# otaviog/align3d

Hardware: AMD Instinct MI355X
Metric: ICP frame-pairs/sec (640x480, 3-lvl, 15 iters) (higher is better)
Workload: dtype f32; 1 GPU; ms3x15 x 64 pairs/GPU, distinct frames, 640x480, 3 lvl x 15 it, HBM-resident (configs[4] shard); pairs_per_gpu=64, global_pairs=64, levels=3, distinct_frames=True, ranks_in_collective=1, collective=none

## Files before the change

### align3d_amd/_abi.py

```python
import ctypes as C
import os
import threading

import numpy as np

A3D_OK = 0
A3D_INVALID_PARAMETER = 1
A3D_MISSING_FIELD = 2
A3D_SOLVE_FAILED = 3
A3D_HIP_ERROR = 4
A3D_NAN_IN_INPUT = 5
A3D_CAST_OVERFLOW = 6

STATUS_NAMES = {
    0: "A3D_OK",
    1: "A3D_INVALID_PARAMETER",
    2: "A3D_MISSING_FIELD",
    3: "A3D_SOLVE_FAILED",
    4: "A3D_HIP_ERROR",
    5: "A3D_NAN_IN_INPUT",
    6: "A3D_CAST_OVERFLOW",
}


class A3dError(Exception):

    def __init__(self, status, message=""):
        self.status = status
        super().__init__(f"{STATUS_NAMES.get(status, status)}: {message}")


class InvalidParameter(A3dError):
    def __init__(self, message):
        super().__init__(A3D_INVALID_PARAMETER, message)


class IcpParamsC(C.Structure):
    _fields_ = [
        ("max_iterations", C.c_uint64),
        ("weight", C.c_float),
        ("color_weight", C.c_float),
        ("max_point_to_plane_distance", C.c_float),
        ("max_distance", C.c_float),
        ("max_normal_angle", C.c_float),
        ("max_color_distance", C.c_float),
    ]


class PoseC(C.Structure):
    _fields_ = [("t", C.c_float * 3), ("q", C.c_float * 4)]


class RangeImageViewC(C.Structure):
    _fields_ = [
        ("points", C.c_void_p),
        ("mask", C.c_void_p),
        ("normals", C.c_void_p),
        ("intensities", C.c_void_p),
        ("intensity_map", C.c_void_p),
        ("fx", C.c_double),
        ("fy", C.c_double),
        ("cx", C.c_double),
        ("cy", C.c_double),
        ("width", C.c_uint64),
        ("height", C.c_uint64),
    ]


class PointCloudViewC(C.Structure):
    _fields_ = [("points", C.c_void_p), ("normals", C.c_void_p), ("len", C.c_uint64)]


class BuilderParamsC(C.Structure):
    _fields_ = [
        ("with_normals", C.c_uint32),
        ("with_intensity", C.c_uint32),
        ("use_bilateral", C.c_uint32),
        ("pad", C.c_uint32),
        ("sigma_space", C.c_double),
        ("sigma_color", C.c_double),
        ("pyramid_levels", C.c_uint64),
        ("blur_sigma", C.c_float),
        ("pad2", C.c_uint32),
    ]


class GnStateC(C.Structure):
    _fields_ = [
        ("hessian", C.c_float * 36),
        ("gradient", C.c_float * 6),
        ("squared_residual_sum", C.c_float),
        ("count", C.c_uint64),
    ]

    def as_dict(self):
        return {
            "H": np.array(self.hessian[:], dtype=np.float32).reshape(6, 6),
            "g": np.array(self.gradient[:], dtype=np.float32),
            "ssq": np.float32(self.squared_residual_sum),
            "count": int(self.count),
        }


def ptr(arr):
    if arr is None:
        return None
    assert arr.flags["C_CONTIGUOUS"], "arrays cross the ABI in standard layout"
    return arr.ctypes.data


_P = C.c_void_p
_PP = C.POINTER(C.c_void_p)
_ST = C.c_int
SIGNATURES = {
    "a3d_abi_version": (C.c_uint32, []),
    "a3d_last_error": (C.c_char_p, []),
    "a3d_status_string": (C.c_char_p, [C.c_int]),
    "a3d_device_count": (_ST, [C.POINTER(C.c_int32)]),
    "a3d_context_create": (_ST, [C.c_int32, _PP]),
    "a3d_context_create_with_priority": (_ST, [C.c_int32, C.c_int32, _PP]),
    "a3d_context_create_pair": (_ST, [C.c_int32, _PP, _PP]),
    "a3d_context_destroy": (_ST, [_P]),
    "a3d_context_synchronize": (_ST, [_P]),
    "a3d_context_stream": (_P, [_P]),
    "a3d_context_device": (C.c_int32, [_P]),
    "a3d_timer_start": (_ST, [_P]),
    "a3d_timer_stop": (_ST, [_P, C.POINTER(C.c_float)]),
    "a3d_malloc": (_ST, [_P, C.c_size_t, _PP]),
    "a3d_host_alloc": (_ST, [_P, C.c_size_t, _PP]),
    "a3d_host_free": (_ST, [_P, _P]),
    "a3d_free": (_ST, [_P, _P]),
    "a3d_memcpy_h2d": (_ST, [_P, _P, _P, C.c_size_t]),
    "a3d_memcpy_d2h": (_ST, [_P, _P, _P, C.c_size_t]),
    "a3d_memcpy_d2d": (_ST, [_P, _P, _P, C.c_size_t]),
    "a3d_icp_params_default": (None, [C.POINTER(IcpParamsC)]),
    "a3d_ms_icp_params_default": (None, [C.POINTER(IcpParamsC)]),
    "a3d_range_image_upload": (_ST, [_P, C.POINTER(RangeImageViewC), _PP]),
    "a3d_range_image_upload_pyramid": (_ST, [_P, C.POINTER(RangeImageViewC), C.c_uint64, _PP]),
    "a3d_range_image_free": (_ST, [_P]),
    "a3d_range_image_compute_normals": (_ST, [_P]),
    "a3d_range_image_download_normals": (_ST, [_P, _P]),
    "a3d_builder_params_default": (None, [C.POINTER(BuilderParamsC)]),
    "a3d_range_image_build_pyramid": (
        _ST,
        [_P, C.POINTER(BuilderParamsC), _P, _P, C.c_uint64, C.c_uint64, C.c_double, C.c_double, C.c_double,
         C.c_double, C.c_double, _PP],
    ),
    "a3d_range_image_build_pyramids": (
        _ST,
        [_P, C.POINTER(BuilderParamsC), C.c_uint64, _PP, _PP, C.c_uint64, C.c_uint64, C.c_double, C.c_double, C.c_double,
         C.c_double, C.c_double, _PP],
    ),
    "a3d_context_last_build_stats": (_ST, [_P, C.POINTER(C.c_uint64)]),
    "a3d_context_set_build_profiling": (_ST, [_P, C.c_int32]),
    "a3d_context_last_build_kernel_ms": (_ST, [_P, C.POINTER(C.c_float)]),
    "a3d_range_image_size": (_ST, [_P, C.POINTER(C.c_uint64), C.POINTER(C.c_uint64)]),
    "a3d_range_image_download": (_ST, [_P, _P, _P, _P, _P, _P, _P, C.POINTER(C.c_double)]),
    "a3d_compute_normals": (_ST, [_P, _P, _P, C.c_uint64, C.c_uint64, _P]),
    "a3d_range_image_compute_normals_batch": (_ST, [_PP, C.c_uint64]),
    "a3d_image_icp_align": (_ST, [_P, C.POINTER(IcpParamsC), _P, _P, C.POINTER(PoseC), C.POINTER(PoseC)]),
    "a3d_image_icp_accumulate": (
        _ST,
        [_P, C.POINTER(IcpParamsC), _P, _P, C.POINTER(PoseC), C.POINTER(GnStateC), C.POINTER(GnStateC)],
    ),
    "a3d_image_icp_align_trace": (
        _ST,
        [_P, C.POINTER(IcpParamsC), _P, _P, C.POINTER(PoseC), C.POINTER(PoseC), _P],
    ),
    "a3d_selftest_division": (_ST, [_P, _P, _P, C.c_uint64, C.POINTER(C.c_uint64)]),
    "a3d_selftest_transform": (_ST, [_P, _P, _P, _P, C.c_uint64, _P, _P, _P]),
    "a3d_multiscale_new": (_ST, [_P, C.POINTER(IcpParamsC), C.c_uint64, _PP, C.c_uint64, _PP]),
    "a3d_multiscale_align": (_ST, [_P, _PP, C.c_uint64, C.POINTER(PoseC)]),
    "a3d_multiscale_align_host": (_ST, [_P, C.POINTER(RangeImageViewC), C.c_uint64, C.POINTER(PoseC)]),
    "a3d_multiscale_free": (_ST, [_P]),
    "a3d_multiscale_batch_new": (
        _ST,
        [_P, C.POINTER(IcpParamsC), C.c_uint64, C.c_uint64, C.c_uint64, _PP, _PP, _PP],
    ),
    "a3d_multiscale_batch_align": (_ST, [_P, C.POINTER(PoseC), _P, C.POINTER(C.c_int32)]),
    "a3d_multiscale_batch_free": (_ST, [_P]),
    "a3d_multiscale_batch_rebind": (_ST, [_P, _P, _P]),
    "a3d_multiscale_batch_last_level_ms": (_ST, [_P, C.c_uint32, C.POINTER(C.c_float), C.POINTER(C.c_uint32)]),
    "a3d_multiscale_batch_results": (_ST, [_P, C.POINTER(PoseC), C.POINTER(C.c_int32)]),
    "a3d_multiscale_batch_last_timing": (_ST, [_P, C.POINTER(C.c_float), C.POINTER(C.c_uint64)]),
    "a3d_multiscale_batch_set_profiling": (_ST, [_P, C.c_int32]),
    "a3d_multiscale_batch_last_kernel_ms": (_ST, [_P, C.POINTER(C.c_float)]),
    "a3d_multiscale_batch_concurrency": (_ST, [_P, C.POINTER(C.c_uint32)]),
    "a3d_multiscale_batch_persistent_levels": (_ST, [_P, C.POINTER(C.c_uint32)]),
    "a3d_context_set_tiling": (_ST, [_P, C.c_uint32]),
    "a3d_context_create_on_pipe": (_ST, [C.c_int32, C.c_int32, C.c_int32, _PP]),
    "a3d_multi_shard_range": (_ST, [C.c_uint64, C.c_uint64, C.c_uint64, C.POINTER(C.c_uint64), C.POINTER(C.c_uint64)]),
    "a3d_multi_context_create": (_ST, [C.POINTER(C.c_int32), C.c_uint64, _PP]),
    "a3d_multi_context_destroy": (_ST, [_P]),
    "a3d_multi_context_size": (C.c_uint64, [_P]),
    "a3d_multi_context_device": (_P, [_P, C.c_uint64]),
    "a3d_multiscale_batch_new_multi": (
        _ST,
        [_P, C.POINTER(IcpParamsC), C.c_uint64, C.c_uint64, C.c_uint64, _PP, _PP, _PP],
    ),
    "a3d_multiscale_multi_batch_align": (_ST, [_P, C.POINTER(PoseC), _P, C.POINTER(C.c_int32), _PP]),
    "a3d_multiscale_multi_batch_free": (_ST, [_P]),
    "a3d_kdtree_stats": (_ST, [_P, C.POINTER(C.c_uint64)]),
    "a3d_kdtree_download": (_ST, [_P, _P, _P, C.POINTER(C.c_uint64)]),
    "a3d_kdtree_new": (_ST, [_P, _P, C.c_uint64, _PP]),
    "a3d_kdtree_new_device": (_ST, [_P, _P, C.c_uint64, _PP]),
    "a3d_kdtree_build_path": (_ST, [_P, C.POINTER(C.c_int32)]),
    "a3d_kdtree_build_ms": (_ST, [_P, C.POINTER(C.c_float)]),
    "a3d_kdtree_nearest": (_ST, [_P, _P, C.c_uint64, _P, _P]),
    "a3d_kdtree_nearest_device": (_ST, [_P, _P, C.c_uint64, _P, _P]),
    "a3d_kdtree_free": (_ST, [_P]),
    "a3d_pcl_icp_new": (_ST, [_P, C.POINTER(IcpParamsC), C.POINTER(PointCloudViewC), _PP]),
    "a3d_pcl_icp_align": (_ST, [_P, C.POINTER(PointCloudViewC), C.POINTER(PoseC)]),
    "a3d_pcl_icp_new_device": (_ST, [_P, C.POINTER(IcpParamsC), C.POINTER(PointCloudViewC), _PP]),
    "a3d_pcl_icp_align_device": (_ST, [_P, C.POINTER(PointCloudViewC), C.POINTER(PoseC)]),
    "a3d_pcl_icp_accumulate": (_ST, [_P, C.POINTER(PointCloudViewC), C.POINTER(PoseC), C.POINTER(GnStateC)]),
    "a3d_pcl_icp_last_device_ms": (_ST, [_P, C.POINTER(C.c_float)]),
    "a3d_pcl_icp_free": (_ST, [_P]),
    "a3d_bilateral_default_sigmas": (None, [C.POINTER(C.c_double), C.POINTER(C.c_double)]),
    "a3d_bilateral_filter_u16": (
        _ST,
        [_P, _P, C.c_uint64, C.c_uint64, C.c_double, C.c_double, _P, C.POINTER(C.c_uint64)],
    ),
    "a3d_bilateral_filter_u16_device": (_ST, [_P, _P, C.c_uint64, C.c_uint64, C.c_uint64, C.c_double, C.c_double, _P]),
}

DIAG_SIGNATURES = {
    "a3d_image_icp_accumulate_exact": (
        _ST,
        [_P, C.POINTER(IcpParamsC), _P, _P, C.POINTER(PoseC), C.POINTER(GnStateC), C.POINTER(GnStateC)],
    ),
    "a3d_image_icp_accumulate_weighted": (
        _ST,
        [_P, C.POINTER(IcpParamsC), _P, _P, C.POINTER(PoseC), C.POINTER(GnStateC)],
    ),
}

_CSRC = os.path.join(os.path.dirname(os.path.abspath(__file__)), "csrc")
LIB_PATH = os.environ.get("A3D_LIBRARY") or os.path.join(_CSRC, "libalign3d_hip.so")
DIAG_LIB_PATH = os.path.join(_CSRC, "libalign3d_hip_diag.so")
_libs = {}


def load_library(path=None):
    path = os.path.abspath(path or LIB_PATH)
    if path in _libs:
        return _libs[path]
    if not os.path.exists(path):
        raise RuntimeError(
            f"{path} not found: build the HIP extension first "
            "(python -c 'import __graft_entry__ as g; g.build()' or make -C align3d_amd/csrc all)"
        )
    lib = C.CDLL(path)
    for name, (restype, argtypes) in SIGNATURES.items():
        fn = getattr(lib, name)
        fn.restype = restype
        fn.argtypes = argtypes
        if restype is _ST:
            _note_failures(lib, fn)
    for name, (restype, argtypes) in DIAG_SIGNATURES.items():
        fn = getattr(lib, name, None)
        if fn is not None:
            fn.restype = restype
            fn.argtypes = argtypes
            if restype is _ST:
                _note_failures(lib, fn)
    if lib.a3d_abi_version() != 1:
        raise RuntimeError("libalign3d_hip.so ABI version mismatch")
    _libs[path] = lib
    return lib


_failed = threading.local()


def _note_failures(lib, fn):
    def errcheck(result, func, args):
        if result != A3D_OK:
            _failed.lib = lib
        return result
    fn.errcheck = errcheck


def check(status, what="", lib=None):
    if status != A3D_OK:
        lib = lib or getattr(_failed, "lib", None) or load_library()
        msg = lib.a3d_last_error().decode("utf-8", "replace")
        raise A3dError(status, f"{what}: {msg}" if what else msg)
```

### align3d_amd/csrc/common.hpp

```cpp
#pragma once
#include <hip/hip_runtime.h>

#include <atomic>
#include <memory>
#include <cstdarg>
#include <cstdio>
#include <cstring>
#include <mutex>
#include <string>
#include <utility>
#include <vector>

#include "../../include/align3d_hip.h"
#include "devmath.hpp"

struct a3d_context;

#ifdef A3D_DIAGNOSTICS
#define A3D_DIAG_ENV(name) getenv(name)
#else
#define A3D_DIAG_ENV(name) ((const char*)nullptr)
#endif

namespace a3d {

void set_error(const char* fmt, ...);

#define A3D_HIP_TRY(expr)                                                                 \
  do {                                                                                    \
    hipError_t _e = (expr);                                                               \
    if (_e != hipSuccess) {                                                               \
      a3d::set_error("%s failed: %s (%s:%d)", #expr, hipGetErrorString(_e), __FILE__, __LINE__); \
      return A3D_HIP_ERROR;                                                               \
    }                                                                                     \
  } while (0)

#define A3D_TRY(expr)                  \
  do {                                 \
    a3d_status _s = (expr);            \
    if (_s != A3D_OK) return _s;       \
  } while (0)

#define A3D_REQUIRE(cond, status, msg) \
  do {                                 \
    if (!(cond)) {                     \
      a3d::set_error("%s", msg);       \
      return status;                   \
    }                                  \
  } while (0)

inline Pose pose_from_c(const a3d_pose* p) {
  return Pose{{p->t[0], p->t[1], p->t[2]}, {p->q[0], p->q[1], p->q[2], p->q[3]}};
}
inline void pose_to_c(const Pose& p, a3d_pose* o) {
  o->t[0] = p.t.x, o->t[1] = p.t.y, o->t[2] = p.t.z;
  o->q[0] = p.q.i, o->q[1] = p.q.j, o->q[2] = p.q.k, o->q[3] = p.q.w;
}

float acos_gate_threshold(float thr, bool strict);

}

namespace a3d {
a3d_status bilateral_filter_device(a3d_context* ctx, const uint16_t* d_img, uint16_t* d_out, uint32_t w, uint32_t h,
                                   double sigma_space, double sigma_color, uint64_t out_grid_dims[3]);
a3d_status upload_pyramid(a3d_context* ctx, const a3d_range_image_view* views, uint64_t n_levels,
                          a3d_device_image** out_images, hipEvent_t* level_events);
a3d_status compute_normals_device(a3d_context* ctx, const float* d_points, const uint8_t* d_mask, float* d_normals,
                                  uint32_t w, uint32_t h);
}

namespace a3d {
struct UseFence;
}
struct a3d_context {
  int device = 0;
  hipStream_t stream = nullptr;
  hipEvent_t ev_start = nullptr, ev_stop = nullptr;
  hipEvent_t kd_ev[2] = {nullptr, nullptr};
  int num_cus = 0;
  void* scratch[3] = {nullptr, nullptr, nullptr};
  size_t scratch_size[3] = {0, 0, 0};
  struct SpareBlock {
    void* p;
    size_t bytes;
  };
  std::vector<SpareBlock> spare_blocks;
  std::atomic<bool> kd_wide_place{true};
  std::atomic<int> kd_quiet_builds{0};
  std::mutex pool_mutex;
  std::vector<std::pair<void*, size_t>> arena_pool;
  std::vector<void*> single_arenas;
  std::vector<void*> arena_slabs;
  std::vector<size_t> slab_sizes;
  size_t slab_bytes_total = 0;
  void* icp_engine = nullptr;
  void (*icp_engine_free)(void*) = nullptr;
  uint32_t* pinned_words = nullptr;
  static constexpr size_t PINNED_WORDS = 16384;
  static constexpr size_t PINNED_EXTRA = 16;
  hipStream_t copy_stream = nullptr;
  std::vector<hipEvent_t> copy_events;
  unsigned long long grid_capacity = 0;
  struct GridLayoutKey {
    const void* region = nullptr;
    unsigned long long capacity = 0;
    uint32_t cell_bytes = 0, flags_stride = 0, frames = 0, columns = 0;
  } grid_clean;
  uint32_t grid_layout_frames = 0;
  std::vector<std::pair<size_t, uint32_t>> arena_requests;
  struct CachedTable {
    uint32_t key[4];
    void* d;
  };
  std::vector<CachedTable> tables;
  int stream_priority = 0;
  std::mutex stream_mutex;
  std::vector<hipStream_t> side_streams;
  uint64_t build_stats[4] = {0, 0, 0, 0};
  bool build_profiling = false;
  std::vector<hipEvent_t> build_events;
  float last_build_kernel_ms = 0.f;
  uint32_t tiles_per_pair = 0;
  int live_arenas = 0;
  bool zombie = false;
};

namespace a3d {
a3d_status ctx_side_stream(a3d_context* ctx, uint32_t index, hipStream_t* out);
a3d_status ctx_scratch(a3d_context* ctx, int which, size_t bytes, void** out);
a3d_status ctx_block_alloc(a3d_context* ctx, size_t bytes, void** out, size_t* out_bytes);
void ctx_block_release(a3d_context* ctx, void* p, size_t bytes);

struct DeviceArena {
  void* base = nullptr;
  size_t bytes = 0;
  bool slab_slice = false;
  std::atomic<int> refs{0};
  std::mutex fence_mutex;
  std::vector<std::shared_ptr<struct UseFence>> fences;
  std::shared_ptr<struct UseFence> self_fence;
};

struct UseFence {
  std::mutex m;
  hipEvent_t ev = nullptr;
  bool recorded = false;
  hipStream_t deferred = nullptr;
  int deferred_device = -1;
  void record_locked(hipStream_t s) {
    if (!ev && hipEventCreateWithFlags(&ev, hipEventDisableTiming) != hipSuccess) {
      ev = nullptr;
      return;
    }
    recorded = hipEventRecord(ev, s) == hipSuccess;
  }
  void record(hipStream_t s) {
    std::lock_guard<std::mutex> lock(m);
    record_locked(s);
  }
  void record_later(hipStream_t s, int device) {
    std::lock_guard<std::mutex> lock(m);
    deferred = s, deferred_device = device;
  }
  void settle_locked() {
    if (deferred && !recorded) {
      int current = -1;
      const bool switched = deferred_device >= 0 && hipGetDevice(&current) == hipSuccess && current != deferred_device &&
                            hipSetDevice(deferred_device) == hipSuccess;
      record_locked(deferred);
      if (!recorded) (void)hipStreamSynchronize(deferred);
      if (switched) (void)hipSetDevice(current);
    }
    deferred = nullptr;
  }
  void wait() {
    std::lock_guard<std::mutex> lock(m);
    settle_locked();
    if (ev && recorded) hipEventSynchronize(ev);
  }
  bool wait_on(hipStream_t s) {
    std::lock_guard<std::mutex> lock(m);
    if (deferred == s && !recorded) return true;
    settle_locked();
    return !(ev && recorded) || hipStreamWaitEvent(s, ev, 0) == hipSuccess;
  }
  void retire() {
    std::lock_guard<std::mutex> lock(m);
    if (ev) hipEventDestroy(ev);
    ev = nullptr, recorded = false;
  }
  ~UseFence() {
    if (ev) hipEventDestroy(ev);
  }
};
#ifdef __HIPCC__
__device__ __forceinline__ uint32_t xcd_contiguous_index(uint32_t b, uint32_t n) {
  const uint32_t g = b & 7u, k = b >> 3, q = n >> 3, r = n & 7u;
  return (g < r ? g * (q + 1u) : r * (q + 1u) + (g - r) * q) + k;
}
#endif

a3d_status ctx_cached_table(a3d_context* ctx, const uint32_t key[4], const void* host, size_t bytes, void** out);

a3d_status ctx_arena_acquire(a3d_context* ctx, size_t bytes, DeviceArena* out);
void ctx_arena_release(a3d_context* ctx, DeviceArena* arena);
void ctx_destroy_now(a3d_context* ctx);
}

struct a3d_device_image;
namespace a3d {
void attach_fence(const a3d_device_image* im, const std::shared_ptr<UseFence>& fence);
}

struct a3d_device_image {
  a3d_context* ctx = nullptr;
  uint32_t width = 0, height = 0;
  double fx64 = 0, fy64 = 0, cx64 = 0, cy64 = 0;
  float fx = 0, fy = 0, cx = 0, cy = 0;
  float* points = nullptr;
  uint8_t* mask = nullptr;
  float* normals = nullptr;
  uint8_t* intensities = nullptr;
  float* imap = nullptr;
  uint8_t* colors = nullptr;
  bool has_normals = false, has_intensities = false, has_imap = false;
  a3d::DeviceArena* arena = nullptr;
  bool built = false;
  bool mask_is_z = false;
  bool own_normals = false;
};
```

### align3d_amd/csrc/devmath.hpp

```cpp
#pragma once
#include <hip/hip_runtime.h>
#include <math.h>
#include <stdint.h>

#define A3D_HD __host__ __device__ __forceinline__

namespace a3d {

struct V3 {
  float x, y, z;
};
A3D_HD V3 operator+(V3 a, V3 b) { return {a.x + b.x, a.y + b.y, a.z + b.z}; }
A3D_HD V3 operator-(V3 a, V3 b) { return {a.x - b.x, a.y - b.y, a.z - b.z}; }
A3D_HD V3 operator*(V3 a, float s) { return {a.x * s, a.y * s, a.z * s}; }
A3D_HD V3 operator/(V3 a, float s) { return {a.x / s, a.y / s, a.z / s}; }
A3D_HD float dot(V3 a, V3 b) { return (a.x * b.x + a.y * b.y) + a.z * b.z; }
A3D_HD float norm_squared(V3 a) { return dot(a, a); }
A3D_HD V3 cross(V3 a, V3 b) {
  return {a.y * b.z - a.z * b.y, a.z * b.x - a.x * b.z, a.x * b.y - a.y * b.x};
}

struct Quat {
  float i, j, k, w;
};
struct Pose {
  V3 t;
  Quat q;
};
A3D_HD Pose pose_eye() { return {{0.f, 0.f, 0.f}, {0.f, 0.f, 0.f, 1.f}}; }

A3D_HD V3 rotate(const Quat& q, V3 v) {
  V3 qv{q.i, q.j, q.k};
  V3 t = cross(qv, v) * 2.0f;
  V3 c = cross(qv, t);
  return (t * q.w + c) + v;
}
A3D_HD V3 transform_vector(const Pose& p, V3 v) { return rotate(p.q, v) + p.t; }
A3D_HD V3 transform_normal(const Pose& p, V3 v) { return rotate(p.q, v); }

A3D_HD Quat qmul(const Quat& a, const Quat& b) {
  Quat r;
  r.w = a.w * b.w - a.i * b.i - a.j * b.j - a.k * b.k;
  r.i = a.w * b.i + a.i * b.w + a.j * b.k - a.k * b.j;
  r.j = a.w * b.j - a.i * b.k + a.j * b.w + a.k * b.i;
  r.k = a.w * b.k + a.i * b.j - a.j * b.i + a.k * b.w;
  return r;
}
A3D_HD Pose compose(const Pose& a, const Pose& b) {
  Pose r;
  r.t = a.t + rotate(a.q, b.t);
  r.q = qmul(a.q, b.q);
  return r;
}

A3D_HD Quat qnormalize(Quat q) {
  float a = q.i * q.i, b = q.j * q.j, c = q.k * q.k, d = q.w * q.w;
  a += c;
  b += d;
  float n = sqrtf(a + b);
  return {q.i / n, q.j / n, q.k / n, q.w / n};
}

A3D_HD float sin_f32(float x) { return sinf(x); }
A3D_HD float cos_f32(float x) { return cosf(x); }

struct Se3Trig {
  float theta, sin_half, cos_half, sin_theta, cos_theta;
};
A3D_HD float se3_theta(const float u[6]) { return sqrtf(norm_squared(V3{u[3], u[4], u[5]})); }

A3D_HD Pose exp_se3_trig(const float u[6], const Se3Trig& tg) {
  const float EPS = 1e-8f;
  V3 omega{u[3], u[4], u[5]};
  float theta_sq0 = norm_squared(omega);
  float theta, imag, real;
  if (theta_sq0 < EPS * EPS) {
    float po4 = theta_sq0 * theta_sq0;
    theta = 0.0f;
    imag = 0.5f - (1.0f / 48.0f) * theta_sq0 + (1.0f / 3840.0f) * po4;
    real = 1.0f - (1.0f / 8.0f) * theta_sq0 + (1.0f / 384.0f) * po4;
  } else {
    theta = tg.theta;
    imag = tg.sin_half / theta;
    real = tg.cos_half;
  }
  Quat q = qnormalize(Quat{imag * omega.x, imag * omega.y, imag * omega.z, real});
  float theta_sq = theta * theta;
  float W[3][3] = {{0.f, -omega.z, omega.y}, {omega.z, 0.f, -omega.x}, {-omega.y, omega.x, 0.f}};
  float V[3][3];
  if (theta_sq < EPS) {
    for (int r = 0; r < 3; ++r)
      for (int c = 0; c < 3; ++c) V[r][c] = (r == c ? 1.0f : 0.0f) + W[r][c] * 0.5f;
  } else {
    float W2[3][3];
    for (int c = 0; c < 3; ++c)
      for (int r = 0; r < 3; ++r) {
        float acc = W[r][0] * W[0][c];
        acc = W[r][1] * W[1][c] + acc;
        acc = W[r][2] * W[2][c] + acc;
        W2[r][c] = acc;
      }
    float a = (1.0f - tg.cos_theta) / theta_sq;
    float b = (theta - tg.sin_theta) / (theta_sq * theta);
    for (int r = 0; r < 3; ++r)
      for (int c = 0; c < 3; ++c) V[r][c] = ((r == c ? 1.0f : 0.0f) + W[r][c] * a) + W2[r][c] * b;
  }
  Pose p;
  float rho[3] = {u[0], u[1], u[2]}, t[3];
  for (int r = 0; r < 3; ++r) {
    float acc = V[r][0] * rho[0];
    acc = V[r][1] * rho[1] + acc;
    acc = V[r][2] * rho[2] + acc;
    t[r] = acc;
  }
  p.t = {t[0], t[1], t[2]};
  p.q = q;
  return p;
}

A3D_HD Pose exp_se3(const float u[6]) {
  Se3Trig tg;
  tg.theta = se3_theta(u);
  const float half = 0.5f * tg.theta;
  tg.sin_half = sin_f32(half), tg.cos_half = cos_f32(half);
  tg.sin_theta = sin_f32(tg.theta), tg.cos_theta = cos_f32(tg.theta);
  return exp_se3_trig(u, tg);
}

A3D_HD void pose_to_matrix(const Pose& p, float m[16]) {
  const float i = p.q.i, j = p.q.j, k = p.q.k, w = p.q.w;
  float ww = w * w, ii = i * i, jj = j * j, kk = k * k;
  float ij = i * j * 2.0f, wk = w * k * 2.0f, wj = w * j * 2.0f, ik = i * k * 2.0f;
  float jk = j * k * 2.0f, wi = w * i * 2.0f;
  m[0] = ww + ii - jj - kk, m[1] = ij - wk, m[2] = wj + ik, m[3] = p.t.x;
  m[4] = wk + ij, m[5] = ww - ii + jj - kk, m[6] = jk - wi, m[7] = p.t.y;
  m[8] = ik - wj, m[9] = wi + jk, m[10] = ww - ii - jj + kk, m[11] = p.t.z;
  m[12] = 0.f, m[13] = 0.f, m[14] = 0.f, m[15] = 1.f;
}

A3D_HD bool gn_solve6(const float H[36], const float g[6], float out[6]) {
  double L[6][6], b[6];
  for (int r = 0; r < 6; ++r) {
    for (int c = 0; c < 6; ++c) L[r][c] = (double)H[r * 6 + c];
    b[r] = (double)g[r];
  }
  for (int j = 0; j < 6; ++j) {
    for (int k = 0; k < j; ++k) {
      double factor = -L[j][k];
      for (int r = j; r < 6; ++r) L[r][j] = factor * L[r][k] + L[r][j];
    }
    double diag = L[j][j];
    if (diag == 0.0) return false;
    if (!(diag >= 0.0)) return false;
    double denom = sqrt(diag);
    L[j][j] = denom;
    for (int r = j + 1; r < 6; ++r) L[r][j] /= denom;
  }
  for (int i = 0; i < 6; ++i) {
    double coeff = b[i] / L[i][i];
    b[i] = coeff;
    for (int r = i + 1; r < 6; ++r) b[r] = -coeff * L[r][i] + b[r];
  }
  for (int i = 5; i >= 0; --i) {
    double d = 0.0;
    for (int r = i + 1; r < 6; ++r) d += L[r][i] * b[r];
    b[i] = (b[i] - d) / L[i][i];
  }
  for (int i = 0; i < 6; ++i) out[i] = (float)b[i];
  return true;
}

A3D_HD constexpr int tri6(int r, int c) { return r * 6 - (r * (r - 1)) / 2 + (c - r); }

#if defined(__HIPCC__)
struct DivBy {
  float negz, y;
};
__device__ __forceinline__ DivBy div_prepare(float z) {
  const float r = __builtin_amdgcn_rcpf(z);
  const float e = __builtin_fmaf(-z, r, 1.0f);
  return {-z, __builtin_fmaf(e, r, r)};
}
__device__ __forceinline__ float div_by(float a, const DivBy d) {
  const float q = a * d.y;
  const float r1 = __builtin_fmaf(d.negz, q, a);
  const float q1 = __builtin_fmaf(r1, d.y, q);
  const float r2 = __builtin_fmaf(d.negz, q1, a);
  return __builtin_fmaf(r2, d.y, q1);
}
__device__ __forceinline__ bool div_den_ok(float z) { return (fabsf(z) > 1e-9f) & (fabsf(z) < 1e9f); }
__device__ __forceinline__ bool div_num_ok(float a) { return (a == 0.0f) | ((fabsf(a) > 1e-20f) & (fabsf(a) < 1e9f)); }


__device__ __forceinline__ V3 normal_from_neighbours_dev(V3 center, V3 left, V3 right, V3 top, V3 bottom) {
  const float ld = norm_squared(left - center), rd = norm_squared(right - center);
  V3 left_to_right;
  if ((ld < 4.0f * rd) & (4.0f * ld > rd))
    left_to_right = right - left;
  else if (ld < rd)
    left_to_right = center - left;
  else
    left_to_right = right - center;
  const float bd = norm_squared(bottom - center), td = norm_squared(top - center);
  V3 bottom_to_top;
  if ((bd < 4.0f * td) & (4.0f * bd > td))
    bottom_to_top = top - bottom;
  else if (bd < td)
    bottom_to_top = center - bottom;
  else
    bottom_to_top = top - center;
  const V3 n = cross(left_to_right, bottom_to_top);
  const float mag = sqrtf(norm_squared(n));
  V3 out{0.f, 0.f, 0.f};
  const bool keep = mag > 1e-6f;
  const bool fast = div_den_ok(mag) & div_num_ok(n.x) & div_num_ok(n.y) & div_num_ok(n.z);
  if (__builtin_expect(__builtin_amdgcn_ballot_w64(keep & !fast) != 0ull, 0)) {
    if (keep) out = n / mag;
  } else if (keep) {
    const DivBy d = div_prepare(mag);
    out = V3{n.x == 0.0f ? n.x : div_by(n.x, d), n.y == 0.0f ? n.y : div_by(n.y, d), n.z == 0.0f ? n.z : div_by(n.z, d)};
  }
  return out;
}

#endif

A3D_HD V3 normal_from_neighbours(V3 center, V3 left, V3 right, V3 top, V3 bottom) {
  const float thr_sq = 2.0f * 2.0f;
  float ld = norm_squared(left - center), rd = norm_squared(right - center);
  float lr_ratio = ld / rd;
  V3 left_to_right;
  if (lr_ratio < thr_sq && lr_ratio > 1.0f / thr_sq)
    left_to_right = right - left;
  else if (ld < rd)
    left_to_right = center - left;
  else
    left_to_right = right - center;
  float bd = norm_squared(bottom - center), td = norm_squared(top - center);
  float bt_ratio = bd / td;
  V3 bottom_to_top;
  if (bt_ratio < thr_sq && bt_ratio > 1.0f / thr_sq)
    bottom_to_top = top - bottom;
  else if (bd < td)
    bottom_to_top = center - bottom;
  else
    bottom_to_top = top - center;
  V3 n = cross(left_to_right, bottom_to_top);
  float mag = sqrtf(norm_squared(n));
  V3 out{0.f, 0.f, 0.f};
  if (mag > 1e-6f) out = n / mag;
  return out;
}

}
```

### align3d_amd/csrc/frame.hip

```cpp
#include <cmath>
#include <cstdlib>
#include <memory>

#include "bilateral.hpp"

using namespace a3d;

namespace {

#ifndef A3D_MAX_BATCH
#define A3D_MAX_BATCH 48
#endif
#ifndef A3D_GRID_BUDGET_GB
#define A3D_GRID_BUDGET_GB 4
#endif
constexpr uint32_t MAX_BATCH = A3D_MAX_BATCH;
struct FrameBases {
  char* arena[MAX_BATCH];
};

typedef float f32x3 __attribute__((ext_vector_type(3)));
typedef f32x3 __attribute__((aligned(4))) f32x3_u;
__device__ __forceinline__ void st_v3(float* base, size_t idx, V3 v) { *(f32x3_u*)(base + 3 * idx) = f32x3{v.x, v.y, v.z}; }
__device__ __forceinline__ void st_v3u(void* base, uint32_t idx, V3 v) {
  *(f32x3_u __attribute__((address_space(1)))*)((a3d_gptr)base + idx * 12u) = f32x3{v.x, v.y, v.z};
}
__device__ __forceinline__ void st_u8u(void* base, uint32_t idx, uint8_t v) {
  *(uint8_t __attribute__((address_space(1)))*)((a3d_gptr)base + idx) = v;
}
__device__ __forceinline__ void st_v3u_stream(void* base, uint32_t idx, V3 v) {
#ifdef A3D_BUILDER_NO_NT
  st_v3u(base, idx, v);
#else
  __builtin_nontemporal_store(f32x3{v.x, v.y, v.z}, (f32x3_u __attribute__((address_space(1)))*)((a3d_gptr)base + idx * 12u));
#endif
}
__device__ __forceinline__ void st_u8u_stream(void* base, uint32_t idx, uint8_t v) {
#ifdef A3D_BUILDER_NO_NT
  st_u8u(base, idx, v);
#else
  __builtin_nontemporal_store(v, (uint8_t __attribute__((address_space(1)))*)((a3d_gptr)base + idx));
#endif
}
__device__ __forceinline__ V3 ld_v3g(const float* base, size_t idx) {
  const f32x3 v = *(const f32x3_u*)(base + 3 * idx);
  return V3{v.x, v.y, v.z};
}

struct LevelLayout {
  uint32_t w, h;
  size_t points, mask, normals, colors, intensities, imap;
};
constexpr uint32_t MAX_LEVELS = 16;
struct PyramidLayout {
  LevelLayout lv[MAX_LEVELS];
};

__device__ __forceinline__ V3 pick_nearest_to_mean(const V3 (&cand)[4], const bool (&ok)[4], int* n_valid) {
  int n = 0;
#pragma unroll
  for (int q = 0; q < 4; ++q) n += ok[q] ? 1 : 0;
  *n_valid = n;
  V3 nearest{0.f, 0.f, 0.f};
  if (n > 0) {
    V3 sum{0.f, 0.f, 0.f};
#pragma unroll
    for (int q = 0; q < 4; ++q)
      if (ok[q]) sum = sum + cand[q];
    V3 mean = sum * (n == 1 ? 1.0f : (n == 2 ? 0.5f : 0.25f));
    if (__builtin_amdgcn_ballot_w64(n == 3) != 0ull)
      if (n == 3) mean = sum / 3.0f;
    float min_dist = 3.402823466e+38f;
#pragma unroll
    for (int q = 0; q < 4; ++q) {
      const float d = norm_squared(cand[q] - mean);
      if (ok[q] && d < min_dist) {
        min_dist = d;
        nearest = cand[q];
      }
    }
  }
  return nearest;
}

#ifdef A3D_DIAGNOSTICS
constexpr int ST_W = 32, ST_H = 16, OWN_W = ST_W - 2, OWN_H = ST_H - 2;

constexpr int L0_PPT = 2, L0_THREADS = ST_W * ST_H / L0_PPT;
#ifndef A3D_L0_PROBE
#define A3D_L0_PROBE 0
#endif
template <bool FILTER>
__global__ void __launch_bounds__(L0_THREADS)
    level0_kernel(const uint16_t* __restrict__ depth, uint32_t w, uint32_t h, double inv_ss, double inv_sc,
                  const double* __restrict__ grids, unsigned long long capacity, uint32_t* __restrict__ scal, float fx,
                  float fy, float cx, float cy, float scale, FrameBases bases, size_t off_points, size_t off_mask,
                  size_t off_normals, bool with_normals, LevelLayout L1, bool emit_l1) {
  __shared__ float sp[3][ST_H][ST_W + 1];
  __shared__ float sn[3][OWN_H][OWN_W + 1];
  __shared__ uint8_t sm[ST_H][ST_W];
  const uint32_t f = blockIdx.z;
  const int lx = threadIdx.x % ST_W, ly0 = threadIdx.x / ST_W;
  const int col = (int)blockIdx.x * OWN_W + lx - 1;
  int ly[L0_PPT], row[L0_PPT];
  bool in[L0_PPT];
  uint32_t d[L0_PPT];
  float px[L0_PPT], py[L0_PPT], pz[L0_PPT];
#pragma unroll
  for (int k = 0; k < L0_PPT; ++k) {
    ly[k] = ly0 + k * (ST_H / L0_PPT);
    row[k] = (int)blockIdx.y * OWN_H + ly[k] - 1;
    in[k] = col >= 0 && col < (int)w && row[k] >= 0 && row[k] < (int)h;
    d[k] = in[k] ? *(const uint16_t __attribute__((address_space(1)))*)((a3d_gptr_c)(depth + (size_t)f * w * h) +
                                                                        (__umul24((uint32_t)row[k], w) + (uint32_t)col) * 2u)
                 : 0u;
    px[k] = py[k] = pz[k] = 0.f;
  }
  const DivBy dfx = div_prepare(fx), dfy = div_prepare(fy);
  const bool focal_ok = div_den_ok(fx) & div_den_ok(fy);
#pragma unroll
  for (int k = 0; k < L0_PPT; ++k) {
    if (in[k]) {
      if (FILTER) {
        uint32_t* sc = scal + f * SC_STRIDE;
        GridDims g;
        uint32_t cmin;
        if (dyn_dims(sc, &g, &cmin)) {
          uint16_t v;
          if (!slice_pixel<true>(d[k], (uint32_t)row[k], (uint32_t)col, inv_ss, inv_sc, cmin, g, grids + f * capacity, &v))
            atomicOr(&sc[SC_OVERFLOW], 1u);
          d[k] = v;
        }
      }
      if (d[k] > 0) {
        pz[k] = (float)d[k] * scale;
        const float ax = ((float)col - cx) * pz[k], ay = ((float)row[k] - cy) * pz[k];
        const bool fast = focal_ok & div_num_ok(ax) & div_num_ok(ay);
        if (__builtin_expect(__builtin_amdgcn_ballot_w64(!fast) != 0ull, 0)) {
          px[k] = ax / fx, py[k] = ay / fy;
        } else {
          px[k] = ax == 0.0f ? ax : div_by(ax, dfx), py[k] = ay == 0.0f ? ay : div_by(ay, dfy);
        }
      }
    }
    sp[0][ly[k]][lx] = px[k], sp[1][ly[k]][lx] = py[k], sp[2][ly[k]][lx] = pz[k];
    sm[ly[k]][lx] = d[k] > 0 ? 1 : 0;
  }
  __syncthreads();
  char* base = bases.arena[f];
  auto at = [&](int y, int x) { return V3{sp[0][y][x], sp[1][y][x], sp[2][y][x]}; };
  bool owned[L0_PPT];
  V3 nrm[L0_PPT];
#pragma unroll
  for (int k = 0; k < L0_PPT; ++k) {
    owned[k] = in[k] && lx != 0 && lx != ST_W - 1 && ly[k] != 0 && ly[k] != ST_H - 1;
    nrm[k] = V3{0.f, 0.f, 0.f};
    if (owned[k] && with_normals && A3D_L0_PROBE != 2 && A3D_L0_PROBE != 4) {
      nrm[k] = normal_from_neighbours_dev(V3{px[k], py[k], pz[k]}, at(ly[k], lx - 1), at(ly[k], lx + 1), at(ly[k] - 1, lx),
                                      at(ly[k] + 1, lx));
      if (emit_l1) sn[0][ly[k] - 1][lx - 1] = nrm[k].x, sn[1][ly[k] - 1][lx - 1] = nrm[k].y, sn[2][ly[k] - 1][lx - 1] = nrm[k].z;
    }
  }
  if (emit_l1) __syncthreads();
#pragma unroll
  for (int k = 0; k < L0_PPT; ++k)
    if (owned[k] && ((A3D_L0_PROBE != 1 && A3D_L0_PROBE != 4) || px[k] == 12345.678f)) {
      const uint32_t idx = __umul24((uint32_t)row[k], w) + (uint32_t)col;
      st_v3u_stream(base + off_points, idx, V3{px[k], py[k], pz[k]});
      st_u8u_stream(base + off_mask, idx, d[k] > 0 ? 1 : 0);
      if (with_normals) st_v3u_stream(base + off_normals, idx, nrm[k]);
    }
  if (!emit_l1 || A3D_L0_PROBE == 3 || A3D_L0_PROBE == 4) return;
  constexpr int L1W = OWN_W / 2, L1N = (OWN_W / 2) * (OWN_H / 2);
  const int t = (int)threadIdx.x;
  const bool normals_task = t >= L1N;
  const int task = normals_task ? t - L1N : t;
  if (task >= L1N || (normals_task && !with_normals)) return;
  const int oy = 2 * (task / L1W), ox = 2 * (task % L1W);
  const uint32_t r0 = blockIdx.y * OWN_H + (uint32_t)oy, c0 = blockIdx.x * OWN_W + (uint32_t)ox;
  if (r0 >= h || c0 >= w) return;
  V3 cand[4];
  bool ok[4];
#pragma unroll
  for (int a = 0; a < 2; ++a)
#pragma unroll
    for (int b = 0; b < 2; ++b) {
      const int q = a * 2 + b;
      cand[q] = normals_task ? V3{sn[0][oy + a][ox + b], sn[1][oy + a][ox + b], sn[2][oy + a][ox + b]}
                             : at(oy + 1 + a, ox + 1 + b);
      ok[q] = sm[oy + 1 + a][ox + 1 + b] == 1;
    }
  int n_valid;
  const V3 pk = pick_nearest_to_mean(cand, ok, &n_valid);
  const uint32_t i1 = __umul24(r0 >> 1, L1.w) + (c0 >> 1);
  st_v3u(base + (normals_task ? L1.normals : L1.points), i1, pk);
  if (!normals_task) st_u8u(base + L1.mask, i1, n_valid > 0 ? 1 : 0);
}
#endif

constexpr int QS = 32, QT = QS / 2;

__device__ __forceinline__ V3 backproject_px(uint32_t d, int row, int col, float fx, float fy, float cx, float cy, float scale,
                                             const DivBy dfx, const DivBy dfy, bool focal_ok) {
  V3 p{0.f, 0.f, 0.f};
  if (d > 0) {
    p.z = (float)d * scale;
    const float ax = ((float)col - cx) * p.z, ay = ((float)row - cy) * p.z;
    const bool fast = focal_ok & div_num_ok(ax) & div_num_ok(ay);
    if (__builtin_expect(__builtin_amdgcn_ballot_w64(!fast) != 0ull, 0)) {
      p.x = ax / fx, p.y = ay / fy;
    } else {
      p.x = ax == 0.0f ? ax : div_by(ax, dfx), p.y = ay == 0.0f ? ay : div_by(ay, dfy);
    }
  }
  return p;
}

template <bool FILTER>
__global__ void __launch_bounds__(256)
    level0_quad_kernel(const uint16_t* __restrict__ depth, uint32_t w, uint32_t h, double inv_ss, double inv_sc,
                       const double* __restrict__ grids, unsigned long long capacity, uint32_t* __restrict__ scal, float fx,
                       float fy, float cx, float cy, float scale, FrameBases bases, size_t off_points, size_t off_mask,
                       size_t off_normals, bool with_normals, LevelLayout L1, bool emit_l1, LevelLayout L2, bool emit_l2,
                       bool l2_is_last, Unsplat unsplat, uint32_t patches_x, uint32_t patches_y) {
  __shared__ float sp[3][QS + 2][QS + 3];
  __shared__ float s1[2][3][QT][QT + 1];
  __shared__ uint8_t s1m[QT][QT];
  __shared__ __attribute__((aligned(4))) uint8_t sm[QS][QS];
#ifndef A3D_LQ_XCD
#define A3D_LQ_XCD 0
#endif
  uint32_t f = blockIdx.z, bx = blockIdx.x, by = blockIdx.y;
  if (patches_x) {
    const uint32_t v = A3D_LQ_XCD ? xcd_contiguous_index(blockIdx.x, gridDim.x) : blockIdx.x;
    const uint32_t per_frame = patches_x * patches_y;
    f = v / per_frame;
    const uint32_t in_frame = v - f * per_frame;
    by = in_frame / patches_x, bx = in_frame - by * patches_x;
  }
  const int t = (int)threadIdx.x, tx = t & (QT - 1), ty = t >> 4;
  const int r0 = (int)by * QS, c0 = (int)bx * QS;
  const uint16_t __attribute__((address_space(1)))* dimg =
      (const uint16_t __attribute__((address_space(1)))*)(depth + (size_t)f * w * h);
  auto load_depth = [&](int row, int col) -> uint32_t {
    const uint32_t r = (uint32_t)min(max(row, 0), (int)h - 1), c = (uint32_t)min(max(col, 0), (int)w - 1);
    return *(const uint16_t __attribute__((address_space(1)))*)((a3d_gptr_c)dimg + (__umul24(r, w) + c) * 2u);
  };
  int row[2], col[2];
  bool rin[2], cin[2];
#pragma unroll
  for (int a = 0; a < 2; ++a) {
    row[a] = r0 + 2 * ty + a, col[a] = c0 + 2 * tx + a;
    rin[a] = row[a] < (int)h, cin[a] = col[a] < (int)w;
  }
  const bool halo_thread = t < 4 * QS;
  const int side = t >> 5, hi = t & (QS - 1);
  const int hy = side == 0 ? 0 : (side == 1 ? QS + 1 : hi + 1), hx = side == 2 ? 0 : (side == 3 ? QS + 1 : hi + 1);
  const int hrow = r0 + hy - 1, hcol = c0 + hx - 1;
  const bool hin = halo_thread && hrow >= 0 && hrow < (int)h && hcol >= 0 && hcol < (int)w;
  uint32_t d[2][2], dh = 0;
#pragma unroll
  for (int a = 0; a < 2; ++a)
#pragma unroll
    for (int b = 0; b < 2; ++b) d[a][b] = load_depth(row[a], col[b]);
  if (halo_thread) dh = load_depth(hrow, hcol);
#pragma unroll
  for (int a = 0; a < 2; ++a)
#pragma unroll
    for (int b = 0; b < 2; ++b) d[a][b] = (rin[a] && cin[b]) ? d[a][b] : 0u;
  dh = hin ? dh : 0u;
  const DivBy dfx = div_prepare(fx), dfy = div_prepare(fy);
  const bool focal_ok = div_den_ok(fx) & div_den_ok(fy);
  GridDims g{0, 0, 0};
  bool grid_ok = false;
  if (FILTER) {
    uint32_t* sc = scal + f * SC_STRIDE;
    uint32_t cmin;
    grid_ok = dyn_dims(sc, &g, &cmin);
    if (grid_ok) {
      const double* grid = grids + f * capacity;
      SliceAxis ry[2], cxs[2];
#pragma unroll
      for (int a = 0; a < 2; ++a) {
        ry[a] = slice_axis_spatial((uint32_t)min(row[a], (int)h - 1), inv_ss, g.gh);
        cxs[a] = slice_axis_spatial((uint32_t)min(col[a], (int)w - 1), inv_ss, g.gw);
      }
      SliceAxis hry{}, hcx{};
      if (halo_thread) {
        hry = slice_axis_spatial((uint32_t)min(max(hrow, 0), (int)h - 1), inv_ss, g.gh);
        hcx = slice_axis_spatial((uint32_t)min(max(hcol, 0), (int)w - 1), inv_ss, g.gw);
      }
      auto colour_axis = [&](uint32_t dv) { return slice_axis((double)(dv - cmin) * inv_sc + 2.0, g.gd); };
      SliceAxis cz[2][2], czh{};
#pragma unroll
      for (int a = 0; a < 2; ++a)
#pragma unroll
        for (int b = 0; b < 2; ++b) cz[a][b] = colour_axis(d[a][b]);
      if (halo_thread) czh = colour_axis(dh);
      auto gather = [&](const SliceAxis& ry_, const SliceAxis& cx_, const SliceAxis& cz_, SliceTaps* tp) {
        tp->za = cz_.frac;
        const uint32_t g0 = __umul24(ry_.lo, g.gw), g1 = __umul24(ry_.hi, g.gw);
        const uint32_t b00 = __umul24(g0 + cx_.lo, g.gd), b01 = __umul24(g0 + cx_.hi, g.gd), b10 = __umul24(g1 + cx_.lo, g.gd),
                       b11 = __umul24(g1 + cx_.hi, g.gd);
        tp->v[0] = cell_value32(grid, b00, cz_.lo), tp->v[1] = cell_value32(grid, b01, cz_.lo);
        tp->v[2] = cell_value32(grid, b10, cz_.lo), tp->v[3] = cell_value32(grid, b11, cz_.lo);
        tp->v[4] = cell_value32(grid, b00, cz_.hi), tp->v[5] = cell_value32(grid, b01, cz_.hi);
        tp->v[6] = cell_value32(grid, b10, cz_.hi), tp->v[7] = cell_value32(grid, b11, cz_.hi);
      };
      bool overflow = false;
      auto finish = [&](const SliceTaps& tp, double ya, double xa, bool in) -> uint32_t {
        uint16_t v;
        const bool fits = slice_combine(tp, ya, xa, &v);
        overflow |= in && !fits;
        return in ? (uint32_t)v : 0u;
      };
      {
        SliceTaps taps[2], htaps;
        gather(ry[0], cxs[0], cz[0][0], &taps[0]);
        gather(ry[0], cxs[1], cz[0][1], &taps[1]);
        if (halo_thread) gather(hry, hcx, czh, &htaps);
        d[0][0] = finish(taps[0], ry[0].frac, cxs[0].frac, rin[0] && cin[0]);
        d[0][1] = finish(taps[1], ry[0].frac, cxs[1].frac, rin[0] && cin[1]);
        __builtin_amdgcn_sched_barrier(0);
        gather(ry[1], cxs[0], cz[1][0], &taps[0]);
        gather(ry[1], cxs[1], cz[1][1], &taps[1]);
        if (halo_thread) dh = finish(htaps, hry.frac, hcx.frac, hin);
        d[1][0] = finish(taps[0], ry[1].frac, cxs[0].frac, rin[1] && cin[0]);
        d[1][1] = finish(taps[1], ry[1].frac, cxs[1].frac, rin[1] && cin[1]);
      }
      if (overflow) atomicOr(&sc[SC_OVERFLOW], 1u);
    }
  }
  V3 P[2][2];
#pragma unroll
  for (int a = 0; a < 2; ++a)
#pragma unroll
    for (int b = 0; b < 2; ++b) {
      P[a][b] = backproject_px(d[a][b], row[a], col[b], fx, fy, cx, cy, scale, dfx, dfy, focal_ok);
      const int y = 2 * ty + a + 1, x = 2 * tx + b + 1;
      sp[0][y][x] = P[a][b].x, sp[1][y][x] = P[a][b].y, sp[2][y][x] = P[a][b].z;
      sm[y - 1][x - 1] = d[a][b] > 0 ? 1 : 0;
    }
  if (halo_thread) {
    const V3 ph = backproject_px(dh, hrow, hcol, fx, fy, cx, cy, scale, dfx, dfy, focal_ok);
    sp[0][hy][hx] = ph.x, sp[1][hy][hx] = ph.y, sp[2][hy][hx] = ph.z;
  }
  __syncthreads();
#ifdef A3D_DIAGNOSTICS
  if (FILTER && grid_ok && unsplat.packed)
    unsplat_columns(unsplat, f, g, inv_ss, r0, min(r0 + QS, (int)h), c0, min(c0 + QS, (int)w), by * patches_x + bx,
                    patches_x * patches_y);
#endif
  char* base = bases.arena[f];
  auto at = [&](int y, int x) { return V3{sp[0][y][x], sp[1][y][x], sp[2][y][x]}; };
  V3 N[2][2];
#pragma unroll
  for (int a = 0; a < 2; ++a)
#pragma unroll
    for (int b = 0; b < 2; ++b) {
      N[a][b] = V3{0.f, 0.f, 0.f};
      if (with_normals && rin[a] && cin[b]) {
        const int y = 2 * ty + a + 1, x = 2 * tx + b + 1;
        const V3 left = b ? P[a][0] : at(y, x - 1), right = b ? at(y, x + 1) : P[a][1];
        const V3 top = a ? P[0][b] : at(y - 1, x), bottom = a ? at(y + 1, x) : P[1][b];
        N[a][b] = normal_from_neighbours_dev(P[a][b], left, right, top, bottom);
      }
    }
#ifndef A3D_LQ_PROBE
#define A3D_LQ_PROBE 0
#endif
  const int sx = t & (QS - 1), sy0 = t >> 5;
  const bool scol_in = c0 + sx < (int)w;
  auto store_rows = [&](size_t off, bool with_mask) {
#pragma unroll
    for (int k = 0; k < 4; ++k) {
      const int y = sy0 + 8 * k;
      if (scol_in && r0 + y < (int)h && (A3D_LQ_PROBE != 1 || sp[0][y + 1][sx + 1] == 12345.678f)) {
        const uint32_t idx = __umul24((uint32_t)(r0 + y), w) + (uint32_t)(c0 + sx);
        st_v3u_stream(base + off, idx, at(y + 1, sx + 1));
        if (with_mask) st_u8u_stream(base + off_mask, idx, sm[y][sx]);
      }
    }
  };
  const bool mask_words = (w & 3u) == 0;
  if (mask_words) {
    const int my = t >> 3, mx = 4 * (t & 7);
    if (r0 + my < (int)h && c0 + mx < (int)w && A3D_LQ_PROBE != 1)
      __builtin_nontemporal_store(*(const uint32_t*)&sm[my][mx],
                                  (uint32_t __attribute__((address_space(1)))*)((a3d_gptr)(base + off_mask) +
                                                                               (__umul24((uint32_t)(r0 + my), w) + (uint32_t)(c0 + mx))));
  }
  store_rows(off_points, !mask_words);
  if (with_normals) {
    __syncthreads();
#pragma unroll
    for (int a = 0; a < 2; ++a)
#pragma unroll
      for (int b = 0; b < 2; ++b) {
        const int y = 2 * ty + a + 1, x = 2 * tx + b + 1;
        sp[0][y][x] = N[a][b].x, sp[1][y][x] = N[a][b].y, sp[2][y][x] = N[a][b].z;
      }
    __syncthreads();
    store_rows(off_normals, false);
  }
  if (!emit_l1 || A3D_LQ_PROBE == 3) return;
  const bool quad_in = rin[0] && cin[0];
  V3 cand[4];
  bool ok[4];
#pragma unroll
  for (int q = 0; q < 4; ++q) cand[q] = P[q >> 1][q & 1], ok[q] = d[q >> 1][q & 1] > 0;
  int n_valid = 0;
  const V3 pk_p = pick_nearest_to_mean(cand, ok, &n_valid);
  V3 pk_n{0.f, 0.f, 0.f};
  if (with_normals) {
#pragma unroll
    for (int q = 0; q < 4; ++q) cand[q] = N[q >> 1][q & 1];
    int unused;
    pk_n = pick_nearest_to_mean(cand, ok, &unused);
  }
  if (quad_in) {
    const uint32_t i1 = __umul24((uint32_t)row[0] >> 1, L1.w) + ((uint32_t)col[0] >> 1);
    if (emit_l2) {
      st_v3u_stream(base + L1.points, i1, pk_p);
      st_u8u_stream(base + L1.mask, i1, n_valid > 0 ? 1 : 0);
      if (with_normals) st_v3u_stream(base + L1.normals, i1, pk_n);
    } else {
      st_v3u(base + L1.points, i1, pk_p);
      st_u8u(base + L1.mask, i1, n_valid > 0 ? 1 : 0);
      if (with_normals) st_v3u(base + L1.normals, i1, pk_n);
    }
  }
  if (!emit_l2) return;
  s1[0][0][ty][tx] = pk_p.x, s1[0][1][ty][tx] = pk_p.y, s1[0][2][ty][tx] = pk_p.z;
  s1[1][0][ty][tx] = pk_n.x, s1[1][1][ty][tx] = pk_n.y, s1[1][2][ty][tx] = pk_n.z;
  s1m[ty][tx] = (quad_in && n_valid > 0) ? 1 : 0;
  __syncthreads();
  const int which = t >> 6;
  if (which > 1 || (which == 1 && !with_normals)) return;
  const int ly = (t >> 3) & 7, lx = t & 7;
  const uint32_t r2 = ((uint32_t)r0 >> 2) + (uint32_t)ly, c2 = ((uint32_t)c0 >> 2) + (uint32_t)lx;
  if (r2 >= L2.h || c2 >= L2.w) return;
#pragma unroll
  for (int q = 0; q < 4; ++q) {
    const int y = 2 * ly + (q >> 1), x = 2 * lx + (q & 1);
    cand[q] = V3{s1[which][0][y][x], s1[which][1][y][x], s1[which][2][y][x]};
    ok[q] = s1m[y][x] == 1;
  }
  const V3 pk2 = pick_nearest_to_mean(cand, ok, &n_valid);
  const uint32_t i2 = __umul24(r2, L2.w) + c2;
  char* dst = base + (which ? L2.normals : L2.points);
  if (l2_is_last) {
    st_v3u_stream(dst, i2, pk2);
    if (!which) st_u8u_stream(base + L2.mask, i2, n_valid > 0 ? 1 : 0);
  } else {
    st_v3u(dst, i2, pk2);
    if (!which) st_u8u(base + L2.mask, i2, n_valid > 0 ? 1 : 0);
  }
}

__global__ void __launch_bounds__(256) scatter_colors_kernel(const uint4* __restrict__ staged, size_t bytes_per_frame,
                                                             size_t off_colors, FrameBases bases) {
  const size_t i = (size_t)blockIdx.x * 256 + threadIdx.x, n16 = bytes_per_frame / 16;
  const uint8_t* src = (const uint8_t*)staged + (size_t)blockIdx.z * bytes_per_frame;
  uint8_t* dst = (uint8_t*)(bases.arena[blockIdx.z] + off_colors);
  if (i < n16) ((uint4*)dst)[i] = ((const uint4*)src)[i];
  if (i == 0)
    for (size_t k = n16 * 16; k < bytes_per_frame; ++k) dst[k] = src[k];
}

__device__ __forceinline__ uint8_t luma_u8(const uint8_t* __restrict__ rgb, uint32_t i) {
  const float l = (float)rgb[3 * i] * 0.3f + (float)rgb[3 * i + 1] * 0.59f + (float)rgb[3 * i + 2] * 0.11f;
  return l >= 255.0f ? 255 : (l <= 0.0f ? 0 : (uint8_t)l);
}

__device__ __forceinline__ uint8_t luma_of(uint32_t r, uint32_t g, uint32_t b) {
  const float l = (float)r * 0.3f + (float)g * 0.59f + (float)b * 0.11f;
  return l >= 255.0f ? 255 : (l <= 0.0f ? 0 : (uint8_t)l);
}
__device__ __forceinline__ float imap_border_cell(const uint8_t* __restrict__ rgb, uint32_t w, uint32_t h, uint32_t r, uint32_t c) {
  if (r >= h && c + 1 < w) return (float)luma_u8(rgb, (h - 1) * w + c) / 255.0f;
  if (c >= w && r + 1 < h) return (float)luma_u8(rgb, r * w + (w - 1)) / 255.0f;
  if ((r == h && c == w) || (r == h + 1 && c == w + 1)) return (float)luma_u8(rgb, (h - 1) * w + (w - 1)) / 255.0f;
  return 0.0f;
}
template <bool QUADS>
__global__ void __launch_bounds__(256) luma_imap_kernel(PyramidLayout layout, FrameBases bases) {
  const LevelLayout L = layout.lv[blockIdx.y];
  const uint32_t i = blockIdx.x * blockDim.x + threadIdx.x;
  const uint32_t w = L.w, h = L.h, mw = w + 2, mh = h + 2;
  char* base = bases.arena[blockIdx.z];
  const uint8_t* __restrict__ rgb = (const uint8_t*)(base + L.colors);
  float* __restrict__ imap = (float*)(base + L.imap);
  if (QUADS) {
    const uint32_t qpr = w / 4, n_quads = h * qpr, n_border = 2 * mw + 2 * h;
    if (i < n_quads) {
      const uint32_t r = i / qpr, c = 4 * (i % qpr), px = r * w + c;
      const uint32_t* src = (const uint32_t*)(rgb + (size_t)px * 3);
      const uint32_t a = src[0], b = src[1], d = src[2];
      const uint8_t l0 = luma_of(a & 255u, (a >> 8) & 255u, (a >> 16) & 255u);
      const uint8_t l1 = luma_of(a >> 24, b & 255u, (b >> 8) & 255u);
      const uint8_t l2 = luma_of((b >> 16) & 255u, b >> 24, d & 255u);
      const uint8_t l3 = luma_of((d >> 8) & 255u, (d >> 16) & 255u, d >> 24);
      const uint32_t packed4 = (uint32_t)l0 | ((uint32_t)l1 << 8) | ((uint32_t)l2 << 16) | ((uint32_t)l3 << 24);
      float* o = imap + (size_t)r * mw + c;
#ifdef A3D_BUILDER_NO_NT
      *(uint32_t*)((uint8_t*)(base + L.intensities) + px) = packed4;
      o[0] = (float)l0 / 255.0f, o[1] = (float)l1 / 255.0f, o[2] = (float)l2 / 255.0f, o[3] = (float)l3 / 255.0f;
#else
      __builtin_nontemporal_store(packed4, (uint32_t*)((uint8_t*)(base + L.intensities) + px));
      __builtin_nontemporal_store((float)l0 / 255.0f, o), __builtin_nontemporal_store((float)l1 / 255.0f, o + 1);
      __builtin_nontemporal_store((float)l2 / 255.0f, o + 2), __builtin_nontemporal_store((float)l3 / 255.0f, o + 3);
#endif
    } else if (i < n_quads + n_border) {
      const uint32_t j = i - n_quads;
      uint32_t r, c;
      if (j < 2 * mw) r = h + j / mw, c = j % mw;
      else r = (j - 2 * mw) / 2, c = w + ((j - 2 * mw) & 1u);
      imap[(size_t)r * mw + c] = imap_border_cell(rgb, w, h, r, c);
    }
    return;
  }
  if (i >= mw * mh) return;
  const uint32_t r = i / mw, c = i % mw;
  float v;
  if (r < h && c < w) {
    const uint8_t l = luma_u8(rgb, r * w + c);
    ((uint8_t*)(base + L.intensities))[r * w + c] = l;
    v = (float)l / 255.0f;
  } else {
    v = imap_border_cell(rgb, w, h, r, c);
  }
  imap[i] = v;
}

__global__ void __launch_bounds__(256) resize_pick_kernel(LevelLayout S, LevelLayout D, FrameBases bases) {
  const uint32_t sw = S.w, sh = S.h, dw = D.w, dh = D.h;
  const uint32_t i = blockIdx.x * blockDim.x + threadIdx.x;
  if (i >= dw * dh) return;
  char* base = bases.arena[blockIdx.z];
  const bool normals = blockIdx.y == 1;
  const float* __restrict__ src = (const float*)(base + (normals ? S.normals : S.points));
  float* __restrict__ dst = (float*)(base + (normals ? D.normals : D.points));
  const uint8_t* __restrict__ src_mask = (const uint8_t*)(base + S.mask);
  const uint32_t dv = i / dw, du = i % dw;
  const float hr = (float)sh / (float)dh, wr = (float)sw / (float)dw;
  const uint32_t sv = (uint32_t)((float)dv * hr), su = (uint32_t)((float)du * wr);
  V3 cand[4];
  bool ok[4];
#pragma unroll
  for (uint32_t a = 0; a < 2; ++a)
#pragma unroll
    for (uint32_t b = 0; b < 2; ++b) {
      const uint32_t r = sv + a, c = su + b, q = a * 2 + b;
      const bool in = r < sh && c < sw;
      const uint32_t k = in ? r * sw + c : 0u;
      ok[q] = in && src_mask[k] == 1;
      cand[q] = ld_v3g(src, k);
    }
  int n;
  const V3 nearest = pick_nearest_to_mean(cand, ok, &n);
  st_v3u_stream(dst, i, nearest);
  if (!normals) st_u8u_stream(base + D.mask, i, n > 0 ? 1 : 0);
}

constexpr int MAX_TAPS = 14;
struct TapRow {
  int32_t left, count;
  float w[MAX_TAPS];
};
__host__ __device__ __forceinline__ void tap_range(uint32_t o, float support, uint32_t size, int32_t* left, int32_t* count) {
  const float in = (float)o + 0.5f;
  int32_t l = (int32_t)floorf(in - support);
  l = l < 0 ? 0 : (l > (int32_t)size - 1 ? (int32_t)size - 1 : l);
  int32_t r = (int32_t)ceilf(in + support);
  r = r < l + 1 ? l + 1 : (r > (int32_t)size ? (int32_t)size : r);
  *left = l, *count = r - l < MAX_TAPS ? r - l : MAX_TAPS;
}

constexpr uint32_t BLUR_TILE = 64, BLUR_ROWS = 4;
constexpr uint32_t BLUR_SPAN = 3 * (2 * BLUR_TILE + MAX_TAPS + 2);
constexpr uint32_t RAW_ROWS = 2 * (BLUR_ROWS - 1) + MAX_TAPS;
constexpr uint32_t RAW_PITCH = ((BLUR_SPAN + 3 + 3) / 4) * 4;
__global__ void __launch_bounds__(256)
    blur_halve_kernel(size_t off_src, uint32_t w, uint32_t dw, uint32_t dh, const TapRow* __restrict__ taps_v,
                      const TapRow* __restrict__ taps_h, size_t off_dst, FrameBases bases) {
  __shared__ uint32_t s_raw[RAW_ROWS * RAW_PITCH / 4];
  __shared__ float s_v[BLUR_ROWS * BLUR_SPAN];
  __shared__ uint32_t s_shift[RAW_ROWS];
  const uint8_t* __restrict__ rgb = (const uint8_t*)(bases.arena[blockIdx.z] + off_src);
  uint8_t* __restrict__ out = (uint8_t*)(bases.arena[blockIdx.z] + off_dst);
  const uint32_t dy0 = blockIdx.y * BLUR_ROWS, rows = min(BLUR_ROWS, dh - dy0);
  const uint32_t dx0 = blockIdx.x * BLUR_TILE, dx1 = min(dx0 + BLUR_TILE, dw) - 1;
  const int32_t vtop = taps_v[dy0].left, vbot = taps_v[dy0 + rows - 1].left + taps_v[dy0 + rows - 1].count;
  const int32_t cmin = taps_h[dx0].left, cmax = taps_h[dx1].left + taps_h[dx1].count;
  const uint32_t span = (uint32_t)(cmax - cmin) * 3u, nraw = (uint32_t)(vbot - vtop);
  const uint32_t words = (span + 3 + 3) / 4;
  for (uint32_t e = threadIdx.x; e < nraw * words; e += 256) {
    const uint32_t j = e / words, k = e % words;
    const size_t first = ((size_t)(vtop + (int32_t)j) * w + (size_t)cmin) * 3;
    s_raw[j * (RAW_PITCH / 4) + k] = *(const uint32_t*)(rgb + (first & ~(size_t)3) + 4 * (size_t)k);
  }
  if (threadIdx.x < nraw)
    s_shift[threadIdx.x] = (uint32_t)((((size_t)(vtop + (int32_t)threadIdx.x) * w + (size_t)cmin) * 3) & 3);
  __syncthreads();
  const uint8_t* raw = (const uint8_t*)s_raw;
  for (uint32_t r = 0; r < rows; ++r) {
    const TapRow* tv = taps_v + dy0 + r;
    const int32_t j0 = tv->left - vtop, vcount = tv->count;
    for (uint32_t x = threadIdx.x; x < span; x += 256) {
      float acc = 0.0f;
#pragma unroll
      for (int k = 0; k < MAX_TAPS; ++k)
        if (k < vcount) {
          const uint32_t j = (uint32_t)(j0 + k);
          acc += (float)raw[j * RAW_PITCH + s_shift[j] + x] * tv->w[k];
        }
      s_v[r * BLUR_SPAN + x] = acc;
    }
  }
  __syncthreads();
  const uint32_t o = threadIdx.x, dx = dx0 + o / 3, ch = o % 3;
  if (o >= BLUR_TILE * 3 || dx >= dw) return;
  const TapRow th = taps_h[dx];
  const uint32_t h0 = (uint32_t)(th.left - cmin) * 3u + ch;
  for (uint32_t r = 0; r < rows; ++r) {
    float acc = 0.0f;
#pragma unroll
    for (int k = 0; k < MAX_TAPS; ++k)
      if (k < th.count) acc += s_v[r * BLUR_SPAN + h0 + 3u * (uint32_t)k] * th.w[k];
    acc = fminf(fmaxf(acc, 0.0f), 255.0f);
    *(uint8_t __attribute__((address_space(1)))*)((a3d_gptr)out + (((dy0 + r) * dw + dx) * 3u + ch)) = (uint8_t)roundf(acc);
  }
}

__global__ void __launch_bounds__(256)
    blur_halve_words_kernel(size_t off_src, uint32_t w, uint32_t h, uint32_t dw, uint32_t dh, float support,
                            const TapRow* __restrict__ taps_v, const TapRow* __restrict__ taps_h, size_t off_dst,
                            FrameBases bases) {
  constexpr uint32_t PITCH_W = RAW_PITCH / 4;
  __shared__ uint32_t s_raw[RAW_ROWS * PITCH_W];
  __shared__ __attribute__((aligned(16))) float s_v[BLUR_ROWS * PITCH_W * 4];
  __shared__ uint32_t s_tv[BLUR_ROWS][16];
  static_assert(sizeof(TapRow) == 64, "a tap row is sixteen words");
  const uint8_t* __restrict__ rgb = (const uint8_t*)(bases.arena[blockIdx.z] + off_src);
  uint8_t* __restrict__ out = (uint8_t*)(bases.arena[blockIdx.z] + off_dst);
  const uint32_t dy0 = blockIdx.y * BLUR_ROWS, rows = min(BLUR_ROWS, dh - dy0);
  const uint32_t dx0 = blockIdx.x * BLUR_TILE, dx1 = min(dx0 + BLUR_TILE, dw) - 1;
  int32_t vtop, vbot, cmin, cmax, cnt;
  tap_range(2 * dy0, support, h, &vtop, &cnt);
  tap_range(2 * (dy0 + rows - 1), support, h, &vbot, &cnt), vbot += cnt;
  tap_range(2 * dx0, support, w, &cmin, &cnt);
  tap_range(2 * dx1, support, w, &cmax, &cnt), cmax += cnt;
  const uint32_t span = (uint32_t)(cmax - cmin) * 3u, nraw = (uint32_t)(vbot - vtop);
  const uint32_t sh = ((uint32_t)cmin * 3u) & 3u;
  const uint32_t words = (span + sh + 3) / 4;
  const uint32_t o = threadIdx.x, dx = dx0 + o / 3, ch = o % 3;
  const bool owns_output = o < BLUR_TILE * 3 && dx < dw;
  uint4 th4[4] = {};
  if (owns_output) {
    const uint4* src = (const uint4*)(taps_h + dx);
#pragma unroll
    for (int i = 0; i < 4; ++i) th4[i] = src[i];
  }
  const bool stages_taps = threadIdx.x < rows * 16u;
  const uint32_t tv_word = stages_taps ? ((const uint32_t*)(taps_v + dy0))[threadIdx.x] : 0u;
  {
    const uint32_t k = threadIdx.x & 127u, jj = threadIdx.x >> 7;
    const uint32_t row_bytes = w * 3u;
    const uint32_t first = (((uint32_t)vtop * w + (uint32_t)cmin) * 3u & ~3u) + 4u * k;
    uint32_t got[RAW_ROWS / 2];
#pragma unroll
    for (uint32_t i = 0; i < RAW_ROWS / 2; ++i) {
      const uint32_t j = jj + 2 * i;
      got[i] = (k < words && j < nraw) ? *(const uint32_t __attribute__((address_space(1)))*)((a3d_gptr_c)rgb + (first + j * row_bytes)) : 0u;
    }
#pragma unroll
    for (uint32_t i = 0; i < RAW_ROWS / 2; ++i) {
      const uint32_t j = jj + 2 * i;
      if (k < words && j < nraw) s_raw[j * PITCH_W + k] = got[i];
    }
  }
  if (stages_taps) s_tv[threadIdx.x >> 4][threadIdx.x & 15u] = tv_word;
  __syncthreads();
  for (uint32_t e = threadIdx.x; e < rows * 128u; e += 256) {
    const uint32_t r = e >> 7, q = e & 127u;
    if (q >= words) continue;
    const int32_t j0 = (int32_t)s_tv[r][0] - vtop, vcount = __builtin_amdgcn_readfirstlane((int32_t)s_tv[r][1]);
    float a0 = 0.0f, a1 = 0.0f, a2 = 0.0f, a3 = 0.0f;
    auto tap = [&](int k) {
      const uint32_t word = s_raw[(uint32_t)(j0 + k) * PITCH_W + q];
      const float wk = __uint_as_float(s_tv[r][2 + k]);
      a0 += (float)(word & 255u) * wk, a1 += (float)((word >> 8) & 255u) * wk;
      a2 += (float)((word >> 16) & 255u) * wk, a3 += (float)(word >> 24) * wk;
    };
    constexpr int SHORT_TAPS = 6;
    if (vcount <= SHORT_TAPS) {
#pragma unroll
      for (int k = 0; k < SHORT_TAPS; ++k)
        if (k < vcount) tap(k);
    } else {
#pragma unroll
      for (int k = 0; k < MAX_TAPS; ++k)
        if (k < vcount) tap(k);
    }
    *(float4*)(s_v + (r * PITCH_W + q) * 4) = make_float4(a0, a1, a2, a3);
  }
  __syncthreads();
  if (!owns_output) return;
  const uint32_t tw[16] = {th4[0].x, th4[0].y, th4[0].z, th4[0].w, th4[1].x, th4[1].y, th4[1].z, th4[1].w,
                           th4[2].x, th4[2].y, th4[2].z, th4[2].w, th4[3].x, th4[3].y, th4[3].z, th4[3].w};
  const int32_t hcount = (int32_t)tw[1];
  const uint32_t h0 = (uint32_t)((int32_t)tw[0] - cmin) * 3u + ch + sh;
  const bool short_taps = __builtin_amdgcn_ballot_w64(hcount > 6) == 0ull;
  for (uint32_t r = 0; r < rows; ++r) {
    float acc = 0.0f;
    if (short_taps) {
#pragma unroll
      for (int k = 0; k < 6; ++k)
        if (k < hcount) acc += s_v[r * PITCH_W * 4 + h0 + 3u * (uint32_t)k] * __uint_as_float(tw[2 + k]);
    } else {
#pragma unroll
      for (int k = 0; k < MAX_TAPS; ++k)
        if (k < hcount) acc += s_v[r * PITCH_W * 4 + h0 + 3u * (uint32_t)k] * __uint_as_float(tw[2 + k]);
    }
    acc = fminf(fmaxf(acc, 0.0f), 255.0f);
    *(uint8_t __attribute__((address_space(1)))*)((a3d_gptr)out + (((dy0 + r) * dw + dx) * 3u + ch)) = (uint8_t)roundf(acc);
  }
}

std::vector<TapRow> make_taps(uint32_t size, float sigma, uint32_t stride, uint32_t count) {
  const float support = 2.0f * sigma;
  std::vector<TapRow> rows(count);
  for (uint32_t k = 0; k < count; ++k) {
    const uint32_t o = k * stride;
    const float in = (float)o + 0.5f;
    const float c = in - 0.5f;
    TapRow r{};
    tap_range(o, support, size, &r.left, &r.count);
    const int64_t left = r.left;
    float sum = 0.0f, wv[MAX_TAPS];
    for (int i = 0; i < r.count; ++i) {
      const float x = (float)(left + i) - c;
      wv[i] = 1.0f / (std::sqrt(2.0f * 3.14159265358979323846f) * sigma) * std::exp(-(x * x) / (2.0f * sigma * sigma));
      sum += wv[i];
    }
    for (int i = 0; i < r.count; ++i) r.w[i] = wv[i] / sum;
    rows[k] = r;
  }
  return rows;
}

inline size_t padded(size_t bytes) { return ((std::max<size_t>(1, bytes) + 255) / 256) * 256; }

struct ArenaPlan {
  PyramidLayout layout{};
  size_t bytes = 0;
};
ArenaPlan plan_arena(uint32_t w, uint32_t h, const a3d_builder_params* prm) {
  ArenaPlan p;
  auto take = [&](size_t bytes) {
    const size_t at = p.bytes;
    p.bytes += padded(bytes);
    return at;
  };
  for (uint64_t l = 0; l < prm->pyramid_levels; ++l) {
    LevelLayout& L = p.layout.lv[l];
    L.w = w >> l, L.h = h >> l;
    const size_t n = (size_t)L.w * L.h;
    L.colors = take(n * 3);
    L.points = take(n * 12);
    L.mask = take(n);
    L.normals = prm->with_normals ? take(n * 12) : 0;
    L.intensities = prm->with_intensity ? take(n) : 0;
    L.imap = prm->with_intensity ? take((size_t)(L.w + 2) * (L.h + 2) * 4) : 0;
  }
  return p;
}

a3d_status taps_for(a3d_context* ctx, uint32_t size, uint32_t count, float sigma, TapRow** out) {
  uint32_t key[4] = {0x54415053u , size, count, 0};
  memcpy(&key[3], &sigma, 4);
  for (const auto& t : ctx->tables)
    if (!memcmp(t.key, key, sizeof(key))) {
      *out = (TapRow*)t.d;
      return A3D_OK;
    }
  const std::vector<TapRow> rows = make_taps(size, sigma, 2, count);
  return ctx_cached_table(ctx, key, rows.data(), rows.size() * sizeof(TapRow), (void**)out);
}

a3d_status enqueue_chunk(a3d_context* ctx, const a3d_builder_params* prm, uint32_t F, const uint16_t* d_depth, uint32_t w,
                         uint32_t h, float fx, float fy, float cx, float cy, float depth_scale, const ArenaPlan& plan,
                         const FrameBases& bases, uint32_t* result, bool depth_part, bool color_part) {
  hipStream_t s = ctx->stream;
  hipStream_t color_stream = s;
  const PyramidLayout& P = plan.layout;
  const LevelLayout& L0 = P.lv[0];
  const bool fuse_allowed = !(A3D_DIAG_ENV("A3D_BUILDER_FUSE_L1") && atoi(A3D_DIAG_ENV("A3D_BUILDER_FUSE_L1")) == 0);
  const bool fuse2_allowed = !(A3D_DIAG_ENV("A3D_BUILDER_FUSE_L2") && atoi(A3D_DIAG_ENV("A3D_BUILDER_FUSE_L2")) == 0);
  const bool fuse_l1 = fuse_allowed && prm->pyramid_levels >= 2 && w % 2 == 0 && h % 2 == 0;
  bool fuse_l2 = fuse_l1 && fuse2_allowed && prm->pyramid_levels >= 3 && w % 4 == 0 && h % 4 == 0;
  bool quad = true;
#ifdef A3D_DIAGNOSTICS
  const bool patch_kernel = A3D_DIAG_ENV("A3D_BUILDER_L0") && !strcmp(A3D_DIAG_ENV("A3D_BUILDER_L0"), "patch");
  quad = !patch_kernel;
  if (!quad) fuse_l2 = false;
#endif
  const LevelLayout& L2 = P.lv[prm->pyramid_levels >= 3 ? 2 : 0];
  const bool l2_is_last = prm->pyramid_levels == 3;
  const dim3 gridq((w + QS - 1) / QS, (h + QS - 1) / QS, F);
  if (!depth_part) {
  } else if (prm->use_bilateral) {
    GridBatch gb;
    const bool defer = quad && A3D_DIAG_ENV("A3D_BUILDER_UNSPLAT") && !strcmp(A3D_DIAG_ENV("A3D_BUILDER_UNSPLAT"), "fused");
    A3D_TRY(bilateral_grids_enqueue(ctx, d_depth, F, w, h, prm->sigma_space, prm->sigma_color, ctx->grid_capacity, &gb, defer));
    if (quad) {
      hipLaunchKernelGGL(level0_quad_kernel<true>, dim3(gridq.x * gridq.y * gridq.z), dim3(256), 0, s, d_depth, w, h, 1.0 / prm->sigma_space,
                         1.0 / prm->sigma_color, (const double*)gb.blurred, gb.capacity, gb.scal, fx, fy, cx, cy, depth_scale,
                         bases, L0.points, L0.mask, L0.normals, prm->with_normals != 0, P.lv[1], fuse_l1, L2, fuse_l2, l2_is_last,
                         gb.unsplat, gridq.x, gridq.y);
      if (defer) {
        A3D_HIP_TRY(hipGetLastError());
        ctx->grid_clean = gb.clean;
      }
    }
#ifdef A3D_DIAGNOSTICS
    else
      hipLaunchKernelGGL(level0_kernel<true>, dim3((w + OWN_W - 1) / OWN_W, (h + OWN_H - 1) / OWN_H, F), dim3(L0_THREADS), 0, s,
                         d_depth, w, h, 1.0 / prm->sigma_space, 1.0 / prm->sigma_color, (const double*)gb.blurred, gb.capacity,
                         gb.scal, fx, fy, cx, cy, depth_scale, bases, L0.points, L0.mask, L0.normals, prm->with_normals != 0,
                         P.lv[1], fuse_l1);
#endif
    A3D_HIP_TRY(hipMemcpyAsync(result, gb.scal, (size_t)F * SC_STRIDE * sizeof(uint32_t), hipMemcpyDeviceToHost, s));
  } else {
    if (quad)
      hipLaunchKernelGGL(level0_quad_kernel<false>, dim3(gridq.x * gridq.y * gridq.z), dim3(256), 0, s, d_depth, w, h, 0.0, 0.0,
                         (const double*)nullptr, 0ull, (uint32_t*)nullptr, fx, fy, cx, cy, depth_scale, bases, L0.points, L0.mask,
                         L0.normals, prm->with_normals != 0, P.lv[1], fuse_l1, L2, fuse_l2, l2_is_last, Unsplat{}, gridq.x, gridq.y);
#ifdef A3D_DIAGNOSTICS
    else
      hipLaunchKernelGGL(level0_kernel<false>, dim3((w + OWN_W - 1) / OWN_W, (h + OWN_H - 1) / OWN_H, F), dim3(L0_THREADS), 0, s,
                         d_depth, w, h, 0.0, 0.0, (const double*)nullptr, 0ull, (uint32_t*)nullptr, fx, fy, cx, cy, depth_scale,
                         bases, L0.points, L0.mask, L0.normals, prm->with_normals != 0, P.lv[1], fuse_l1);
#endif
  }
  float sigma = prm->blur_sigma;
  if (sigma <= 0.0f) sigma = 1.0f;
  for (uint64_t l = 1; l < prm->pyramid_levels; ++l) {
    const LevelLayout &S = P.lv[l - 1], &D = P.lv[l];
    if (depth_part && !(l == 1 && fuse_l1) && !(l == 2 && fuse_l2))
      hipLaunchKernelGGL(resize_pick_kernel, dim3((D.w * D.h + 255) / 256, prm->with_normals ? 2 : 1, F), dim3(256), 0, s, S,
                         D, bases);
    if (!color_part) continue;
    TapRow *d_tv = nullptr, *d_th = nullptr;
    A3D_TRY(taps_for(ctx, S.h, D.h, sigma, &d_tv));
    A3D_TRY(taps_for(ctx, S.w, D.w, sigma, &d_th));
    static const bool blur_words = !(A3D_DIAG_ENV("A3D_BUILDER_BLUR") && !strcmp(A3D_DIAG_ENV("A3D_BUILDER_BLUR"), "bytes"));
    const dim3 blur_grid((D.w + BLUR_TILE - 1) / BLUR_TILE, (D.h + BLUR_ROWS - 1) / BLUR_ROWS, F);
    if (blur_words && (S.w * 3) % 4 == 0 && (RAW_PITCH / 4) <= 128)
      hipLaunchKernelGGL(blur_halve_words_kernel, blur_grid, dim3(256), 0, color_stream, S.colors, S.w, S.h, D.w, D.h, 2.0f * sigma, d_tv,
                         d_th, D.colors, bases);
    else
      hipLaunchKernelGGL(blur_halve_kernel, blur_grid, dim3(256), 0, color_stream, S.colors, S.w, D.w, D.h, d_tv, d_th, D.colors, bases);
  }
  if (prm->with_intensity && color_part) {
    bool quads = true;
    for (uint64_t l = 0; l < prm->pyramid_levels; ++l) quads = quads && P.lv[l].w % 4 == 0;
    if (quads)
      hipLaunchKernelGGL(luma_imap_kernel<true>, dim3((h * (w / 4) + 2 * (w + 2) + 2 * h + 255) / 256, (uint32_t)prm->pyramid_levels, F),
                         dim3(256), 0, color_stream, P, bases);
    else
      hipLaunchKernelGGL(luma_imap_kernel<false>, dim3(((w + 2) * (h + 2) + 255) / 256, (uint32_t)prm->pyramid_levels, F),
                         dim3(256), 0, color_stream, P, bases);
  }
  A3D_HIP_TRY(hipGetLastError());
  return A3D_OK;
}

struct Chunk {
  uint32_t F = 0;
  FrameBases bases{};
  uint16_t* d_depth = nullptr;
  uint8_t* d_colors = nullptr;
  bool colors_staged = false;
  std::vector<a3d_device_image*> images;
  uint32_t* result = nullptr;
};

a3d_status chunk_prepare(a3d_context* ctx, const a3d_builder_params* prm, const ArenaPlan& plan, Chunk& c,
                         const uint16_t* const* depth, const uint8_t* const* rgb, uint32_t w, uint32_t h, double fx,
                         double fy, double cx, double cy, hipEvent_t uploaded, bool mask_is_z) {
  const size_t n = (size_t)w * h;
  const uint64_t L = prm->pyramid_levels;
  for (uint32_t f = 0; f < c.F; ++f) {
    DeviceArena* arena = new DeviceArena();
    if (ctx_arena_acquire(ctx, plan.bytes, arena) != A3D_OK) {
      delete arena;
      set_error("a3d_range_image_build_pyramids: hipMalloc(%zu) failed", plan.bytes);
      return A3D_HIP_ERROR;
    }
    c.bases.arena[f] = (char*)arena->base;
    for (uint64_t l = 0; l < L; ++l) {
      const LevelLayout& Y = plan.layout.lv[l];
      a3d_device_image* im = new a3d_device_image();
      im->ctx = ctx, im->arena = arena, im->built = true;
      im->mask_is_z = mask_is_z;
      ++arena->refs;
      im->width = Y.w, im->height = Y.h;
      const double k = std::ldexp(1.0, -(int)l);
      im->fx64 = fx * k, im->fy64 = fy * k, im->cx64 = cx * k, im->cy64 = cy * k;
      im->fx = (float)im->fx64, im->fy = (float)im->fy64, im->cx = (float)im->cx64, im->cy = (float)im->cy64;
      char* b = (char*)arena->base;
      im->colors = (uint8_t*)(b + Y.colors), im->points = (float*)(b + Y.points), im->mask = (uint8_t*)(b + Y.mask);
      if (prm->with_normals) im->normals = (float*)(b + Y.normals), im->has_normals = true;
      if (prm->with_intensity) {
        im->intensities = (uint8_t*)(b + Y.intensities), im->imap = (float*)(b + Y.imap);
        im->has_intensities = im->has_imap = true;
      }
      c.images.push_back(im);
    }
  }
  auto page_locked = [](const void* p) {
    hipPointerAttribute_t a;
    if (hipPointerGetAttributes(&a, p) != hipSuccess) {
      (void)hipGetLastError();
      return false;
    }
    return a.type == hipMemoryTypeHost;
  };
  bool depth_contig = page_locked(depth[0]), rgb_contig = (n * 3) % 16 == 0 && page_locked(rgb[0]);
  for (uint32_t f = 1; f < c.F; ++f) {
    depth_contig &= depth[f] == depth[f - 1] + n;
    rgb_contig &= rgb[f] == rgb[f - 1] + n * 3;
  }
  hipError_t e = hipSuccess;
  if (depth_contig) {
    e = hipMemcpyAsync(c.d_depth, depth[0], (size_t)c.F * n * 2, hipMemcpyHostToDevice, ctx->copy_stream);
  } else {
    for (uint32_t f = 0; f < c.F && e == hipSuccess; ++f)
      e = hipMemcpyAsync(c.d_depth + (size_t)f * n, depth[f], n * 2, hipMemcpyHostToDevice, ctx->copy_stream);
  }
  c.colors_staged = rgb_contig && c.F > 1;
  if (e == hipSuccess && c.colors_staged) {
    e = hipMemcpyAsync(c.d_colors, rgb[0], (size_t)c.F * n * 3, hipMemcpyHostToDevice, ctx->copy_stream);
  } else {
    for (uint32_t f = 0; f < c.F && e == hipSuccess; ++f)
      e = hipMemcpyAsync(c.bases.arena[f] + plan.layout.lv[0].colors, rgb[f], n * 3, hipMemcpyHostToDevice, ctx->copy_stream);
  }
  if (e != hipSuccess) {
    set_error("a3d_range_image_build_pyramids: upload failed: %s", hipGetErrorString(e));
    return A3D_HIP_ERROR;
  }
  A3D_HIP_TRY(hipEventRecord(uploaded, ctx->copy_stream));
  return A3D_OK;
}

a3d_status build_frames(a3d_context* ctx, const a3d_builder_params* prm, uint64_t n_frames, uint64_t chunk_frames,
                        const uint16_t* const* depth, const uint8_t* const* rgb, uint32_t w, uint32_t h, double fx,
                        double fy, double cx, double cy, double depth_scale, a3d_device_image** out_levels) {
  hipStream_t s = ctx->stream;
  const size_t n = (size_t)w * h;
  const ArenaPlan plan = plan_arena(w, h, prm);
  const size_t n_chunks = (size_t)((n_frames + chunk_frames - 1) / chunk_frames);
  std::vector<Chunk> chunks(n_chunks);
  auto fail = [&](a3d_status st) {
    hipStreamSynchronize(ctx->copy_stream);
    hipStreamSynchronize(s);
    for (Chunk& c : chunks)
      for (a3d_device_image* im : c.images) a3d_range_image_free(im);
    return st;
  };
  void* staging = nullptr;
  const size_t depth_bytes = padded((size_t)n_frames * n * 2);
  if (ctx_scratch(ctx, 0, depth_bytes + (size_t)n_frames * n * 3 + 256, &staging) != A3D_OK) return A3D_HIP_ERROR;
  while (ctx->copy_events.size() < n_chunks) {
    hipEvent_t e;
    A3D_HIP_TRY(hipEventCreateWithFlags(&e, hipEventDisableTiming));
    ctx->copy_events.push_back(e);
  }
  if (prm->use_bilateral && ctx->grid_capacity == 0)
    ctx->grid_capacity = bilateral_grid_cells(w, h, prm->sigma_space, prm->sigma_color, 4096);
  for (size_t k = 0; k < n_chunks; ++k) {
    Chunk& c = chunks[k];
    const uint64_t f0 = k * chunk_frames;
    c.F = (uint32_t)std::min<uint64_t>(chunk_frames, n_frames - f0);
    c.d_depth = (uint16_t*)staging + f0 * n;
    c.d_colors = (uint8_t*)staging + depth_bytes + f0 * n * 3;
    c.result = ctx->pinned_words + k * (MAX_BATCH * SC_STRIDE);
    const float fscale = (float)depth_scale;
    const bool mask_is_z = fscale >= 1.1754944e-38f && std::isfinite(fscale);
    const a3d_status st = chunk_prepare(ctx, prm, plan, c, depth + f0, rgb + f0, w, h, fx, fy, cx, cy, ctx->copy_events[k],
                                        mask_is_z);
    if (st != A3D_OK) return fail(st);
  }
  std::vector<size_t> todo(n_chunks);
  for (size_t k = 0; k < n_chunks; ++k) todo[k] = k;
  size_t n_profiled = 0;
  for (int attempt = 0; attempt < 3 && !todo.empty(); ++attempt) {
    for (size_t k : todo) {
      Chunk& c = chunks[k];
      if (attempt == 0 && hipStreamWaitEvent(s, ctx->copy_events[k], 0) != hipSuccess) return fail(A3D_HIP_ERROR);
      if (ctx->build_profiling) {
        while (ctx->build_events.size() < 2 * (n_profiled + 1)) {
          hipEvent_t e;
          if (hipEventCreate(&e) != hipSuccess) return fail(A3D_HIP_ERROR);
          ctx->build_events.push_back(e);
        }
        (void)hipEventRecord(ctx->build_events[2 * n_profiled], s);
      }
      if (attempt == 0 && c.colors_staged)
        hipLaunchKernelGGL(scatter_colors_kernel, dim3((uint32_t)((n * 3 / 16 + 255) / 256), 1, c.F), dim3(256), 0, s,
                           (const uint4*)c.d_colors, n * 3, plan.layout.lv[0].colors, c.bases);
      const a3d_status st = enqueue_chunk(ctx, prm, c.F, c.d_depth, w, h, (float)fx, (float)fy, (float)cx, (float)cy,
                                          (float)depth_scale, plan, c.bases, c.result, true, attempt == 0);
      if (st != A3D_OK) return fail(st);
      if (ctx->build_profiling) (void)hipEventRecord(ctx->build_events[2 * n_profiled++ + 1], s);
    }
    if (hipStreamSynchronize(s) != hipSuccess) {
      set_error("a3d_range_image_build_pyramids: %s", hipGetErrorString(hipGetLastError()));
      return fail(A3D_HIP_ERROR);
    }
    if (!prm->use_bilateral) {
      todo.clear();
      break;
    }
    unsigned long long need = 0;
    bool overflow = false;
    std::vector<size_t> again;
    for (size_t k : todo) {
      bool redo = false;
      for (uint32_t f = 0; f < chunks[k].F; ++f) {
        const uint32_t* r = chunks[k].result + f * SC_STRIDE;
        if (r[SC_TOO_BIG]) need = std::max<unsigned long long>(need, (unsigned long long)r[SC_GH] * r[SC_GW] * r[SC_GD]), redo = true;
        overflow |= r[SC_OVERFLOW] != 0 && !r[SC_TOO_BIG];
      }
      if (redo) again.push_back(k);
    }
    if (overflow) {
      set_error("bilateral slice produced a value outside u16 (the reference panics in num::cast().unwrap())");
      return fail(A3D_CAST_OVERFLOW);
    }
    if (need >= (1ull << 29)) {
      set_error("a3d_range_image_build_pyramids: a frame's bilateral grid would have %llu cells (the device builder handles "
                "grids below 2^29 cells: raise sigma_color or sigma_space)", need);
      return fail(A3D_INVALID_PARAMETER);
    }
    if (need) ctx->grid_capacity = need + need / 4;
    todo.swap(again);
  }
  if (!todo.empty()) {
    set_error("a3d_range_image_build_pyramids: the bilateral grid kept outgrowing its scratch region");
    return fail(A3D_HIP_ERROR);
  }
  for (size_t k = 0; k < n_profiled; ++k) {
    float ms = 0.f;
    if (hipEventElapsedTime(&ms, ctx->build_events[2 * k], ctx->build_events[2 * k + 1]) == hipSuccess) ctx->last_build_kernel_ms += ms;
  }
  size_t o = 0;
  for (Chunk& c : chunks) {
    for (a3d_device_image* im : c.images) out_levels[o++] = im;
    ctx->build_stats[0] += c.F;
    if (prm->use_bilateral)
      for (uint32_t f = 0; f < c.F; ++f) {
        const uint32_t* r = c.result + f * SC_STRIDE;
        ctx->build_stats[1] += (uint64_t)r[SC_GH] * r[SC_GW] * r[SC_GD];
        ctx->build_stats[2] += r[SC_NLIST], ctx->build_stats[3] += r[SC_NZERO];
      }
  }
  return A3D_OK;
}

}

extern "C" {

void a3d_builder_params_default(a3d_builder_params* out) {
  out->with_normals = 1;
  out->with_intensity = 1;
  out->use_bilateral = 0;
  a3d_bilateral_default_sigmas(&out->sigma_space, &out->sigma_color);
  out->pyramid_levels = 3;
  out->blur_sigma = 1.0f;
}

a3d_status a3d_range_image_build_pyramids(a3d_context* ctx, const a3d_builder_params* prm, uint64_t n_frames,
                                          const uint16_t* const* depth_frames, const uint8_t* const* rgb_frames,
                                          uint64_t width, uint64_t height, double fx, double fy, double cx, double cy,
                                          double depth_scale, a3d_device_image** out_levels) {
  A3D_REQUIRE(ctx && prm && depth_frames && rgb_frames && out_levels, A3D_INVALID_PARAMETER, "null argument");
  A3D_REQUIRE(n_frames >= 1 && n_frames <= (1u << 20), A3D_INVALID_PARAMETER, "bad frame count");
  for (uint64_t f = 0; f < n_frames; ++f)
    A3D_REQUIRE(depth_frames[f] && rgb_frames[f], A3D_INVALID_PARAMETER, "null frame pointer");
  A3D_REQUIRE(width > 0 && height > 0 && width * height < (1ull << 28), A3D_INVALID_PARAMETER, "bad image size");
  A3D_REQUIRE(width < (1ull << 23) && height < (1ull << 23), A3D_INVALID_PARAMETER, "image side too long");
  A3D_REQUIRE(prm->pyramid_levels >= 1 && prm->pyramid_levels <= MAX_LEVELS, A3D_INVALID_PARAMETER, "bad pyramid_levels");
  A3D_REQUIRE((width >> (prm->pyramid_levels - 1)) >= 2 && (height >> (prm->pyramid_levels - 1)) >= 2,
              A3D_INVALID_PARAMETER, "image too small for this many pyramid levels");
  A3D_REQUIRE(!prm->use_bilateral || (prm->sigma_space > 0.0 && prm->sigma_color > 0.0 && std::isfinite(prm->sigma_space) &&
                                      std::isfinite(prm->sigma_color)),
              A3D_INVALID_PARAMETER, "bilateral sigmas must be positive and finite");
  A3D_REQUIRE(std::isfinite(prm->blur_sigma), A3D_INVALID_PARAMETER, "blur_sigma must be finite");
  A3D_REQUIRE(prm->pyramid_levels == 1 || prm->blur_sigma <= 3.0f, A3D_INVALID_PARAMETER,
              "blur_sigma above 3 is not supported by the device builder");
  A3D_REQUIRE(!prm->use_bilateral || width * height < (1ull << 24), A3D_INVALID_PARAMETER,
              "the device frame builder's bilateral filter handles images below 2^24 pixels");
  A3D_HIP_TRY(hipSetDevice(ctx->device));
  const uint64_t L = prm->pyramid_levels;
  uint64_t chunk = MAX_BATCH;
  if (prm->use_bilateral) {
    const unsigned long long cap = ctx->grid_capacity ? ctx->grid_capacity
                                                      : bilateral_grid_cells((uint32_t)width, (uint32_t)height, prm->sigma_space,
                                                                             prm->sigma_color, 4096);
    chunk = std::max<uint64_t>(1, std::min<uint64_t>(MAX_BATCH, ((unsigned long long)A3D_GRID_BUDGET_GB << 30) / (cap * 24 + 1)));
  }
  for (uint64_t& v : ctx->build_stats) v = 0;
  ctx->last_build_kernel_ms = 0.f;
  const uint64_t pass = chunk * (a3d_context::PINNED_WORDS / (MAX_BATCH * SC_STRIDE));
  for (uint64_t f0 = 0; f0 < n_frames; f0 += pass) {
    const uint64_t F = std::min<uint64_t>(pass, n_frames - f0);
    const uint64_t pieces = (F + chunk - 1) / chunk, balanced = (F + pieces - 1) / pieces;
    const a3d_status st = build_frames(ctx, prm, F, balanced, depth_frames + f0, rgb_frames + f0, (uint32_t)width, (uint32_t)height,
                                       fx, fy, cx, cy, depth_scale, out_levels + f0 * L);
    if (st != A3D_OK) {
      for (uint64_t k = 0; k < f0 * L; ++k) a3d_range_image_free(out_levels[k]);
      return st;
    }
  }
  return A3D_OK;
}

a3d_status a3d_range_image_build_pyramid(a3d_context* ctx, const a3d_builder_params* prm, const uint16_t* depth,
                                         const uint8_t* rgb, uint64_t width, uint64_t height, double fx, double fy,
                                         double cx, double cy, double depth_scale, a3d_device_image** out_levels) {
  return a3d_range_image_build_pyramids(ctx, prm, 1, &depth, &rgb, width, height, fx, fy, cx, cy, depth_scale, out_levels);
}

a3d_status a3d_context_last_build_stats(a3d_context* ctx, uint64_t out_stats[4]) {
  A3D_REQUIRE(ctx && out_stats, A3D_INVALID_PARAMETER, "null argument");
  for (int k = 0; k < 4; ++k) out_stats[k] = ctx->build_stats[k];
  return A3D_OK;
}

a3d_status a3d_context_set_build_profiling(a3d_context* ctx, int32_t on) {
  A3D_REQUIRE(ctx, A3D_INVALID_PARAMETER, "ctx is null");
  ctx->build_profiling = on != 0;
  return A3D_OK;
}
a3d_status a3d_context_last_build_kernel_ms(a3d_context* ctx, float* out_ms) {
  A3D_REQUIRE(ctx && out_ms, A3D_INVALID_PARAMETER, "null argument");
  *out_ms = ctx->last_build_kernel_ms;
  return A3D_OK;
}

a3d_status a3d_range_image_size(const a3d_device_image* im, uint64_t* out_width, uint64_t* out_height) {
  A3D_REQUIRE(im && out_width && out_height, A3D_INVALID_PARAMETER, "null argument");
  *out_width = im->width, *out_height = im->height;
  return A3D_OK;
}

a3d_status a3d_range_image_download(a3d_device_image* im, float* points, uint8_t* mask, float* normals,
                                    uint8_t* intensities, float* intensity_map, uint8_t* colors, double out_intrinsics[4]) {
  A3D_REQUIRE(im, A3D_INVALID_PARAMETER, "image is null");
  hipStream_t s = im->ctx->stream;
  const size_t n = (size_t)im->width * im->height;
  auto get = [&](void* dst, const void* src, size_t bytes, const char* what) -> a3d_status {
    if (!dst) return A3D_OK;
    A3D_REQUIRE(src, A3D_MISSING_FIELD, what);
    A3D_HIP_TRY(hipMemcpyAsync(dst, src, bytes, hipMemcpyDeviceToHost, s));
    return A3D_OK;
  };
  A3D_TRY(get(points, im->points, n * 12, "image has no points"));
  A3D_TRY(get(mask, im->mask, n, "image has no mask"));
  A3D_TRY(get(normals, im->has_normals ? im->normals : nullptr, n * 12, "image has no normals"));
  A3D_TRY(get(intensities, im->has_intensities ? im->intensities : nullptr, n, "image has no intensities"));
  A3D_TRY(get(intensity_map, im->has_imap ? im->imap : nullptr, (size_t)(im->width + 2) * (im->height + 2) * 4,
              "image has no intensity map"));
  A3D_TRY(get(colors, im->colors, n * 3, "image has no colors"));
  if (out_intrinsics) out_intrinsics[0] = im->fx64, out_intrinsics[1] = im->fy64, out_intrinsics[2] = im->cx64, out_intrinsics[3] = im->cy64;
  A3D_HIP_TRY(hipStreamSynchronize(s));
  return A3D_OK;
}

}
```

### align3d_amd/csrc/image_icp.hip

```cpp
#include <cstdlib>
#include <memory>

#include "icp_engine.hpp"

using namespace a3d;

namespace {

struct LevelDesc {
  const float* src_points;
  const uint8_t* src_mask;
  const uint8_t* src_intensities;
  const float* tgt_points;
  const float* tgt_normals;
  const uint8_t* tgt_mask;
  const float* imap;
  uint32_t src_n;
  uint32_t tw, th;
  float fx, fy, cx, cy;
  uint32_t flags;
  uint32_t ppt;
  uint32_t pad;
};
static_assert(sizeof(LevelDesc) == 96, "LevelDesc layout");

struct Gates {
  float max_distance_sqr;
  float max_color_distance_sqr;
  float dot_reject_max;
};

__device__ __forceinline__ uint32_t f32_as_usize(float x) {
  uint32_t r;
  asm("v_cvt_u32_f32_e32 %0, %1" : "=v"(r) : "v"(x));
  return r;
}
__device__ __forceinline__ int32_t f32_as_i32(float x) {
  int32_t r;
  asm("v_cvt_i32_f32_e32 %0, %1" : "=v"(r) : "v"(x));
  return r;
}

typedef const char __attribute__((address_space(1)))* gptr_c;
template <typename T>
__device__ __forceinline__ T ld(const void* base, uint32_t byte_off) {
  return *(const T __attribute__((address_space(1)))*)((gptr_c)base + byte_off);
}
typedef float f32x3 __attribute__((ext_vector_type(3)));
typedef f32x3 __attribute__((aligned(4))) f32x3_u;
typedef float f32x2 __attribute__((ext_vector_type(2)));
typedef f32x2 __attribute__((aligned(4))) f32x2_u;
__device__ __forceinline__ V3 ld_v3(const float* base, uint32_t idx) {
  uint32_t off;
  asm("v_lshl_add_u32 %0, %1, 1, %1" : "=v"(off) : "v"(idx));
  const f32x3 v = ld<f32x3_u>(base, off << 2);
  return {v.x, v.y, v.z};
}


__device__ __forceinline__ uint32_t texel_offset(uint32_t row, uint32_t width, uint32_t col) {
  return (__umul24(row, width) + col) * 4u;
}

__device__ __forceinline__ float bilerp(float v00, float v10, float v01, float v11, float uf, float vf) {
  float u0 = v00 * (1.0f - uf) + v10 * uf;
  float u1 = v01 * (1.0f - uf) + v11 * uf;
  return u0 * (1.0f - vf) + u1 * vf;
}
__device__ __forceinline__ float bilinear_at(const float* imap, uint32_t mw, float u, float v) {
  const uint32_t ui = f32_as_usize(u), vi = f32_as_usize(v);
  const uint32_t o = texel_offset(vi, mw, ui);
  const f32x2 a = ld<f32x2_u>(imap, o), b = ld<f32x2_u>(imap, o + mw * 4u);
  return bilerp(a.x, a.y, b.x, b.y, u - (float)ui, v - (float)vi);
}

struct SrcPx {
  V3 sp;
  uint8_t intensity;
  bool live;
};
template <bool ZMASK = false>
__device__ __forceinline__ SrcPx stage_a(const LevelDesc& d, uint32_t i, bool in_range) {
  const uint32_t ii = in_range ? i : 0u;
  SrcPx s;
  s.sp = ld_v3(d.src_points, ii);
  s.intensity = ld<uint8_t>(d.src_intensities, ii);
  if (ZMASK) {
    s.live = in_range & (s.sp.z != 0.0f);
    return s;
  }
  const uint8_t mask = ld<uint8_t>(d.src_mask, ii);
  s.live = in_range & (mask != 0);
  return s;
}

struct ProjPx {
  V3 p;
  float u, v;
  V3 tp, tn;
  uint8_t tmask;
  bool live;
};
template <bool ZMASK = false>
__device__ __forceinline__ ProjPx stage_b(const LevelDesc& d, const Pose& T, const SrcPx& s, float twf, float thf) {
  ProjPx o;
  o.p = transform_vector(T, s.sp);
  const float z = o.p.z, au = o.p.x * d.fx, av = o.p.y * d.fy;
  const DivBy dz = div_prepare(z);
  float qu = div_by(au, dz), qv = div_by(av, dz);
  if (__builtin_expect(__builtin_amdgcn_ballot_w64(!(div_den_ok(z) & div_num_ok(au) & div_num_ok(av))) != 0ull, 0))
    qu = au / z, qv = av / z;
  o.u = qu + d.cx;
  o.v = qv + d.cy;
  const float ur = o.u + 0.5f, vr = o.v + 0.5f;
  o.live = s.live & !((ur <= -1.0f) | (ur >= twf) | (vr <= -1.0f) | (vr >= thf));
  const uint32_t col = (uint32_t)f32_as_i32(ur), row = (uint32_t)f32_as_i32(vr);
  const uint32_t tidx = o.live ? __umul24(row, d.tw) + col : 0u;
  o.tp = ld_v3(d.tgt_points, tidx);
  o.tn = ld_v3(d.tgt_normals, tidx);
  o.tmask = ZMASK ? (uint8_t)0 : ld<uint8_t>(d.tgt_mask, tidx);
  return o;
}

struct MapPx {
  float t00, t10, t01, t11;
  uint32_t ui, vi;
};
template <bool ZMASK = false>
__device__ __forceinline__ MapPx stage_c(const LevelDesc& d, const Gates& gt, ProjPx& px, uint32_t mw) {
  const V3 diff = px.tp - px.p;
  const float pn = dot(px.p, px.tn);
  px.live = px.live & (ZMASK ? px.tp.z != 0.0f : px.tmask == 1)
            & !(norm_squared(diff) > gt.max_distance_sqr)
            & !((pn >= -1.0f) & (pn <= gt.dot_reject_max));
  MapPx m;
  m.ui = f32_as_usize(px.u), m.vi = f32_as_usize(px.v);
  const uint32_t o = px.live ? texel_offset(m.vi, mw, m.ui) : 0u;
  const f32x2 a = ld<f32x2_u>(d.imap, o), b = ld<f32x2_u>(d.imap, o + mw * 4u);
  m.t00 = a.x, m.t10 = a.y, m.t01 = b.x, m.t11 = b.y;
  return m;
}

struct Terms {
  float Jg[6], rg;
  float Jc[6], rc;
  bool color;
};
template <bool EXACT = false>
__device__ __forceinline__ Terms stage_d(const LevelDesc& d, const Gates& gt, const ProjPx& px, const MapPx& m,
                                         uint8_t intensity, uint32_t mw) {
  auto fms = [](float a, float b, float c, float e) { return __builtin_fmaf(a, b, -(c * e)); };
  Terms t;
  const V3 P = px.p, n = px.tn;
  {
    const V3 df = px.tp - P;
    t.Jg[0] = n.x, t.Jg[1] = n.y, t.Jg[2] = n.z;
    if (EXACT) {
      t.rg = dot(df, n);
      const V3 tw = cross(P, n);
      t.Jg[3] = tw.x, t.Jg[4] = tw.y, t.Jg[5] = tw.z;
    } else {
      t.rg = __builtin_fmaf(df.z, n.z, __builtin_fmaf(df.y, n.y, df.x * n.x));
      t.Jg[3] = fms(P.y, n.z, P.z, n.y), t.Jg[4] = fms(P.z, n.x, P.x, n.z), t.Jg[5] = fms(P.x, n.y, P.y, n.x);
    }
  }
  const float uf = px.u - (float)m.ui, vf = px.v - (float)m.vi;
  const float value = bilerp(m.t00, m.t10, m.t01, m.t11, uf, vf);
  const float Hh = 0.005f, H_INV = 1.0f / 0.005f;
  const float u2 = px.u + Hh, v2 = px.v + Hh;
  float uh = bilerp(m.t00, m.t10, m.t01, m.t11, u2 - (float)m.ui, vf);
  float vh = bilerp(m.t00, m.t10, m.t01, m.t11, uf, v2 - (float)m.vi);
  const bool u_leaves = f32_as_usize(u2) != m.ui, v_leaves = f32_as_usize(v2) != m.vi;
  if (__builtin_expect(__builtin_amdgcn_ballot_w64(u_leaves | v_leaves) != 0ull, 0)) {
    if (u_leaves) uh = bilinear_at(d.imap, mw, u2, px.v);
    if (v_leaves) vh = bilinear_at(d.imap, mw, px.u, v2);
  }
  const float du = (uh - value) * H_INV;
  const float dv = (vh - value) * H_INV;
  const float sc = (float)intensity * 0.003921569f;
  const float z = P.z;
  t.rc = sc - value;
  t.color = t.rc * t.rc <= gt.max_color_distance_sqr;
  if (EXACT) {
    const float zz = z * z;
    const float dfx = d.fx / z, dcx = -P.x * d.fx / zz, dfy = d.fy / z, dcy = -P.y * d.fy / zz;
    const V3 gr{du * dfx, dv * dfy, du * dcx + dv * dcy};
    const V3 tw = cross(P, gr);
    t.Jc[0] = gr.x, t.Jc[1] = gr.y, t.Jc[2] = gr.z, t.Jc[3] = tw.x, t.Jc[4] = tw.y, t.Jc[5] = tw.z;
    return t;
  }
  const float r0 = __builtin_amdgcn_rcpf(z);
  const float rz = __builtin_fmaf(__builtin_fmaf(-z, r0, 1.0f), r0, r0), rzz = rz * rz;
  const float dfx = d.fx * rz, dfy = d.fy * rz, dcx = (-P.x * d.fx) * rzz, dcy = (-P.y * d.fy) * rzz;
  const V3 gr{du * dfx, dv * dfy, __builtin_fmaf(du, dcx, dv * dcy)};
  t.Jc[0] = gr.x, t.Jc[1] = gr.y, t.Jc[2] = gr.z;
  t.Jc[3] = fms(P.y, gr.z, P.z, gr.y), t.Jc[4] = fms(P.z, gr.x, P.x, gr.z), t.Jc[5] = fms(P.x, gr.y, P.y, gr.x);
  return t;
}

#ifdef A3D_DIAGNOSTICS
template <int G, bool MERGED>
__global__ void __launch_bounds__(256, MERGED ? 5 : 1)
    image_icp_kernel(const LevelDesc* __restrict__ descs, JobState* __restrict__ states, Gates gt,
                     float* __restrict__ partials, unsigned* __restrict__ counters, SolveArgs solve, int PPT) {
  const int pair = blockIdx.y;
  const uint32_t tile = blockIdx.x;
  constexpr int NACC = MERGED ? GN_MERGED : GN_PARTIAL;
  float acc[NACC];
#pragma unroll
  for (int k = 0; k < NACC; ++k) acc[k] = 0.0f;
  const float wg = solve.weight, wc = solve.color_weight;
  auto accumulate = [&](const Terms& t) {
    if (MERGED) {
      float Jg[6], Jc[6];
#pragma unroll
      for (int k = 0; k < 6; ++k) Jg[k] = wg * t.Jg[k], Jc[k] = t.color ? wc * t.Jc[k] : 0.0f;
      gn_step_merged(acc, t.rg, Jg, t.color ? t.rc : 0.0f, Jc, t.color ? 1.0f : 0.0f);
    } else {
      gn_step(acc, t.rg, t.Jg);
      if (t.color) gn_step(acc + (MERGED ? 0 : GN_ACC), t.rc, t.Jc);
    }
  };
  JobState* st = &states[pair];
#ifdef A3D_TAIL_STAMPS
  if (threadIdx.x == 0 && pair == 0 && blockIdx.x == 0) g_tail_stamps[8] = __builtin_amdgcn_s_memrealtime();
#endif
  if (st->status == A3D_OK) {
    const LevelDesc d = descs[pair];
    const Pose T = st->pose;
    const uint32_t mw = d.tw + 2;
    const float twf = (float)d.tw, thf = (float)d.th;
    const uint32_t base = tile * (256u * (uint32_t)PPT) + threadIdx.x;
    auto src_at = [&](int k0, int g) {
      const uint32_t i = base + (uint32_t)(k0 + g) * 256u;
      return stage_a(d, i, (k0 < PPT) && (i < d.src_n));
    };
    if (G == 1) {
      SrcPx sa, sb;
      ProjPx pa, pb;
      uint8_t ia, ib;
      {
        const SrcPx s0 = src_at(0, 0);
        sa = src_at(1, 0);
        pa = stage_b(d, T, s0, twf, thf);
        ia = s0.intensity;
      }
      auto step = [&](ProjPx& cur, uint8_t cur_i, ProjPx& nxt, uint8_t& nxt_i, const SrcPx& s_next, SrcPx& s_new, int k0) {
        s_new = src_at(k0 + 2, 0);
        const MapPx mp = stage_c(d, gt, cur, mw);
        nxt = stage_b(d, T, s_next, twf, thf);
        nxt_i = s_next.intensity;
        if (cur.live) accumulate(stage_d(d, gt, cur, mp, cur_i, mw));
      };
#pragma unroll 1
      for (int k0 = 0; k0 < PPT; k0 += 2) {
        step(pa, ia, pb, ib, sa, sb, k0);
        step(pb, ib, pa, ia, sb, sa, k0 + 1);
      }
    } else {
    SrcPx s1[G];
    ProjPx cur[G];
    uint8_t cur_int[G];
#pragma unroll
    for (int g = 0; g < G; ++g) {
      const SrcPx s0 = src_at(0, g);
      s1[g] = src_at(G, g);
      cur[g] = stage_b(d, T, s0, twf, thf);
      cur_int[g] = s0.intensity;
    }
#pragma unroll 1
    for (int k0 = 0; k0 < PPT; k0 += G) {
      SrcPx s2[G];
      MapPx mp[G];
      ProjPx nxt[G];
      uint8_t nxt_int[G];
#pragma unroll
      for (int g = 0; g < G; ++g) s2[g] = src_at(k0 + 2 * G, g);
#pragma unroll
      for (int g = 0; g < G; ++g) mp[g] = stage_c(d, gt, cur[g], mw);
#pragma unroll
      for (int g = 0; g < G; ++g) {
        nxt[g] = stage_b(d, T, s1[g], twf, thf);
        nxt_int[g] = s1[g].intensity;
      }
#pragma unroll
      for (int g = 0; g < G; ++g) {
        if (cur[g].live) accumulate(stage_d(d, gt, cur[g], mp[g], cur_int[g], mw));
      }
#pragma unroll
      for (int g = 0; g < G; ++g) cur[g] = nxt[g], cur_int[g] = nxt_int[g], s1[g] = s2[g];
    }
    }
  }
#ifdef A3D_TAIL_STAMPS
  if (threadIdx.x == 0 && pair == 0 && blockIdx.x == 0) g_tail_stamps[9] = __builtin_amdgcn_s_memrealtime();
#endif
  SolveArgs sa = solve;
  if (st->status != A3D_OK) sa.mode = SOLVE_NONE;
  block_finish<NACC>(acc, partials + (size_t)pair * gridDim.x * GN_PARTIAL, tile, gridDim.x,
                     counters + pair, st, sa, pair);
}

__global__ void __launch_bounds__(256)
    image_icp_exact_kernel(const LevelDesc* __restrict__ descs, const JobState* __restrict__ states, Gates gt,
                           float* __restrict__ partials, int PPT) {
  float acc[GN_PARTIAL];
#pragma unroll
  for (int k = 0; k < GN_PARTIAL; ++k) acc[k] = 0.0f;
  const LevelDesc d = descs[0];
  const Pose T = states[0].pose;
  const uint32_t mw = d.tw + 2;
  const float twf = (float)d.tw, thf = (float)d.th;
  auto step_exact = [](float* a, float r, const float J[6]) {
    int t = 0;
    for (int i = 0; i < 6; ++i)
      for (int j = i; j < 6; ++j) {
        const float m = J[i] * J[j];
        a[t] = a[t] + m;
        ++t;
      }
    for (int i = 0; i < 6; ++i) {
      const float m = J[i] * r;
      a[21 + i] = a[21 + i] + m;
    }
    const float rr = r * r;
    a[27] = a[27] + rr;
    a[28] += 1.0f;
  };
  for (int k0 = 0; k0 < PPT; ++k0) {
    const uint32_t i = blockIdx.x * (256u * (uint32_t)PPT) + threadIdx.x + (uint32_t)k0 * 256u;
    const SrcPx s0 = stage_a(d, i, i < d.src_n);
    ProjPx px = stage_b(d, T, s0, twf, thf);
    const MapPx mp = stage_c(d, gt, px, mw);
    if (px.live) {
      const Terms t = stage_d<true>(d, gt, px, mp, s0.intensity, mw);
      step_exact(acc, t.rg, t.Jg);
      if (t.color) step_exact(acc + GN_ACC, t.rc, t.Jc);
    }
  }
  block_reduce_store<GN_PARTIAL, false>(acc, partials + (size_t)blockIdx.x * GN_PARTIAL);
}

#endif

template <bool ZMASK>
__device__ __forceinline__ SrcPx pixel_source_at(const LevelDesc& d, uint32_t base, int ppt, int k0) {
  const uint32_t i = base + (uint32_t)k0 * 256u;
  return stage_a<ZMASK>(d, i, (k0 < ppt) && (i < d.src_n));
}
template <bool ZMASK>
__device__ __forceinline__ void pixel_pass(const LevelDesc& d, const Gates& gt, const Pose& T, uint32_t base, int ppt,
                                           const SrcPx& s0, SrcPx sa, float (&acc)[GN_PARTIAL]) {
  const uint32_t mw = d.tw + 2;
  const float twf = (float)d.tw, thf = (float)d.th;
  SrcPx sb;
  ProjPx pa = stage_b<ZMASK>(d, T, s0, twf, thf), pb;
  uint8_t ia = s0.intensity, ib;
  auto step = [&](ProjPx& cur, uint8_t cur_i, ProjPx& nxt, uint8_t& nxt_i, const SrcPx& s_next, SrcPx& s_new, int k0) {
    s_new = pixel_source_at<ZMASK>(d, base, ppt, k0 + 2);
    const MapPx mp = stage_c<ZMASK>(d, gt, cur, mw);
    nxt = stage_b<ZMASK>(d, T, s_next, twf, thf);
    nxt_i = s_next.intensity;
    if (cur.live) {
      const Terms t = stage_d(d, gt, cur, mp, cur_i, mw);
      gn_step(acc, t.rg, t.Jg);
      if (t.color) gn_step(acc + GN_ACC, t.rc, t.Jc);
    }
  };
#pragma unroll 1
  for (int k0 = 0; k0 < ppt; k0 += 2) {
    step(pa, ia, pb, ib, sa, sb, k0);
    step(pb, ib, pa, ia, sb, sa, k0 + 1);
  }
}

template <bool ZMASK>
__global__ void __launch_bounds__(256, 1)
    image_icp_head_kernel(const LevelDesc* __restrict__ descs, const JobState* __restrict__ states_in,
                          JobState* __restrict__ states_out, Gates gt, const float* __restrict__ partials_in,
                          float* __restrict__ partials_out, uint32_t job_stride, HeadArgs head) {
  __shared__ uint32_t s_state[JOB_WORDS];
  const int pair = blockIdx.y;
  const uint32_t tile = blockIdx.x;
  float acc[GN_PARTIAL];
#pragma unroll
  for (int k = 0; k < GN_PARTIAL; ++k) acc[k] = 0.0f;
#if defined(A3D_DIAGNOSTICS) && defined(A3D_TAIL_STAMPS)
  const bool stamping = threadIdx.x == 0 && pair == 0 && tile + 1 == gridDim.x;
  unsigned long long* stamp = g_tail_stamps + 16 + 8 * ((states_out > states_in) ? 1 : 0);
#define A3D_HEAD_STAMP(k) do { if (stamping) stamp[k] = __builtin_amdgcn_s_memrealtime(); } while (0)
#else
#define A3D_HEAD_STAMP(k) do { } while (0)
#endif
  A3D_HEAD_STAMP(0);
  const LevelDesc d = descs[pair];
  const int ppt = (int)d.ppt;
  const uint32_t base = tile * (256u * (uint32_t)ppt) + threadIdx.x;
  const SrcPx s0 = pixel_source_at<ZMASK>(d, base, ppt, 0), s1 = pixel_source_at<ZMASK>(d, base, ppt, 1);
  A3D_HEAD_STAMP(1);
  head_advance(states_in + pair, tile == 0 ? states_out + pair : nullptr, partials_in + (size_t)pair * job_stride, head,
               pair, s_state, tile == 0);
  A3D_HEAD_STAMP(2);
  if ((int)s_state[15] == A3D_OK) {
    auto uni = [&](int k) { return __uint_as_float(__builtin_amdgcn_readfirstlane(s_state[k])); };
    const Pose T{{uni(0), uni(1), uni(2)}, {uni(3), uni(4), uni(5), uni(6)}};
    pixel_pass<ZMASK>(d, gt, T, base, ppt, s0, s1, acc);
  }
  A3D_HEAD_STAMP(3);
  block_reduce_store<GN_PARTIAL, false>(acc, partials_out + (size_t)pair * job_stride + (size_t)tile * GN_PARTIAL);
  A3D_HEAD_STAMP(4);
#undef A3D_HEAD_STAMP
}

#ifdef A3D_DIAGNOSTICS
struct PersistLevel {
  uint32_t desc_base;
  uint32_t iterations;
  uint32_t tiles;
  float weight, color_weight;
  Gates gates;
};
constexpr int PERSIST_MAX_LEVELS = 16;
constexpr uint32_t PAIR_CTRL_WORDS = 64;
constexpr uint32_t ROSTER_CLOSED = 0x80000000u;
constexpr unsigned long long ROSTER_WAIT_TICKS = 2000ull, PERSIST_SPIN_BOUND_TICKS = 200'000'000ull;
struct PersistPlan {
  uint32_t n_levels;
  uint32_t seq0;
  uint32_t counter_base;
  uint32_t finish;
  uint32_t parity;
  int trace_index0;
  int trace_stride;
  HeadArgs prev;
  PersistLevel lv[PERSIST_MAX_LEVELS];
};
struct PersistOut {
  Pose* poses;
  int32_t* status;
  float* matrices;
  unsigned long long* stamps;
};

template <bool ZMASK>
__global__ void __launch_bounds__(256, 4)
    image_icp_persistent_kernel(const LevelDesc* __restrict__ descs, uint32_t n_pairs_total, JobState* __restrict__ states,
                                float* __restrict__ partials, uint32_t partials_half, uint32_t job_stride,
                                unsigned* __restrict__ ctrl, PersistPlan plan, PersistOut out) {
  __shared__ uint32_t s_state[JOB_WORDS];
  __shared__ uint32_t s_rank, s_members;
  __shared__ int s_go;
  const int pair = blockIdx.y;
  unsigned* const counter = ctrl + (size_t)pair * PAIR_CTRL_WORDS;
  unsigned* const roster = counter + 1 + plan.parity;
  unsigned* const members = counter + 3 + plan.parity;
  float* const job_partials = partials + (size_t)pair * job_stride;
  if (threadIdx.x == 0) {
    const uint32_t old = __hip_atomic_fetch_add(roster, 1u, __ATOMIC_RELAXED, __HIP_MEMORY_SCOPE_AGENT);
    uint32_t rank = old & 0xffffu, R = 0;
    if (old & ROSTER_CLOSED) {
      rank = 0xffffffffu;
    } else {
      unsigned long long t0 = 0;
      for (uint32_t spin = 0;; ++spin) {
        R = __hip_atomic_load(members, __ATOMIC_RELAXED, __HIP_MEMORY_SCOPE_AGENT);
        if (R) break;
        uint32_t cur = __hip_atomic_load(roster, __ATOMIC_RELAXED, __HIP_MEMORY_SCOPE_AGENT);
        bool close = !(cur & ROSTER_CLOSED) && (cur & 0xffffu) >= gridDim.x;
        if (!close && !(cur & ROSTER_CLOSED) && (spin & 15u) == 15u) {
          const unsigned long long now = __builtin_amdgcn_s_memrealtime();
          if (!t0) t0 = now;
          close = now - t0 > ROSTER_WAIT_TICKS;
        }
        if (close && __hip_atomic_compare_exchange_strong(roster, &cur, cur | ROSTER_CLOSED, __ATOMIC_RELAXED,
                                                          __ATOMIC_RELAXED, __HIP_MEMORY_SCOPE_AGENT)) {
          R = cur & 0xffffu;
          __hip_atomic_store(members, R, __ATOMIC_RELAXED, __HIP_MEMORY_SCOPE_AGENT);
          break;
        }
        __builtin_amdgcn_s_sleep(1);
      }
    }
    s_rank = rank, s_members = R;
  }
  if (threadIdx.x < JOB_WORDS) s_state[threadIdx.x] = ((const uint32_t*)(states + (size_t)(plan.seq0 & 1u) * n_pairs_total + pair))[threadIdx.x];
  __syncthreads();
  const uint32_t rank = s_rank, R = s_members;
  if (rank == 0xffffffffu) return;
  HeadArgs prev = plan.prev;
  uint32_t seq = plan.seq0;
  uint32_t expected = plan.counter_base;
  int trace_index = plan.trace_index0;
  bool alive = true;
  auto head = [&](bool write_trace) {
    if (prev.mode != SOLVE_NONE) {
      if (threadIdx.x == 0) {
        int go = 1;
        unsigned long long t0 = 0;
        for (uint32_t spin = 0; (int)(__hip_atomic_load(counter, __ATOMIC_RELAXED, __HIP_MEMORY_SCOPE_AGENT) - expected) < 0; ++spin) {
          __builtin_amdgcn_s_sleep(1);
          if ((spin & 255u) == 255u) {
            const unsigned long long now = __builtin_amdgcn_s_memrealtime();
            if (!t0) t0 = now;
            if (now - t0 > PERSIST_SPIN_BOUND_TICKS) {
              go = 0;
              break;
            }
          }
        }
        s_go = go;
      }
      __syncthreads();
      if (!s_go) {
        alive = false;
        return;
      }
    }
    const uint32_t state_bits = threadIdx.x < JOB_WORDS ? s_state[threadIdx.x] : 0u;
    head_sum_and_advance<true>(state_bits, job_partials + (size_t)((seq + 1u) & 1u) * partials_half, prev, pair, s_state,
                               write_trace);
  };
#pragma unroll 1
  for (uint32_t l = 0; l < plan.n_levels && alive; ++l) {
    const PersistLevel lv = plan.lv[l];
    const LevelDesc d = descs[lv.desc_base + pair];
    const int ppt = (int)d.ppt;
    const uint32_t own_tiles = (d.src_n + 256u * d.ppt - 1u) / (256u * d.ppt);
    const uint32_t mine = rank < lv.tiles ? (lv.tiles - rank + R - 1u) / R : 0u;
    if (out.stamps && rank == 0 && threadIdx.x == 0) out.stamps[((size_t)pair * plan.n_levels + l) * 2] = __builtin_amdgcn_s_memrealtime();
#pragma unroll 1
    for (uint32_t it = 0; it < lv.iterations; ++it) {
      const uint32_t base0 = rank * (256u * (uint32_t)ppt) + threadIdx.x;
      SrcPx s0{}, s1{};
      if (mine) s0 = pixel_source_at<ZMASK>(d, base0, ppt, 0), s1 = pixel_source_at<ZMASK>(d, base0, ppt, 1);
      head(rank == 0);
      if (!alive) break;
      const bool ok = (int)s_state[15] == A3D_OK;
      auto uni = [&](int k) { return __uint_as_float(__builtin_amdgcn_readfirstlane(s_state[k])); };
      const Pose T{{uni(0), uni(1), uni(2)}, {uni(3), uni(4), uni(5), uni(6)}};
#pragma unroll 1
      for (uint32_t tile = rank; tile < lv.tiles; tile += R) {
        float acc[GN_PARTIAL];
#pragma unroll
        for (int k = 0; k < GN_PARTIAL; ++k) acc[k] = 0.0f;
        if (ok && tile < own_tiles) {
          const uint32_t base = tile * (256u * (uint32_t)ppt) + threadIdx.x;
          if (tile != rank) s0 = pixel_source_at<ZMASK>(d, base, ppt, 0), s1 = pixel_source_at<ZMASK>(d, base, ppt, 1);
          pixel_pass<ZMASK>(d, lv.gates, T, base, ppt, s0, s1, acc);
        }
        block_reduce_store<GN_PARTIAL, true>(acc, job_partials + (size_t)(seq & 1u) * partials_half + (size_t)tile * GN_PARTIAL);
        __syncthreads();
      }
      if (mine) {
        asm volatile("s_waitcnt vmcnt(0)" ::: "memory");
        __syncthreads();
        if (threadIdx.x == 0) __hip_atomic_fetch_add(counter, mine, __ATOMIC_RELAXED, __HIP_MEMORY_SCOPE_AGENT);
      }
      expected += lv.tiles;
      prev.weight = lv.weight, prev.color_weight = lv.color_weight, prev.mode = SOLVE_IMAGE_ICP;
      prev.tiles = lv.tiles;
      prev.first_in_level = it == 0, prev.last_in_level = it + 1 == lv.iterations;
      prev.trace_index = trace_index++;
      ++seq;
    }
    if (out.stamps && rank == 0 && threadIdx.x == 0) out.stamps[((size_t)pair * plan.n_levels + l) * 2 + 1] = __builtin_amdgcn_s_memrealtime();
  }
  if (alive && plan.finish) head(rank == 0);
  if (rank != 0) return;
  if (threadIdx.x == 0) {
    __hip_atomic_store(counter + 1 + (plan.parity ^ 1u), 0u, __ATOMIC_RELAXED, __HIP_MEMORY_SCOPE_AGENT);
    __hip_atomic_store(counter + 3 + (plan.parity ^ 1u), 0u, __ATOMIC_RELAXED, __HIP_MEMORY_SCOPE_AGENT);
  }
  if (!alive) {
    if (threadIdx.x == 0) {
      states[(size_t)(seq & 1u) * n_pairs_total + pair].status = A3D_HIP_ERROR;
      if (out.status) out.status[pair] = A3D_HIP_ERROR;
    }
    return;
  }
  if (threadIdx.x < JOB_WORDS) ((uint32_t*)(states + (size_t)(seq & 1u) * n_pairs_total + pair))[threadIdx.x] = s_state[threadIdx.x];
  if (plan.finish && threadIdx.x == 0) {
    const float* f = (const float*)s_state;
    const Pose p{{f[0], f[1], f[2]}, {f[3], f[4], f[5], f[6]}};
    if (out.poses) out.poses[pair] = p;
    if (out.status) out.status[pair] = (int32_t)s_state[15];
    if (out.matrices) {
      float m[16];
      pose_to_matrix(p, m);
      for (int k = 0; k < 16; ++k) out.matrices[(size_t)pair * 16 + k] = m[k];
    }
  }
}

#endif

#ifdef A3D_DIAGNOSTICS
struct LevelPlan {
  uint32_t iterations;
  uint32_t epoch_base;
  int trace_base;
};

template <int G>
__global__ void __launch_bounds__(256, 3)
    image_icp_level_kernel(const LevelDesc* __restrict__ descs, JobState* __restrict__ states, Gates gt,
                           float* __restrict__ partials, unsigned* __restrict__ counters,
                           unsigned* __restrict__ epochs, SolveArgs solve, LevelPlan plan, int PPT) {
  __shared__ float s_pose[8];
  __shared__ int s_go;
  const int pair = blockIdx.y;
  JobState* st = &states[pair];
  const LevelDesc d = descs[pair];
  const uint32_t mw = d.tw + 2;
  const float twf = (float)d.tw, thf = (float)d.th;
  const uint32_t base = blockIdx.x * (256u * (uint32_t)PPT) + threadIdx.x;
  float* job_partials = partials + (size_t)pair * gridDim.x * GN_PARTIAL;
#pragma unroll 1
  for (uint32_t it = 0; it < plan.iterations; ++it) {
    if (threadIdx.x == 0) {
      const unsigned want = plan.epoch_base + it;
      int go = load_status(st) == A3D_OK;
      unsigned spins = 0;
      while (go && __hip_atomic_load(&epochs[pair], __ATOMIC_RELAXED, __HIP_MEMORY_SCOPE_AGENT) != want) {
        __builtin_amdgcn_s_sleep(4);
        ++spins;
        if ((spins & 63u) == 0 && load_status(st) != A3D_OK) go = 0;
        if (spins > (1u << 22)) {
          store_status(st, A3D_HIP_ERROR);
          go = 0;
        }
      }
      if (go && load_status(st) != A3D_OK) go = 0;
      const Pose T0 = load_pose(&st->pose);
      s_pose[0] = T0.t.x, s_pose[1] = T0.t.y, s_pose[2] = T0.t.z;
      s_pose[3] = T0.q.i, s_pose[4] = T0.q.j, s_pose[5] = T0.q.k, s_pose[6] = T0.q.w;
      s_go = go;
    }
    __syncthreads();
    if (!s_go) return;
    auto uni = [](float v) { return __uint_as_float(__builtin_amdgcn_readfirstlane(__float_as_uint(v))); };
    const Pose T{{uni(s_pose[0]), uni(s_pose[1]), uni(s_pose[2])},
                 {uni(s_pose[3]), uni(s_pose[4]), uni(s_pose[5]), uni(s_pose[6])}};
    float acc[GN_PARTIAL];
#pragma unroll
    for (int k = 0; k < GN_PARTIAL; ++k) acc[k] = 0.0f;
    {
      auto src_at = [&](int k0, int g) {
        const uint32_t i = base + (uint32_t)(k0 + g) * 256u;
        return stage_a(d, i, (k0 < PPT) && (i < d.src_n));
      };
      SrcPx s1[G];
      ProjPx cur[G];
      uint8_t cur_int[G];
#pragma unroll
      for (int g = 0; g < G; ++g) {
        const SrcPx s0 = src_at(0, g);
        s1[g] = src_at(G, g);
        cur[g] = stage_b(d, T, s0, twf, thf);
        cur_int[g] = s0.intensity;
      }
#pragma unroll 1
      for (int k0 = 0; k0 < PPT; k0 += G) {
        SrcPx s2[G];
        MapPx mp[G];
        ProjPx nxt[G];
        uint8_t nxt_int[G];
#pragma unroll
        for (int g = 0; g < G; ++g) s2[g] = src_at(k0 + 2 * G, g);
#pragma unroll
        for (int g = 0; g < G; ++g) mp[g] = stage_c(d, gt, cur[g], mw);
#pragma unroll
        for (int g = 0; g < G; ++g) {
          nxt[g] = stage_b(d, T, s1[g], twf, thf);
          nxt_int[g] = s1[g].intensity;
        }
#pragma unroll
        for (int g = 0; g < G; ++g) {
          if (cur[g].live) {
            const Terms t = stage_d(d, gt, cur[g], mp[g], cur_int[g], mw);
            gn_step(acc, t.rg, t.Jg);
            if (t.color) gn_step(acc + GN_ACC, t.rc, t.Jc);
          }
        }
#pragma unroll
        for (int g = 0; g < G; ++g) cur[g] = nxt[g], cur_int[g] = nxt_int[g], s1[g] = s2[g];
      }
    }
    __syncthreads();
    SolveArgs sa = solve;
    sa.first_in_level = it == 0;
    sa.last_in_level = it + 1 == plan.iterations;
    sa.trace_index = plan.trace_base + (int)it;
    float* out = job_partials + (size_t)blockIdx.x * GN_PARTIAL;
    block_reduce_store<GN_PARTIAL, true>(acc, out);
    const bool was_last = block_publish_and_finish(job_partials, gridDim.x, counters + pair, st, sa, pair);
    if (was_last && threadIdx.x == 0) {
      asm volatile("s_waitcnt vmcnt(0)" ::: "memory");
      __hip_atomic_store(&epochs[pair], plan.epoch_base + it + 1, __ATOMIC_RELAXED, __HIP_MEMORY_SCOPE_AGENT);
    }
    __syncthreads();
  }
}

typedef float f32x4_t __attribute__((ext_vector_type(4)));

__device__ __forceinline__ int feat_chunk(int row, int chunk) { return row * 16 + ((chunk ^ ((row >> 1) & 3)) << 2); }

__device__ __forceinline__ int tile_index_of_partial(int k) {
  const int a = k >= GN_ACC ? 1 : 0, kk = k - a * GN_ACC, base = a * 7;
  int row, col;
  if (kk < 21) {
    int i = 0, rem = kk;
    while (rem >= 6 - i) { rem -= 6 - i; ++i; }
    row = base + i, col = base + i + rem;
  } else if (kk < 27) {
    row = base + (kk - 21), col = base + 6;
  } else if (kk == 27) {
    row = col = base + 6;
  } else {
    row = col = 14 + a;
  }
  return row * 16 + col;
}

template <int G>
__global__ void __launch_bounds__(256)
    image_icp_mfma_kernel(const LevelDesc* __restrict__ descs, JobState* __restrict__ states, Gates gt,
                          float* __restrict__ partials, unsigned* __restrict__ counters, SolveArgs solve, int PPT) {
  __shared__ __attribute__((aligned(16))) float slab[4][64 * 16];
  const int pair = blockIdx.y;
  const int lane = threadIdx.x & 63, wave = threadIdx.x >> 6;
  float* const my_slab = slab[wave];
  f32x4_t acc0 = {0.f, 0.f, 0.f, 0.f}, acc1 = {0.f, 0.f, 0.f, 0.f};
  JobState* st = &states[pair];
  if (st->status == A3D_OK) {
    const LevelDesc d = descs[pair];
    const Pose T = st->pose;
    const uint32_t mw = d.tw + 2;
    const float twf = (float)d.tw, thf = (float)d.th;
    const uint32_t base = blockIdx.x * (256u * (uint32_t)PPT) + threadIdx.x;
    const int rd_row0 = lane >> 4, rd_chunk = (lane & 15) >> 2, rd_word = lane & 3;
    auto src_at = [&](int k0, int g) {
      const uint32_t i = base + (uint32_t)(k0 + g) * 256u;
      return stage_a(d, i, (k0 < PPT) && (i < d.src_n));
    };
    SrcPx s1[G];
    ProjPx cur[G];
    uint8_t cur_int[G];
#pragma unroll
    for (int g = 0; g < G; ++g) {
      const SrcPx s0 = src_at(0, g);
      s1[g] = src_at(G, g);
      cur[g] = stage_b(d, T, s0, twf, thf);
      cur_int[g] = s0.intensity;
    }
#pragma unroll 1
    for (int k0 = 0; k0 < PPT; k0 += G) {
      SrcPx s2[G];
      MapPx mp[G];
      ProjPx nxt[G];
      uint8_t nxt_int[G];
#pragma unroll
      for (int g = 0; g < G; ++g) s2[g] = src_at(k0 + 2 * G, g);
#pragma unroll
      for (int g = 0; g < G; ++g) mp[g] = stage_c(d, gt, cur[g], mw);
#pragma unroll
      for (int g = 0; g < G; ++g) {
        nxt[g] = stage_b(d, T, s1[g], twf, thf);
        nxt_int[g] = s1[g].intensity;
      }
#pragma unroll
      for (int g = 0; g < G; ++g) {
        f32x4_t f0 = {0.f, 0.f, 0.f, 0.f}, f1 = f0, f2 = f0, f3 = f0;
        if (cur[g].live) {
          const Terms t = stage_d(d, gt, cur[g], mp[g], cur_int[g], mw);
          f0 = f32x4_t{t.Jg[0], t.Jg[1], t.Jg[2], t.Jg[3]};
          f1.x = t.Jg[4], f1.y = t.Jg[5], f1.z = t.rg;
          f3.z = 1.0f;
          if (t.color) {
            f1.w = t.Jc[0];
            f2 = f32x4_t{t.Jc[1], t.Jc[2], t.Jc[3], t.Jc[4]};
            f3.x = t.Jc[5], f3.y = t.rc, f3.w = 1.0f;
          }
        }
        *(f32x4_t*)(my_slab + feat_chunk(lane, 0)) = f0;
        *(f32x4_t*)(my_slab + feat_chunk(lane, 1)) = f1;
        *(f32x4_t*)(my_slab + feat_chunk(lane, 2)) = f2;
        *(f32x4_t*)(my_slab + feat_chunk(lane, 3)) = f3;
        float x[16];
#pragma unroll
        for (int m = 0; m < 16; ++m) x[m] = my_slab[feat_chunk(4 * m + rd_row0, rd_chunk) + rd_word];
#pragma unroll
        for (int m = 0; m < 16; m += 2) {
          acc0 = __builtin_amdgcn_mfma_f32_16x16x4f32(x[m], x[m], acc0, 0, 0, 0);
          acc1 = __builtin_amdgcn_mfma_f32_16x16x4f32(x[m + 1], x[m + 1], acc1, 0, 0, 0);
        }
      }
#pragma unroll
      for (int g = 0; g < G; ++g) cur[g] = nxt[g], cur_int[g] = nxt_int[g], s1[g] = s2[g];
    }
  }
  __syncthreads();
  float* tiles_lds = &slab[0][0];
  {
    const f32x4_t t = acc0 + acc1;
    const int colx = lane & 15, row4 = (lane >> 4) * 4;
    tiles_lds[wave * 256 + (row4 + 0) * 16 + colx] = t.x;
    tiles_lds[wave * 256 + (row4 + 1) * 16 + colx] = t.y;
    tiles_lds[wave * 256 + (row4 + 2) * 16 + colx] = t.z;
    tiles_lds[wave * 256 + (row4 + 3) * 16 + colx] = t.w;
  }
  __syncthreads();
  float* job_partials = partials + (size_t)pair * gridDim.x * GN_PARTIAL;
  if (threadIdx.x < GN_PARTIAL) {
    const int e = tile_index_of_partial(threadIdx.x);
    const float v = (tiles_lds[e] + tiles_lds[256 + e]) + (tiles_lds[512 + e] + tiles_lds[768 + e]);
    __hip_atomic_store((unsigned*)(job_partials + (size_t)blockIdx.x * GN_PARTIAL) + threadIdx.x, __float_as_uint(v),
                       __ATOMIC_RELAXED, __HIP_MEMORY_SCOPE_AGENT);
  }
  SolveArgs sa = solve;
  if (st->status != A3D_OK) sa.mode = SOLVE_NONE;
  block_publish_and_finish(job_partials, gridDim.x, counters + pair, st, sa, pair);
}

#endif

__global__ void division_selftest_kernel(const float* __restrict__ num, const float* __restrict__ den, uint32_t n,
                                         unsigned* __restrict__ mismatches) {
  const uint32_t i = blockIdx.x * blockDim.x + threadIdx.x;
  if (i >= n) return;
  const float a = num[i], z = den[i];
  if (!(div_den_ok(z) && div_num_ok(a))) return;
  const float q = div_by(a, div_prepare(z)), want = a / z;
  if (__float_as_uint(q) != __float_as_uint(want)) atomicAdd(mismatches, 1u);
}

}

#ifdef A3D_DIAGNOSTICS
constexpr uint32_t CTRL_WORDS_PER_PAIR = PAIR_CTRL_WORDS;
#else
constexpr uint32_t CTRL_WORDS_PER_PAIR = 0;
#endif

struct a3d_multiscale_batch {
  a3d_context* ctx = nullptr;
  uint32_t n_pairs = 0, n_levels = 0;
  std::vector<a3d_icp_params> params;
  std::vector<Gates> gates;
  std::vector<uint32_t> tiles, ppt, group;
  std::vector<LevelDesc> h_descs;
  void* d_block = nullptr;
  LevelDesc* d_descs = nullptr;
  JobState* d_states = nullptr;
  hipEvent_t level_ready[16] = {};
  float* d_partials = nullptr;
  size_t partials_capacity = 0;
  size_t partials_half = 0;
  uint32_t max_tiles = 1;
  unsigned* d_counters = nullptr;
  uint32_t counter_base = 0;
  uint32_t persist_parity = 0;
  uint32_t persist_mask = 0;
  uint32_t persist_resident_blocks = 0;
  bool persist_disabled = false;
  bool persist_used = false;
  std::vector<uint32_t> persist_levels;
  uint32_t last_groups = 1;
  unsigned long long* d_stamps = nullptr;
  Pose* d_poses = nullptr;
  Pose* d_init = nullptr;
  int32_t* d_status = nullptr;
  double* d_readback = nullptr;
  hipEvent_t ev0 = nullptr, ev1 = nullptr;
  std::vector<hipEvent_t> kev;
  std::vector<uint8_t> kev_level;
  float last_level_ms[16] = {0};
  uint32_t last_level_launches[16] = {0};
  bool profile_kernels = false;
  uint32_t resident_blocks = 1024;
  bool zmask = false;
  uint32_t n_streams = 1;
  hipStream_t aux_streams[3] = {nullptr, nullptr, nullptr};
  hipEvent_t ev_fork = nullptr, ev_join[3] = {nullptr, nullptr, nullptr};
  float last_total_ms = 0.f, last_kernel_ms = 0.f;
  uint64_t last_kernel_launches = 0;
  const Pose* last_init = nullptr;
  uint32_t last_levels = 0;
  float* last_matrices = nullptr;
  std::shared_ptr<UseFence> fence = std::make_shared<UseFence>();
  std::shared_ptr<UseFence> descs_uploaded = std::make_shared<UseFence>();
#ifdef A3D_DIAGNOSTICS
  unsigned* d_epochs = nullptr;
  bool use_level_kernel = false;
  uint32_t level_mask = 0;
  uint32_t level_resident_blocks = 0;
  bool use_mfma = false, merged_accumulators = false;
  bool head_solve = true;
  bool exact_solve = false;
#endif

  ~a3d_multiscale_batch() {
    fence->retire();
    hipFree(d_block);
    hipFree(d_partials);
    hipFree(d_stamps);
    if (ev0) hipEventDestroy(ev0);
    if (ev1) hipEventDestroy(ev1);
    for (auto e : kev) hipEventDestroy(e);
    for (int i = 0; i < 3; ++i) {
      if (ev_join[i]) hipEventDestroy(ev_join[i]);
    }
    if (ev_fork) hipEventDestroy(ev_fork);
  }
};

namespace {

a3d_status fill_desc(const a3d_device_image* target, const a3d_device_image* source, LevelDesc* d) {
  A3D_REQUIRE(target && source, A3D_INVALID_PARAMETER, "null image handle");
  A3D_REQUIRE(target->has_imap, A3D_MISSING_FIELD, "Please, the target image should have a intensity map.");
  A3D_REQUIRE(target->has_normals, A3D_MISSING_FIELD, "Please, the target image should have normals.");
  A3D_REQUIRE(source->has_intensities, A3D_MISSING_FIELD,
              "Please, the source image should have intensity colors.");
  d->imap = target->imap;
  d->src_points = source->points, d->src_mask = source->mask, d->src_intensities = source->intensities;
  d->tgt_points = target->points, d->tgt_normals = target->normals, d->tgt_mask = target->mask;
  d->src_n = source->width * source->height;
  d->tw = target->width;
  d->th = target->height;
  d->fx = target->fx, d->fy = target->fy, d->cx = target->cx, d->cy = target->cy;
  d->flags = (target->mask_is_z && source->mask_is_z) ? 1u : 0u;
  d->ppt = 2, d->pad = 0;
  return A3D_OK;
}

Gates make_gates(const a3d_icp_params& p) {
  Gates g;
  g.max_distance_sqr = p.max_distance * p.max_distance;
  g.max_color_distance_sqr = p.max_color_distance * p.max_color_distance;
  g.dot_reject_max = acos_gate_threshold(p.max_normal_angle, false);
  return g;
}

void tiling_for(uint32_t n, uint32_t want, uint32_t group, uint32_t* tiles, uint32_t* ppt) {
  const uint32_t step = std::max(2u, group);
  want = std::max(1u, std::min(want, std::max(1u, (n + 256 * step - 1) / (256 * step))));
  uint32_t p = (n + 256 * want - 1) / (256 * want);
  p = std::max(step, ((p + step - 1) / step) * step);
  *ppt = p;
  *tiles = std::max(1u, (n + 256 * p - 1) / (256 * p));
}

void plan_tiling(a3d_multiscale_batch* b) {
  const uint32_t P = b->n_pairs, L = b->n_levels;
  const uint32_t pinned = b->ctx->tiles_per_pair;
  float waves = P >= 8 ? (b->n_streams > 2 ? 1.5f : 1.0f) : 0.25f;
  if (const char* env = A3D_DIAG_ENV("A3D_ICP_WAVES"))
    if (*env) waves = (float)atof(env);
  uint32_t mask = 0;
  if (const char* env = A3D_DIAG_ENV("A3D_ICP_PERSIST"))
    if (*env) mask = (uint32_t)strtoul(env, nullptr, 0) & ((1u << L) - 1u);
  if (!b->persist_resident_blocks) mask = 0;
  const uint32_t persist_tiles_cap = std::max(1u, b->persist_resident_blocks / std::max(1u, P));
  for (uint32_t l = 0; l < L; ++l) {
    uint32_t max_n = 0;
    for (uint32_t p = 0; p < P; ++p) max_n = std::max(max_n, b->h_descs[(size_t)l * P + p].src_n);
    b->group[l] = 1;
    float w = waves;
#ifdef A3D_DIAGNOSTICS
    if (const char* env = getenv("A3D_ICP_GROUP")) b->group[l] = atoi(env) == 2 ? 2 : 1;
    if (const char* env = getenv("A3D_ICP_GROUP_LEVELS")) {
      unsigned gl[3] = {1, 1, 1};
      sscanf(env, "%u,%u,%u", &gl[0], &gl[1], &gl[2]);
      if (l < 3) b->group[l] = (gl[l] == 2 || gl[l] == 4) ? gl[l] : 1;
    }
    if (const char* env = getenv("A3D_ICP_WAVES_LEVELS")) {
      float wl[3] = {waves, waves, waves};
      sscanf(env, "%f,%f,%f", &wl[0], &wl[1], &wl[2]);
      if (l < 3) w = wl[l];
    }
#endif
    uint32_t want = std::max(1u, (uint32_t)((float)b->resident_blocks * w / (float)P + 0.5f));
    if ((mask >> l) & 1u) want = std::min(want, persist_tiles_cap);
    if (pinned) want = pinned;
    uint32_t tiles = 0, ppt = 0;
    tiling_for(max_n, want, b->group[l], &tiles, &ppt);
#ifdef A3D_DIAGNOSTICS
    if (const char* env = getenv("A3D_ICP_VARIANT")) {
      unsigned ep = 0, eg = 0;
      if (sscanf(env, "%u,%u", &ep, &eg) == 2 && ep && (eg == 1 || eg == 2)) {
        b->group[l] = eg;
        ppt = ((ep + 1) / 2) * 2;
        tiles = (max_n + 256 * ppt - 1) / (256 * ppt);
      }
    }
#endif
    for (uint32_t p = 0; p < P; ++p) {
      LevelDesc& d = b->h_descs[(size_t)l * P + p];
      d.ppt = ppt;
      if (pinned) {
        uint32_t t_own = 0;
        tiling_for(d.src_n, pinned, 1, &t_own, &d.ppt);
        tiles = p == 0 ? t_own : std::max(tiles, t_own);
      }
    }
    b->tiles[l] = tiles, b->ppt[l] = ppt;
    if (((mask >> l) & 1u) && (uint64_t)tiles * P > b->persist_resident_blocks) mask &= ~(1u << l);
  }
  uint32_t run = 0;
  for (uint32_t l = L; l-- > 0;) {
    if (!((mask >> l) & 1u)) break;
    run |= 1u << l;
  }
  b->persist_mask = b->persist_disabled ? 0u : run;
}

#ifdef A3D_DIAGNOSTICS
a3d_status launch_pixel_kernel(a3d_multiscale_batch* b, uint32_t level, const SolveArgs& solve, uint32_t p0,
                               uint32_t count, hipStream_t s) {
  dim3 grid(b->tiles[level], count), block(256);
  const LevelDesc* descs = b->d_descs + (size_t)level * b->n_pairs + p0;
  JobState* states = b->d_states + p0;
  float* partials = b->d_partials + (size_t)p0 * b->max_tiles * GN_PARTIAL;
  unsigned* counters = b->d_counters + p0;
  const int ppt = (int)b->ppt[level];
  if (b->use_mfma) {
    if (b->group[level] == 2)
      hipLaunchKernelGGL((image_icp_mfma_kernel<2>), grid, block, 0, s, descs, states, b->gates[level],
                         partials, counters, solve, ppt);
    else
      hipLaunchKernelGGL((image_icp_mfma_kernel<1>), grid, block, 0, s, descs, states, b->gates[level],
                         partials, counters, solve, ppt);
  } else {
    if (b->group[level] == 4)
      hipLaunchKernelGGL((image_icp_kernel<4, false>), grid, block, 0, s, descs, states, b->gates[level], partials,
                         counters, solve, ppt);
    else if (b->group[level] == 2)
      hipLaunchKernelGGL((image_icp_kernel<2, false>), grid, block, 0, s, descs, states, b->gates[level], partials,
                         counters, solve, ppt);
    else if (b->merged_accumulators && solve.mode == SOLVE_IMAGE_ICP) {
      SolveArgs merged = solve;
      merged.mode = SOLVE_IMAGE_ICP_MERGED;
      hipLaunchKernelGGL((image_icp_kernel<1, true>), grid, block, 0, s, descs, states, b->gates[level], partials,
                         counters, merged, ppt);
    } else
      hipLaunchKernelGGL((image_icp_kernel<1, false>), grid, block, 0, s, descs, states, b->gates[level], partials,
                         counters, solve, ppt);
  }
  A3D_HIP_TRY(hipGetLastError());
  return A3D_OK;
}
#endif

a3d_status launch_head_kernel(a3d_multiscale_batch* b, uint32_t level, uint32_t seq, const HeadArgs& prev, uint32_t p0,
                              uint32_t count, hipStream_t s) {
  const uint32_t P = b->n_pairs;
  const uint32_t job_stride = b->max_tiles * GN_PARTIAL;
  const JobState* st_in = b->d_states + (size_t)(seq & 1u) * P + p0;
  JobState* st_out = b->d_states + (size_t)((seq + 1u) & 1u) * P + p0;
  const float* part_in = b->d_partials + (size_t)((seq + 1u) & 1u) * b->partials_half + (size_t)p0 * job_stride;
  float* part_out = b->d_partials + (size_t)(seq & 1u) * b->partials_half + (size_t)p0 * job_stride;
  const LevelDesc* descs = b->d_descs + (size_t)level * P + p0;
  if (b->zmask)
    hipLaunchKernelGGL(image_icp_head_kernel<true>, dim3(b->tiles[level], count), dim3(256), 0, s, descs, st_in, st_out,
                       b->gates[level], part_in, part_out, job_stride, prev);
  else
    hipLaunchKernelGGL(image_icp_head_kernel<false>, dim3(b->tiles[level], count), dim3(256), 0, s, descs, st_in, st_out,
                       b->gates[level], part_in, part_out, job_stride, prev);
  A3D_HIP_TRY(hipGetLastError());
  return A3D_OK;
}

a3d_status batch_commit_descs(a3d_multiscale_batch* b) {
  const uint32_t P = b->n_pairs, L = b->n_levels;
  plan_tiling(b);
  size_t max_partials = 1;
  for (uint32_t l = 0; l < L; ++l) max_partials = std::max(max_partials, (size_t)P * b->tiles[l] * GN_PARTIAL);
  b->max_tiles = (uint32_t)(max_partials / ((size_t)P * GN_PARTIAL));
  const char* zenv = A3D_DIAG_ENV("A3D_ICP_ZMASK");
  b->zmask = !(zenv && atoi(zenv) == 0);
  for (const LevelDesc& dsc : b->h_descs) b->zmask = b->zmask && (dsc.flags & 1u);
  b->partials_half = max_partials;
  if (b->partials_capacity < 2 * max_partials) {
    if (b->d_partials) A3D_HIP_TRY(hipFree(b->d_partials));
    b->d_partials = nullptr;
    b->partials_capacity = 0;
    A3D_HIP_TRY(hipMalloc((void**)&b->d_partials, 2 * max_partials * sizeof(float)));
    b->partials_capacity = 2 * max_partials;
  }
  A3D_HIP_TRY(hipMemcpyAsync(b->d_descs, b->h_descs.data(), b->h_descs.size() * sizeof(LevelDesc),
                             hipMemcpyHostToDevice, b->ctx->stream));
  return A3D_OK;
}

a3d_status batch_create(a3d_context* ctx, const a3d_icp_params* params, uint32_t n_levels, uint32_t n_pairs,
                        std::unique_ptr<a3d_multiscale_batch>* out) {
  auto b = std::make_unique<a3d_multiscale_batch>();
  b->ctx = ctx;
  b->n_pairs = n_pairs;
  b->n_levels = n_levels;
  b->params.assign(params, params + n_levels);
  for (uint32_t l = 0; l < n_levels; ++l) b->gates.push_back(make_gates(params[l]));
  b->tiles.assign(n_levels, 0);
  b->ppt.assign(n_levels, 2);
  b->group.assign(n_levels, 1);
  b->h_descs.resize((size_t)n_levels * n_pairs);
  auto resident = [&](auto kernel, int fallback_per_cu) {
    int per_cu = 0;
    if (hipOccupancyMaxActiveBlocksPerMultiprocessor(&per_cu, kernel, 256, 0) != hipSuccess || per_cu < 1)
      per_cu = fallback_per_cu;
    return (uint32_t)std::max(1, ctx->num_cus) * (uint32_t)std::max(0, per_cu);
  };
  b->resident_blocks = resident(image_icp_head_kernel<true>, 4);
#ifdef A3D_DIAGNOSTICS
  b->persist_resident_blocks = resident(image_icp_persistent_kernel<true>, 0);
  if (const char* env = getenv("A3D_ICP_ACCUM")) {
    b->use_mfma = strcmp(env, "mfma") == 0;
    b->merged_accumulators = strcmp(env, "merged") == 0;
  }
  if (const char* env = getenv("A3D_ICP_HANDOFF")) b->head_solve = strcmp(env, "ticket") != 0;
  if (const char* env = getenv("A3D_ICP_SOLVE")) b->exact_solve = strcmp(env, "exact") == 0;
  if (const char* env = getenv("A3D_ICP_PERSISTENT")) b->use_level_kernel = atoi(env) != 0;
  if (const char* env = getenv("A3D_ICP_PERSISTENT_LEVELS")) b->level_mask = (uint32_t)strtoul(env, nullptr, 0);
  if (!b->head_solve) b->resident_blocks = resident(image_icp_kernel<1, false>, 4);
  if (b->merged_accumulators) b->resident_blocks = resident(image_icp_kernel<1, true>, 4);
  b->level_resident_blocks = resident(image_icp_level_kernel<1>, 0);
  if (b->use_level_kernel && b->level_resident_blocks) b->resident_blocks = b->level_resident_blocks;
#endif
  A3D_HIP_TRY(hipSetDevice(ctx->device));
  {
    size_t total = 0;
    auto take = [&](size_t bytes) {
      const size_t at = total;
      total += ((bytes + 255) / 256) * 256;
      return at;
    };
    const size_t o_descs = take(b->h_descs.size() * sizeof(LevelDesc)), o_states = take(2 * n_pairs * sizeof(JobState)),
                 o_counters = take((size_t)n_pairs * CTRL_WORDS_PER_PAIR * sizeof(unsigned)), o_epochs = take(n_pairs * sizeof(unsigned)),
                 o_poses = take(n_pairs * sizeof(Pose)), o_init = take(n_pairs * sizeof(Pose)),
                 o_status = take(n_pairs * sizeof(int32_t)), o_readback = take(GN_PARTIAL * sizeof(double));
    A3D_HIP_TRY(hipMalloc((void**)&b->d_block, total));
    char* base = (char*)b->d_block;
    b->d_descs = (LevelDesc*)(base + o_descs), b->d_states = (JobState*)(base + o_states);
    b->d_counters = (unsigned*)(base + o_counters);
#ifdef A3D_DIAGNOSTICS
    b->d_epochs = (unsigned*)(base + o_epochs);
#else
    (void)o_epochs;
#endif
    b->d_poses = (Pose*)(base + o_poses), b->d_init = (Pose*)(base + o_init);
    b->d_status = (int32_t*)(base + o_status), b->d_readback = (double*)(base + o_readback);
  }
  if (CTRL_WORDS_PER_PAIR)
    A3D_HIP_TRY(hipMemsetAsync(b->d_counters, 0, (size_t)n_pairs * CTRL_WORDS_PER_PAIR * sizeof(unsigned), ctx->stream));
  b->n_streams = n_pairs >= 12 ? 3u : (n_pairs >= 8 ? 2u : 1u);
  if (const char* env = A3D_DIAG_ENV("A3D_ICP_STREAMS")) b->n_streams = (uint32_t)std::min(4, std::max(1, atoi(env)));
  b->n_streams = std::min(b->n_streams, n_pairs);
#ifdef A3D_DIAGNOSTICS
  if (b->use_level_kernel) b->n_streams = 1u;
#endif
  if (b->n_streams > 1) {
    A3D_HIP_TRY(hipEventCreateWithFlags(&b->ev_fork, hipEventDisableTiming));
    for (uint32_t g = 1; g < b->n_streams; ++g) {
      A3D_TRY(ctx_side_stream(ctx, g - 1, &b->aux_streams[g - 1]));
      A3D_HIP_TRY(hipEventCreateWithFlags(&b->ev_join[g - 1], hipEventDisableTiming));
    }
  }
  A3D_HIP_TRY(hipEventCreate(&b->ev0));
  A3D_HIP_TRY(hipEventCreate(&b->ev1));
  *out = std::move(b);
  return A3D_OK;
}

a3d_status batch_enqueue(a3d_multiscale_batch* b, const Pose* d_init, uint32_t levels_to_run, float* d_matrices,
                         float* d_trace, int trace_stride) {
  hipStream_t s = b->ctx->stream;
  const uint32_t P = b->n_pairs;
  b->last_init = d_init, b->last_levels = levels_to_run, b->last_matrices = d_matrices;
  b->persist_used = false;
  A3D_HIP_TRY(hipEventRecord(b->ev0, s));
  A3D_TRY(launch_job_init(s, b->d_states, d_init, (int)P));
  size_t kidx = 0;
  int trace_index = 0;
  auto profile_begin = [&](hipStream_t ps) -> a3d_status {
    if (!b->profile_kernels) return A3D_OK;
    if (b->kev.size() < 2 * (kidx + 1)) {
      hipEvent_t e0, e1;
      A3D_HIP_TRY(hipEventCreate(&e0));
      A3D_HIP_TRY(hipEventCreate(&e1));
      b->kev.push_back(e0);
      b->kev.push_back(e1);
    }
    A3D_HIP_TRY(hipEventRecord(b->kev[2 * kidx], ps));
    return A3D_OK;
  };
  uint32_t profile_level = 0;
  auto profile_end = [&](hipStream_t ps) -> a3d_status {
    if (b->profile_kernels) A3D_HIP_TRY(hipEventRecord(b->kev[2 * kidx + 1], ps));
    if (b->kev_level.size() <= kidx) b->kev_level.resize(kidx + 1);
    b->kev_level[kidx] = (uint8_t)profile_level;
    ++kidx;
    return A3D_OK;
  };
  bool head = true;
  uint32_t S = d_trace ? 1u : b->n_streams;
#ifdef A3D_DIAGNOSTICS
  bool level_kernel = b->use_level_kernel && !b->use_mfma && b->level_resident_blocks > 0;
  for (uint32_t l = 0; l < levels_to_run; ++l)
    level_kernel = level_kernel && (uint64_t)b->tiles[l] * P <= b->level_resident_blocks && b->group[l] == 1;
  uint32_t mask = 0;
  if (!level_kernel && !b->use_mfma && !d_trace && b->level_resident_blocks > 0)
    for (uint32_t l = 0; l < levels_to_run; ++l)
      if (((b->level_mask >> l) & 1u) && (uint64_t)b->tiles[l] * P <= b->level_resident_blocks && b->group[l] == 1)
        mask |= 1u << l;
  if (level_kernel || mask) A3D_HIP_TRY(hipMemsetAsync(b->d_epochs, 0, P * sizeof(unsigned), s));
  if (level_kernel) S = 1u;
  head = b->head_solve && !level_kernel && !mask && !b->use_mfma && !b->merged_accumulators && !getenv("A3D_ICP_NOSOLVE");
  for (uint32_t l = 0; l < levels_to_run; ++l) head = head && b->group[l] == 1;
  uint32_t epoch_base = 0;
#endif
  if (S > 1) {
    A3D_HIP_TRY(hipEventRecord(b->ev_fork, s));
    for (uint32_t g = 1; g < S; ++g) A3D_HIP_TRY(hipStreamWaitEvent(b->aux_streams[g - 1], b->ev_fork, 0));
  }
  HeadArgs prev{};
  prev.mode = SOLVE_NONE;
  prev.trace = d_trace, prev.trace_stride = trace_stride;
#ifdef A3D_DIAGNOSTICS
  prev.exact_solve = b->exact_solve;
#endif
  uint32_t seq = 0;
  const uint32_t job_stride = b->max_tiles * GN_PARTIAL;
  bool finished_in_kernel = false;
  uint32_t first_per_iteration = levels_to_run;
#ifdef A3D_DIAGNOSTICS
  uint32_t pmask = head ? (b->persist_mask & ((1u << levels_to_run) - 1u)) : 0u;
  if (pmask && !((pmask >> (levels_to_run - 1)) & 1u)) pmask = 0;
  for (uint32_t l = 0; l < levels_to_run && l < 16; ++l)
    if (b->level_ready[l]) pmask = 0;
  if (pmask) {
    PersistPlan plan{};
    plan.seq0 = 0, plan.counter_base = b->counter_base, plan.trace_index0 = 0, plan.trace_stride = trace_stride;
    plan.parity = b->persist_parity;
    b->persist_parity ^= 1u;
    plan.prev = prev;
    uint32_t published = 0;
    for (uint32_t l = levels_to_run; l-- > 0;) {
      if (!((pmask >> l) & 1u) || plan.n_levels == PERSIST_MAX_LEVELS) break;
      const a3d_icp_params& prm = b->params[l];
      PersistLevel& lv = plan.lv[plan.n_levels++];
      lv.desc_base = l * P, lv.iterations = (uint32_t)prm.max_iterations, lv.tiles = b->tiles[l];
      lv.weight = prm.weight, lv.color_weight = prm.color_weight, lv.gates = b->gates[l];
      published += lv.iterations * lv.tiles;
      first_per_iteration = l;
    }
    plan.finish = first_per_iteration == 0 ? 1u : 0u;
    uint32_t grid_x = 1;
    for (uint32_t k = 0; k < plan.n_levels; ++k) grid_x = std::max(grid_x, plan.lv[k].tiles);
    if (b->profile_kernels && !b->d_stamps)
      A3D_HIP_TRY(hipMalloc((void**)&b->d_stamps, (size_t)P * 2 * PERSIST_MAX_LEVELS * sizeof(unsigned long long)));
    profile_level = 255;
    b->persist_levels.clear();
    for (uint32_t k = 0; k < plan.n_levels; ++k) b->persist_levels.push_back(plan.lv[k].desc_base / P);
    for (uint32_t g = 0; g < S; ++g) {
      const uint32_t p0 = (uint32_t)((uint64_t)P * g / S), p1 = (uint32_t)((uint64_t)P * (g + 1) / S);
      hipStream_t gs = g == 0 ? s : b->aux_streams[g - 1];
      PersistOut po{};
      if (plan.finish) po.poses = b->d_poses + p0, po.status = b->d_status + p0, po.matrices = d_matrices ? d_matrices + (size_t)p0 * 16 : nullptr;
      po.stamps = b->profile_kernels ? b->d_stamps + (size_t)p0 * 2 * plan.n_levels : nullptr;
      PersistPlan gp = plan;
      gp.prev.trace = d_trace;
      A3D_TRY(profile_begin(gs));
      if (b->zmask)
        hipLaunchKernelGGL(image_icp_persistent_kernel<true>, dim3(grid_x, p1 - p0), dim3(256), 0, gs, b->d_descs + p0, P,
                           b->d_states + p0, b->d_partials + (size_t)p0 * job_stride, (uint32_t)b->partials_half, job_stride,
                           b->d_counters + (size_t)p0 * PAIR_CTRL_WORDS, gp, po);
      else
        hipLaunchKernelGGL(image_icp_persistent_kernel<false>, dim3(grid_x, p1 - p0), dim3(256), 0, gs, b->d_descs + p0, P,
                           b->d_states + p0, b->d_partials + (size_t)p0 * job_stride, (uint32_t)b->partials_half, job_stride,
                           b->d_counters + (size_t)p0 * PAIR_CTRL_WORDS, gp, po);
      A3D_HIP_TRY(hipGetLastError());
      A3D_TRY(profile_end(gs));
    }
    b->persist_used = true;
    b->counter_base += published;
    for (uint32_t k = 0; k < plan.n_levels; ++k) {
      const PersistLevel& lv = plan.lv[k];
      if (!lv.iterations) continue;
      prev.weight = lv.weight, prev.color_weight = lv.color_weight, prev.mode = SOLVE_IMAGE_ICP, prev.tiles = lv.tiles;
      prev.first_in_level = lv.iterations == 1, prev.last_in_level = 1;
      seq += lv.iterations, trace_index += (int)lv.iterations;
      prev.trace_index = trace_index - 1;
    }
    finished_in_kernel = plan.finish != 0;
  }
#endif
  for (uint32_t l = first_per_iteration; l-- > 0;) {
    const a3d_icp_params& prm = b->params[l];
    profile_level = l;
    if (l < 16 && b->level_ready[l])
      for (uint32_t g = 0; g < S; ++g) A3D_HIP_TRY(hipStreamWaitEvent(g == 0 ? s : b->aux_streams[g - 1], b->level_ready[l], 0));
    if (head) {
      for (uint64_t it = 0; it < prm.max_iterations; ++it) {
        for (uint32_t g = 0; g < S; ++g) {
          const uint32_t p0 = (uint32_t)((uint64_t)P * g / S), p1 = (uint32_t)((uint64_t)P * (g + 1) / S);
          hipStream_t gs = g == 0 ? s : b->aux_streams[g - 1];
          A3D_TRY(profile_begin(gs));
          A3D_TRY(launch_head_kernel(b, l, seq, prev, p0, p1 - p0, gs));
          A3D_TRY(profile_end(gs));
        }
        prev.weight = prm.weight, prev.color_weight = prm.color_weight, prev.mode = SOLVE_IMAGE_ICP;
        prev.tiles = b->tiles[l];
        prev.first_in_level = it == 0, prev.last_in_level = it + 1 == prm.max_iterations;
        prev.trace_index = trace_index;
        ++trace_index;
        ++seq;
      }
      continue;
    }
#ifdef A3D_DIAGNOSTICS
    SolveArgs sa{};
    sa.weight = prm.weight, sa.color_weight = prm.color_weight;
    sa.mode = getenv("A3D_ICP_NOSOLVE") ? SOLVE_NONE : SOLVE_IMAGE_ICP;
    sa.trace = d_trace, sa.trace_stride = trace_stride;
    if (level_kernel || ((mask >> l) & 1u)) {
      if (prm.max_iterations == 0) continue;
      LevelPlan plan;
      plan.iterations = (uint32_t)prm.max_iterations;
      plan.epoch_base = epoch_base;
      plan.trace_base = trace_index;
      sa.first_in_level = sa.last_in_level = 0;
      sa.trace_index = 0;
      for (uint32_t g = 0; g < S; ++g) {
        const uint32_t p0 = (uint32_t)((uint64_t)P * g / S), p1 = (uint32_t)((uint64_t)P * (g + 1) / S);
        hipStream_t gs = g == 0 ? s : b->aux_streams[g - 1];
        A3D_TRY(profile_begin(gs));
        hipLaunchKernelGGL((image_icp_level_kernel<1>), dim3(b->tiles[l], p1 - p0), dim3(256), 0, gs,
                           b->d_descs + (size_t)l * P + p0, b->d_states + p0, b->gates[l],
                           b->d_partials + (size_t)p0 * b->max_tiles * GN_PARTIAL, b->d_counters + p0, b->d_epochs + p0,
                           sa, plan, (int)b->ppt[l]);
        A3D_HIP_TRY(hipGetLastError());
        A3D_TRY(profile_end(gs));
      }
      epoch_base += plan.iterations;
      trace_index += (int)plan.iterations;
      continue;
    }
    for (uint64_t it = 0; it < prm.max_iterations; ++it) {
      sa.first_in_level = it == 0, sa.last_in_level = it + 1 == prm.max_iterations;
      sa.trace_index = trace_index;
      for (uint32_t g = 0; g < S; ++g) {
        const uint32_t p0 = (uint32_t)((uint64_t)P * g / S), p1 = (uint32_t)((uint64_t)P * (g + 1) / S);
        hipStream_t gs = g == 0 ? s : b->aux_streams[g - 1];
        A3D_TRY(profile_begin(gs));
        A3D_TRY(launch_pixel_kernel(b, l, sa, p0, p1 - p0, gs));
        A3D_TRY(profile_end(gs));
      }
      ++trace_index;
    }
#endif
  }
  for (uint32_t g = 1; g < S; ++g) {
    A3D_HIP_TRY(hipEventRecord(b->ev_join[g - 1], b->aux_streams[g - 1]));
    A3D_HIP_TRY(hipStreamWaitEvent(s, b->ev_join[g - 1], 0));
  }
  if (finished_in_kernel) {
  } else if (head) {
    A3D_TRY(launch_job_finish_head(s, b->d_states + (size_t)(seq & 1u) * P,
                                   b->d_partials + (size_t)((seq + 1u) & 1u) * b->partials_half, job_stride, prev,
                                   b->d_poses, b->d_status, d_matrices, (int)P));
  } else {
    A3D_TRY(launch_job_finish(s, b->d_states, b->d_poses, b->d_status, d_matrices, (int)P));
  }
  A3D_HIP_TRY(hipEventRecord(b->ev1, s));
  b->last_kernel_launches = kidx;
  b->last_groups = S;
  return A3D_OK;
}

void batch_drain_after_failure(a3d_multiscale_batch* b) {
  for (uint32_t g = 1; g < b->n_streams; ++g)
    if (b->aux_streams[g - 1]) (void)hipStreamSynchronize(b->aux_streams[g - 1]);
  (void)hipStreamSynchronize(b->ctx->stream);
  (void)hipGetLastError();
  if (CTRL_WORDS_PER_PAIR)
    (void)hipMemsetAsync(b->d_counters, 0, (size_t)b->n_pairs * CTRL_WORDS_PER_PAIR * sizeof(unsigned), b->ctx->stream);
  b->counter_base = 0, b->persist_parity = 0;
}

a3d_status batch_collect_timing(a3d_multiscale_batch* b) {
  A3D_HIP_TRY(hipEventSynchronize(b->ev1));
  A3D_HIP_TRY(hipEventElapsedTime(&b->last_total_ms, b->ev0, b->ev1));
  b->last_kernel_ms = 0.f;
  for (int l = 0; l < 16; ++l) b->last_level_ms[l] = 0.f, b->last_level_launches[l] = 0;
  if (b->profile_kernels) {
    for (size_t k = 0; k < b->last_kernel_launches; ++k) {
      float ms = 0.f;
      A3D_HIP_TRY(hipEventElapsedTime(&ms, b->kev[2 * k], b->kev[2 * k + 1]));
      b->last_kernel_ms += ms;
      const uint32_t l = k < b->kev_level.size() ? b->kev_level[k] : 0u;
      if (l < 16) b->last_level_ms[l] += ms, ++b->last_level_launches[l];
    }
    if (b->persist_used && b->d_stamps && !b->persist_levels.empty()) {
      const uint32_t P = b->n_pairs, nl = (uint32_t)b->persist_levels.size(), S = b->last_groups;
      std::vector<unsigned long long> st((size_t)P * 2 * nl);
      A3D_HIP_TRY(hipMemcpy(st.data(), b->d_stamps, st.size() * sizeof(unsigned long long), hipMemcpyDeviceToHost));
      for (uint32_t g = 0; g < S; ++g) {
        const uint32_t p0 = (uint32_t)((uint64_t)P * g / S), p1 = (uint32_t)((uint64_t)P * (g + 1) / S);
        for (uint32_t k = 0; k < nl; ++k) {
          unsigned long long lo = ~0ull, hi = 0;
          for (uint32_t p = p0; p < p1; ++p) {
            lo = std::min(lo, st[((size_t)p * nl + k) * 2]);
            hi = std::max(hi, st[((size_t)p * nl + k) * 2 + 1]);
          }
          const uint32_t l = b->persist_levels[k];
          if (l < 16 && hi >= lo) {
// ... 462 lines not shown
```

### include/align3d_hip.h

```cpp
#ifndef ALIGN3D_HIP_H
#define ALIGN3D_HIP_H

#include <stddef.h>
#include <stdint.h>

#ifdef __cplusplus
extern "C" {
#endif

#define A3D_ABI_VERSION 1

typedef enum a3d_status {
  A3D_OK = 0,
  A3D_INVALID_PARAMETER = 1,
  A3D_MISSING_FIELD = 2,
  A3D_SOLVE_FAILED = 3,
  A3D_HIP_ERROR = 4,
  A3D_NAN_IN_INPUT = 5,
  A3D_CAST_OVERFLOW = 6
} a3d_status;

typedef struct a3d_icp_params {
  uint64_t max_iterations;
  float weight;
  float color_weight;
  float max_point_to_plane_distance;
  float max_distance;
  float max_normal_angle;
  float max_color_distance;
} a3d_icp_params;

typedef struct a3d_pose {
  float t[3];
  float q[4];
} a3d_pose;

typedef struct a3d_range_image_view {
  const float* points;
  const uint8_t* mask;
  const float* normals;
  const uint8_t* intensities;
  const float* intensity_map;
  double fx, fy, cx, cy;
  uint64_t width, height;
} a3d_range_image_view;

typedef struct a3d_point_cloud_view {
  const float* points;
  const float* normals;
  uint64_t len;
} a3d_point_cloud_view;

typedef struct a3d_gn_state {
  float hessian[36];
  float gradient[6];
  float squared_residual_sum;
  uint64_t count;
} a3d_gn_state;

typedef struct a3d_builder_params {
  uint32_t with_normals;
  uint32_t with_intensity;
  uint32_t use_bilateral;
  uint32_t pad;
  double sigma_space, sigma_color;
  uint64_t pyramid_levels;
  float blur_sigma;
  uint32_t pad2;
} a3d_builder_params;

typedef struct a3d_context a3d_context;
typedef struct a3d_device_image a3d_device_image;
typedef struct a3d_multiscale a3d_multiscale;
typedef struct a3d_multiscale_batch a3d_multiscale_batch;
typedef struct a3d_multi_context a3d_multi_context;
typedef struct a3d_multiscale_multi_batch a3d_multiscale_multi_batch;
typedef struct a3d_kdtree a3d_kdtree;
typedef struct a3d_pcl_icp a3d_pcl_icp;


uint32_t a3d_abi_version(void);
a3d_status a3d_device_count(int32_t* out_count);
const char* a3d_last_error(void);
const char* a3d_status_string(a3d_status s);

a3d_status a3d_context_create(int32_t device_index, a3d_context** out_ctx);
a3d_status a3d_context_create_with_priority(int32_t device_index, int32_t priority, a3d_context** out_ctx);
a3d_status a3d_context_set_tiling(a3d_context* ctx, uint32_t tiles_per_pair);
a3d_status a3d_context_create_on_pipe(int32_t device_index, int32_t priority, int32_t main_slot, a3d_context** out_ctx);
a3d_status a3d_context_create_pair(int32_t device_index, a3d_context** out_aligner, a3d_context** out_builder);
a3d_status a3d_context_destroy(a3d_context* ctx);
a3d_status a3d_context_synchronize(a3d_context* ctx);
void* a3d_context_stream(a3d_context* ctx);
int32_t a3d_context_device(a3d_context* ctx);

a3d_status a3d_timer_start(a3d_context* ctx);
a3d_status a3d_timer_stop(a3d_context* ctx, float* out_ms);

a3d_status a3d_malloc(a3d_context* ctx, size_t bytes, void** out_device_ptr);
a3d_status a3d_free(a3d_context* ctx, void* device_ptr);
a3d_status a3d_host_alloc(a3d_context* ctx, size_t bytes, void** out_host_ptr);
a3d_status a3d_host_free(a3d_context* ctx, void* host_ptr);
a3d_status a3d_memcpy_h2d(a3d_context* ctx, void* dst_device, const void* src_host, size_t bytes);
a3d_status a3d_memcpy_d2h(a3d_context* ctx, void* dst_host, const void* src_device, size_t bytes);
a3d_status a3d_memcpy_d2d(a3d_context* ctx, void* dst_device, const void* src_device, size_t bytes);


void a3d_icp_params_default(a3d_icp_params* out);
void a3d_ms_icp_params_default(a3d_icp_params out[3]);


a3d_status a3d_range_image_upload(a3d_context* ctx, const a3d_range_image_view* view,
                                  a3d_device_image** out_image);
a3d_status a3d_range_image_upload_pyramid(a3d_context* ctx, const a3d_range_image_view* views, uint64_t n_levels,
                                          a3d_device_image** out_images);
a3d_status a3d_range_image_free(a3d_device_image* image);

a3d_status a3d_range_image_compute_normals(a3d_device_image* image);
a3d_status a3d_range_image_download_normals(a3d_device_image* image, float* out_normals);

void a3d_builder_params_default(a3d_builder_params* out);
a3d_status a3d_range_image_build_pyramid(a3d_context* ctx, const a3d_builder_params* params,
                                         const uint16_t* depth, const uint8_t* rgb, uint64_t width,
                                         uint64_t height, double fx, double fy, double cx, double cy,
                                         double depth_scale, a3d_device_image** out_levels);
a3d_status a3d_range_image_build_pyramids(a3d_context* ctx, const a3d_builder_params* params, uint64_t n_frames,
                                          const uint16_t* const* depth_frames, const uint8_t* const* rgb_frames,
                                          uint64_t width, uint64_t height, double fx, double fy, double cx, double cy,
                                          double depth_scale, a3d_device_image** out_levels);
a3d_status a3d_context_last_build_stats(a3d_context* ctx, uint64_t out_stats[4]);
a3d_status a3d_context_set_build_profiling(a3d_context* ctx, int32_t on);
a3d_status a3d_context_last_build_kernel_ms(a3d_context* ctx, float* out_ms);
a3d_status a3d_range_image_size(const a3d_device_image* image, uint64_t* out_width, uint64_t* out_height);
a3d_status a3d_range_image_download(a3d_device_image* image, float* points, uint8_t* mask, float* normals,
                                    uint8_t* intensities, float* intensity_map, uint8_t* colors,
                                    double out_intrinsics[4]);

a3d_status a3d_range_image_compute_normals_batch(a3d_device_image* const* images, uint64_t n);

a3d_status a3d_compute_normals(a3d_context* ctx, const float* points, const uint8_t* mask,
                               uint64_t width, uint64_t height, float* out_normals);


a3d_status a3d_image_icp_align(a3d_context* ctx, const a3d_icp_params* params,
                               const a3d_device_image* target, const a3d_device_image* source,
                               const a3d_pose* init_pose, a3d_pose* out_pose);

a3d_status a3d_image_icp_accumulate(a3d_context* ctx, const a3d_icp_params* params,
                                    const a3d_device_image* target, const a3d_device_image* source,
                                    const a3d_pose* pose, a3d_gn_state* out_geom,
                                    a3d_gn_state* out_color);

#ifdef A3D_DIAGNOSTICS
a3d_status a3d_image_icp_accumulate_exact(a3d_context* ctx, const a3d_icp_params* params, const a3d_device_image* target,
                                          const a3d_device_image* source, const a3d_pose* pose,
                                          a3d_gn_state* out_geom, a3d_gn_state* out_color);
a3d_status a3d_image_icp_accumulate_weighted(a3d_context* ctx, const a3d_icp_params* params,
                                             const a3d_device_image* target, const a3d_device_image* source,
                                             const a3d_pose* pose, a3d_gn_state* out_state);
#endif

a3d_status a3d_image_icp_align_trace(a3d_context* ctx, const a3d_icp_params* params,
                                     const a3d_device_image* target, const a3d_device_image* source,
                                     const a3d_pose* init_pose, a3d_pose* out_pose, float* out_trace);

a3d_status a3d_selftest_transform(a3d_context* ctx, const float* updates6, const a3d_pose* poses, const float* points3,
                                  uint64_t n, a3d_pose* out_composed, float* out_points3, float* out_normals3);
a3d_status a3d_selftest_division(a3d_context* ctx, const float* numerators, const float* denominators,
                                 uint64_t n, uint64_t* out_mismatches);


a3d_status a3d_multiscale_new(a3d_context* ctx, const a3d_icp_params* params, uint64_t n_params,
                              const a3d_device_image* const* target_pyramid, uint64_t n_levels,
                              a3d_multiscale** out);
a3d_status a3d_multiscale_align(a3d_multiscale* ms, const a3d_device_image* const* source_pyramid,
                                uint64_t n_source_levels, a3d_pose* out_pose);
a3d_status a3d_multiscale_align_host(a3d_multiscale* ms, const a3d_range_image_view* source_pyramid,
                                     uint64_t n_source_levels, a3d_pose* out_pose);
a3d_status a3d_multiscale_free(a3d_multiscale* ms);

a3d_status a3d_multiscale_batch_new(a3d_context* ctx, const a3d_icp_params* params,
                                    uint64_t n_params, uint64_t n_pairs, uint64_t n_levels,
                                    const a3d_device_image* const* target_pyramids,
                                    const a3d_device_image* const* source_pyramids,
                                    a3d_multiscale_batch** out);
a3d_status a3d_multiscale_batch_align(a3d_multiscale_batch* batch, a3d_pose* out_poses_host,
                                      float* out_matrices_device, int32_t* out_status_host);
a3d_status a3d_multiscale_batch_results(a3d_multiscale_batch* batch, a3d_pose* out_poses_host, int32_t* out_status_host);
a3d_status a3d_multiscale_batch_rebind(a3d_multiscale_batch* batch, const a3d_device_image* const* target_pyramids,
                                       const a3d_device_image* const* source_pyramids);
a3d_status a3d_multiscale_batch_free(a3d_multiscale_batch* batch);
a3d_status a3d_multiscale_batch_set_profiling(a3d_multiscale_batch* batch, int32_t on);
a3d_status a3d_multiscale_batch_last_kernel_ms(a3d_multiscale_batch* batch, float* out_kernel_ms);
a3d_status a3d_multiscale_batch_last_level_ms(a3d_multiscale_batch* batch, uint32_t level, float* out_ms,
                                              uint32_t* out_launches);
a3d_status a3d_multiscale_batch_persistent_levels(a3d_multiscale_batch* batch, uint32_t* out_mask);
a3d_status a3d_multiscale_batch_concurrency(a3d_multiscale_batch* batch, uint32_t* out_streams);
a3d_status a3d_multiscale_batch_last_timing(a3d_multiscale_batch* batch, float* out_total_ms,
                                            uint64_t* out_pixel_kernel_launches);


a3d_status a3d_multi_shard_range(uint64_t n_items, uint64_t n_devices, uint64_t device, uint64_t* out_begin,
                                 uint64_t* out_end);
a3d_status a3d_multi_context_create(const int32_t* device_ids, uint64_t n_devices, a3d_multi_context** out);
a3d_status a3d_multi_context_destroy(a3d_multi_context* mc);
uint64_t a3d_multi_context_size(const a3d_multi_context* mc);
a3d_context* a3d_multi_context_device(a3d_multi_context* mc, uint64_t index);
a3d_status a3d_multiscale_batch_new_multi(a3d_multi_context* mc, const a3d_icp_params* params, uint64_t n_params,
                                          uint64_t n_pairs, uint64_t n_levels,
                                          const a3d_device_image* const* target_pyramids,
                                          const a3d_device_image* const* source_pyramids,
                                          a3d_multiscale_multi_batch** out);
a3d_status a3d_multiscale_multi_batch_align(a3d_multiscale_multi_batch* batch, a3d_pose* out_poses_host,
                                            float* out_matrices_host, int32_t* out_status_host,
                                            const float** out_matrices_device0);
a3d_status a3d_multiscale_multi_batch_free(a3d_multiscale_multi_batch* batch);


a3d_status a3d_kdtree_new(a3d_context* ctx, const float* points, uint64_t n, a3d_kdtree** out);
a3d_status a3d_kdtree_new_device(a3d_context* ctx, const void* d_points, uint64_t n, a3d_kdtree** out);
a3d_status a3d_kdtree_build_path(a3d_kdtree* tree, int32_t* out_path);
a3d_status a3d_kdtree_build_ms(a3d_kdtree* tree, float* out_ms);
a3d_status a3d_kdtree_nearest(a3d_kdtree* tree, const float* queries, uint64_t m,
                              uint64_t* out_indices, float* out_sqr_distances);
a3d_status a3d_kdtree_nearest_device(a3d_kdtree* tree, const void* d_queries, uint64_t m,
                                     void* d_indices, void* d_sqr_distances);
a3d_status a3d_kdtree_free(a3d_kdtree* tree);
a3d_status a3d_kdtree_stats(a3d_kdtree* tree, uint64_t out3[3]);
a3d_status a3d_kdtree_download(a3d_kdtree* tree, float* out_split, float* out_leaves, uint64_t out_counts[2]);


a3d_status a3d_pcl_icp_new(a3d_context* ctx, const a3d_icp_params* params,
                           const a3d_point_cloud_view* target, a3d_pcl_icp** out);
a3d_status a3d_pcl_icp_align(a3d_pcl_icp* icp, const a3d_point_cloud_view* source,
                             a3d_pose* out_pose);
a3d_status a3d_pcl_icp_new_device(a3d_context* ctx, const a3d_icp_params* params,
                                  const a3d_point_cloud_view* d_target, a3d_pcl_icp** out);
a3d_status a3d_pcl_icp_align_device(a3d_pcl_icp* icp, const a3d_point_cloud_view* d_source,
                                    a3d_pose* out_pose);
a3d_status a3d_pcl_icp_accumulate(a3d_pcl_icp* icp, const a3d_point_cloud_view* source,
                                  const a3d_pose* pose, a3d_gn_state* out_state);
a3d_status a3d_pcl_icp_last_device_ms(a3d_pcl_icp* icp, float* out_ms);
a3d_status a3d_pcl_icp_free(a3d_pcl_icp* icp);


void a3d_bilateral_default_sigmas(double* out_sigma_space, double* out_sigma_color);
a3d_status a3d_bilateral_filter_u16(a3d_context* ctx, const uint16_t* image, uint64_t width,
                                    uint64_t height, double sigma_space, double sigma_color,
                                    uint16_t* out_image, uint64_t out_grid_dims[3]);
a3d_status a3d_bilateral_filter_u16_device(a3d_context* ctx, const uint16_t* d_images, uint64_t n_images,
                                           uint64_t width, uint64_t height, double sigma_space, double sigma_color,
                                           uint16_t* d_out);

#ifdef __cplusplus
}
#endif
#endif
```

Measured before the change: 22370 frame-pairs/s.

## Recompute level-0 ICP points from a stored 16-bit depth plane

```diff
diff --git a/align3d_amd/_abi.py b/align3d_amd/_abi.py
--- a/align3d_amd/_abi.py
+++ b/align3d_amd/_abi.py
@@ -233,6 +233,7 @@
         _ST,
         [_P, C.POINTER(IcpParamsC), _P, _P, C.POINTER(PoseC), C.POINTER(GnStateC)],
     ),
+    "a3d_range_image_download_depth16": (_ST, [_P, _P, C.POINTER(C.c_float), C.POINTER(C.c_int32)]),
 }
 
 _CSRC = os.path.join(os.path.dirname(os.path.abspath(__file__)), "csrc")
diff --git a/align3d_amd/csrc/common.hpp b/align3d_amd/csrc/common.hpp
--- a/align3d_amd/csrc/common.hpp
+++ b/align3d_amd/csrc/common.hpp
@@ -228,5 +228,8 @@
   a3d::DeviceArena* arena = nullptr;
   bool built = false;
   bool mask_is_z = false;
+  uint16_t* depth16 = nullptr;
+  float depth_scale = 0, bp_fx = 0, bp_fy = 0, bp_cx = 0, bp_cy = 0;
+  bool points_from_depth = false;
   bool own_normals = false;
 };
diff --git a/align3d_amd/csrc/devmath.hpp b/align3d_amd/csrc/devmath.hpp
--- a/align3d_amd/csrc/devmath.hpp
+++ b/align3d_amd/csrc/devmath.hpp
@@ -191,6 +191,22 @@
 __device__ __forceinline__ bool div_den_ok(float z) { return (fabsf(z) > 1e-9f) & (fabsf(z) < 1e9f); }
 __device__ __forceinline__ bool div_num_ok(float a) { return (a == 0.0f) | ((fabsf(a) > 1e-20f) & (fabsf(a) < 1e9f)); }
 
+__device__ __forceinline__ V3 backproject_px(uint32_t d, int row, int col, float fx, float fy, float cx, float cy, float scale,
+                                             const DivBy dfx, const DivBy dfy, bool focal_ok) {
+  V3 p{0.f, 0.f, 0.f};
+  if (d > 0) {
+    p.z = (float)d * scale;
+    const float ax = ((float)col - cx) * p.z, ay = ((float)row - cy) * p.z;
+    const bool fast = focal_ok & div_num_ok(ax) & div_num_ok(ay);
+    if (__builtin_expect(__builtin_amdgcn_ballot_w64(!fast) != 0ull, 0)) {
+      p.x = ax / fx, p.y = ay / fy;
+    } else {
+      p.x = ax == 0.0f ? ax : div_by(ax, dfx), p.y = ay == 0.0f ? ay : div_by(ay, dfy);
+    }
+  }
+  return p;
+}
+
 
 __device__ __forceinline__ V3 normal_from_neighbours_dev(V3 center, V3 left, V3 right, V3 top, V3 bottom) {
   const float ld = norm_squared(left - center), rd = norm_squared(right - center);
diff --git a/align3d_amd/csrc/frame.hip b/align3d_amd/csrc/frame.hip
--- a/align3d_amd/csrc/frame.hip
+++ b/align3d_amd/csrc/frame.hip
@@ -42,6 +42,20 @@
   __builtin_nontemporal_store(v, (uint8_t __attribute__((address_space(1)))*)((a3d_gptr)base + idx));
 #endif
 }
+__device__ __forceinline__ void st_u16u_stream(void* base, uint32_t idx, uint16_t v) {
+#ifdef A3D_BUILDER_NO_NT
+  *(uint16_t __attribute__((address_space(1)))*)((a3d_gptr)base + idx * 2u) = v;
+#else
+  __builtin_nontemporal_store(v, (uint16_t __attribute__((address_space(1)))*)((a3d_gptr)base + idx * 2u));
+#endif
+}
+__device__ __forceinline__ void st_u16x2u_stream(void* base, uint32_t idx, uint32_t lo, uint32_t hi) {
+#ifdef A3D_BUILDER_NO_NT
+  *(uint32_t __attribute__((address_space(1)))*)((a3d_gptr)base + idx * 2u) = lo | (hi << 16);
+#else
+  __builtin_nontemporal_store(lo | (hi << 16), (uint32_t __attribute__((address_space(1)))*)((a3d_gptr)base + idx * 2u));
+#endif
+}
 __device__ __forceinline__ V3 ld_v3g(const float* base, size_t idx) {
   const f32x3 v = *(const f32x3_u*)(base + 3 * idx);
   return V3{v.x, v.y, v.z};
@@ -50,6 +64,7 @@
 struct LevelLayout {
   uint32_t w, h;
   size_t points, mask, normals, colors, intensities, imap;
+  size_t depth16;
 };
 constexpr uint32_t MAX_LEVELS = 16;
 struct PyramidLayout {
@@ -95,7 +110,7 @@
     level0_kernel(const uint16_t* __restrict__ depth, uint32_t w, uint32_t h, double inv_ss, double inv_sc,
                   const double* __restrict__ grids, unsigned long long capacity, uint32_t* __restrict__ scal, float fx,
                   float fy, float cx, float cy, float scale, FrameBases bases, size_t off_points, size_t off_mask,
-                  size_t off_normals, bool with_normals, LevelLayout L1, bool emit_l1) {
+                  size_t off_normals, size_t off_depth16, bool with_normals, LevelLayout L1, bool emit_l1) {
   __shared__ float sp[3][ST_H][ST_W + 1];
   __shared__ float sn[3][OWN_H][OWN_W + 1];
   __shared__ uint8_t sm[ST_H][ST_W];
@@ -132,16 +147,8 @@
           d[k] = v;
         }
       }
-      if (d[k] > 0) {
-        pz[k] = (float)d[k] * scale;
-        const float ax = ((float)col - cx) * pz[k], ay = ((float)row[k] - cy) * pz[k];
-        const bool fast = focal_ok & div_num_ok(ax) & div_num_ok(ay);
-        if (__builtin_expect(__builtin_amdgcn_ballot_w64(!fast) != 0ull, 0)) {
-          px[k] = ax / fx, py[k] = ay / fy;
-        } else {
-          px[k] = ax == 0.0f ? ax : div_by(ax, dfx), py[k] = ay == 0.0f ? ay : div_by(ay, dfy);
-        }
-      }
+      const V3 p = backproject_px(d[k], row[k], col, fx, fy, cx, cy, scale, dfx, dfy, focal_ok);
+      px[k] = p.x, py[k] = p.y, pz[k] = p.z;
     }
     sp[0][ly[k]][lx] = px[k], sp[1][ly[k]][lx] = py[k], sp[2][ly[k]][lx] = pz[k];
     sm[ly[k]][lx] = d[k] > 0 ? 1 : 0;
@@ -168,6 +175,7 @@
       const uint32_t idx = __umul24((uint32_t)row[k], w) + (uint32_t)col;
       st_v3u_stream(base + off_points, idx, V3{px[k], py[k], pz[k]});
       st_u8u_stream(base + off_mask, idx, d[k] > 0 ? 1 : 0);
+      st_u16u_stream(base + off_depth16, idx, (uint16_t)d[k]);
       if (with_normals) st_v3u_stream(base + off_normals, idx, nrm[k]);
     }
   if (!emit_l1 || A3D_L0_PROBE == 3 || A3D_L0_PROBE == 4) return;
@@ -200,28 +208,14 @@
 
 constexpr int QS = 32, QT = QS / 2;
 
-__device__ __forceinline__ V3 backproject_px(uint32_t d, int row, int col, float fx, float fy, float cx, float cy, float scale,
-                                             const DivBy dfx, const DivBy dfy, bool focal_ok) {
-  V3 p{0.f, 0.f, 0.f};
-  if (d > 0) {
-    p.z = (float)d * scale;
-    const float ax = ((float)col - cx) * p.z, ay = ((float)row - cy) * p.z;
-    const bool fast = focal_ok & div_num_ok(ax) & div_num_ok(ay);
-    if (__builtin_expect(__builtin_amdgcn_ballot_w64(!fast) != 0ull, 0)) {
-      p.x = ax / fx, p.y = ay / fy;
-    } else {
-      p.x = ax == 0.0f ? ax : div_by(ax, dfx), p.y = ay == 0.0f ? ay : div_by(ay, dfy);
-    }
-  }
-  return p;
-}
 
 template <bool FILTER>
 __global__ void __launch_bounds__(256)
     level0_quad_kernel(const uint16_t* __restrict__ depth, uint32_t w, uint32_t h, double inv_ss, double inv_sc,
                        const double* __restrict__ grids, unsigned long long capacity, uint32_t* __restrict__ scal, float fx,
                        float fy, float cx, float cy, float scale, FrameBases bases, size_t off_points, size_t off_mask,
-                       size_t off_normals, bool with_normals, LevelLayout L1, bool emit_l1, LevelLayout L2, bool emit_l2,
+                       size_t off_normals, size_t off_depth16, bool with_normals, LevelLayout L1, bool emit_l1, LevelLayout L2,
+                       bool emit_l2,
                        bool l2_is_last, Unsplat unsplat, uint32_t patches_x, uint32_t patches_y) {
   __shared__ float sp[3][QS + 2][QS + 3];
   __shared__ float s1[2][3][QT][QT + 1];
@@ -391,6 +385,19 @@
                                                                                (__umul24((uint32_t)(r0 + my), w) + (uint32_t)(c0 + mx))));
   }
   store_rows(off_points, !mask_words);
+  if (A3D_LQ_PROBE != 1) {
+#pragma unroll
+    for (int a = 0; a < 2; ++a) {
+      if (!rin[a]) continue;
+      const uint32_t i0 = __umul24((uint32_t)row[a], w) + (uint32_t)col[0];
+      if ((w & 1u) == 0) {
+        if (cin[0]) st_u16x2u_stream(base + off_depth16, i0, d[a][0], d[a][1]);
+      } else {
+        if (cin[0]) st_u16u_stream(base + off_depth16, i0, (uint16_t)d[a][0]);
+        if (cin[1]) st_u16u_stream(base + off_depth16, i0 + 1u, (uint16_t)d[a][1]);
+      }
+    }
+  }
   if (with_normals) {
     __syncthreads();
 #pragma unroll
@@ -770,6 +777,7 @@
     L.colors = take(n * 3);
     L.points = take(n * 12);
     L.mask = take(n);
+    L.depth16 = l == 0 ? take(n * 2) : 0;
     L.normals = prm->with_normals ? take(n * 12) : 0;
     L.intensities = prm->with_intensity ? take(n) : 0;
     L.imap = prm->with_intensity ? take((size_t)(L.w + 2) * (L.h + 2) * 4) : 0;
@@ -817,8 +825,8 @@
     if (quad) {
       hipLaunchKernelGGL(level0_quad_kernel<true>, dim3(gridq.x * gridq.y * gridq.z), dim3(256), 0, s, d_depth, w, h, 1.0 / prm->sigma_space,
                          1.0 / prm->sigma_color, (const double*)gb.blurred, gb.capacity, gb.scal, fx, fy, cx, cy, depth_scale,
-                         bases, L0.points, L0.mask, L0.normals, prm->with_normals != 0, P.lv[1], fuse_l1, L2, fuse_l2, l2_is_last,
-                         gb.unsplat, gridq.x, gridq.y);
+                         bases, L0.points, L0.mask, L0.normals, L0.depth16, prm->with_normals != 0, P.lv[1], fuse_l1, L2, fuse_l2,
+                         l2_is_last, gb.unsplat, gridq.x, gridq.y);
       if (defer) {
         A3D_HIP_TRY(hipGetLastError());
         ctx->grid_clean = gb.clean;
@@ -828,20 +836,21 @@
     else
       hipLaunchKernelGGL(level0_kernel<true>, dim3((w + OWN_W - 1) / OWN_W, (h + OWN_H - 1) / OWN_H, F), dim3(L0_THREADS), 0, s,
                          d_depth, w, h, 1.0 / prm->sigma_space, 1.0 / prm->sigma_color, (const double*)gb.blurred, gb.capacity,
-                         gb.scal, fx, fy, cx, cy, depth_scale, bases, L0.points, L0.mask, L0.normals, prm->with_normals != 0,
-                         P.lv[1], fuse_l1);
+                         gb.scal, fx, fy, cx, cy, depth_scale, bases, L0.points, L0.mask, L0.normals, L0.depth16,
+                         prm->with_normals != 0, P.lv[1], fuse_l1);
 #endif
     A3D_HIP_TRY(hipMemcpyAsync(result, gb.scal, (size_t)F * SC_STRIDE * sizeof(uint32_t), hipMemcpyDeviceToHost, s));
   } else {
     if (quad)
       hipLaunchKernelGGL(level0_quad_kernel<false>, dim3(gridq.x * gridq.y * gridq.z), dim3(256), 0, s, d_depth, w, h, 0.0, 0.0,
                          (const double*)nullptr, 0ull, (uint32_t*)nullptr, fx, fy, cx, cy, depth_scale, bases, L0.points, L0.mask,
-                         L0.normals, prm->with_normals != 0, P.lv[1], fuse_l1, L2, fuse_l2, l2_is_last, Unsplat{}, gridq.x, gridq.y);
+                         L0.normals, L0.depth16, prm->with_normals != 0, P.lv[1], fuse_l1, L2, fuse_l2, l2_is_last, Unsplat{},
+                         gridq.x, gridq.y);
 #ifdef A3D_DIAGNOSTICS
     else
       hipLaunchKernelGGL(level0_kernel<false>, dim3((w + OWN_W - 1) / OWN_W, (h + OWN_H - 1) / OWN_H, F), dim3(L0_THREADS), 0, s,
                          d_depth, w, h, 0.0, 0.0, (const double*)nullptr, 0ull, (uint32_t*)nullptr, fx, fy, cx, cy, depth_scale,
-                         bases, L0.points, L0.mask, L0.normals, prm->with_normals != 0, P.lv[1], fuse_l1);
+                         bases, L0.points, L0.mask, L0.normals, L0.depth16, prm->with_normals != 0, P.lv[1], fuse_l1);
 #endif
   }
   float sigma = prm->blur_sigma;
@@ -889,7 +898,7 @@
 
 a3d_status chunk_prepare(a3d_context* ctx, const a3d_builder_params* prm, const ArenaPlan& plan, Chunk& c,
                          const uint16_t* const* depth, const uint8_t* const* rgb, uint32_t w, uint32_t h, double fx,
-                         double fy, double cx, double cy, hipEvent_t uploaded, bool mask_is_z) {
+                         double fy, double cx, double cy, float depth_scale, hipEvent_t uploaded, bool mask_is_z) {
   const size_t n = (size_t)w * h;
   const uint64_t L = prm->pyramid_levels;
   for (uint32_t f = 0; f < c.F; ++f) {
@@ -911,6 +920,12 @@
       im->fx64 = fx * k, im->fy64 = fy * k, im->cx64 = cx * k, im->cy64 = cy * k;
       im->fx = (float)im->fx64, im->fy = (float)im->fy64, im->cx = (float)im->cx64, im->cy = (float)im->cy64;
       char* b = (char*)arena->base;
+      if (l == 0) {
+        im->depth16 = (uint16_t*)(b + Y.depth16);
+        im->depth_scale = depth_scale;
+        im->bp_fx = (float)fx, im->bp_fy = (float)fy, im->bp_cx = (float)cx, im->bp_cy = (float)cy;
+        im->points_from_depth = mask_is_z;
+      }
       im->colors = (uint8_t*)(b + Y.colors), im->points = (float*)(b + Y.points), im->mask = (uint8_t*)(b + Y.mask);
       if (prm->with_normals) im->normals = (float*)(b + Y.normals), im->has_normals = true;
       if (prm->with_intensity) {
@@ -989,8 +1004,8 @@
     c.result = ctx->pinned_words + k * (MAX_BATCH * SC_STRIDE);
     const float fscale = (float)depth_scale;
     const bool mask_is_z = fscale >= 1.1754944e-38f && std::isfinite(fscale);
-    const a3d_status st = chunk_prepare(ctx, prm, plan, c, depth + f0, rgb + f0, w, h, fx, fy, cx, cy, ctx->copy_events[k],
-                                        mask_is_z);
+    const a3d_status st = chunk_prepare(ctx, prm, plan, c, depth + f0, rgb + f0, w, h, fx, fy, cx, cy, fscale,
+                                        ctx->copy_events[k], mask_is_z);
     if (st != A3D_OK) return fail(st);
   }
   std::vector<size_t> todo(n_chunks);
@@ -1181,4 +1196,20 @@
   return A3D_OK;
 }
 
-}
+#ifdef A3D_DIAGNOSTICS
+a3d_status a3d_range_image_download_depth16(a3d_device_image* im, uint16_t* out_depth, float out_backproject[5],
+                                            int32_t* out_points_from_depth) {
+  A3D_REQUIRE(im && out_depth && out_backproject && out_points_from_depth, A3D_INVALID_PARAMETER, "null argument");
+  A3D_REQUIRE(im->depth16, A3D_MISSING_FIELD, "image has no depth plane");
+  hipSetDevice(im->ctx->device);
+  const size_t n = (size_t)im->width * im->height;
+  A3D_HIP_TRY(hipMemcpyAsync(out_depth, im->depth16, n * 2, hipMemcpyDeviceToHost, im->ctx->stream));
+  A3D_HIP_TRY(hipStreamSynchronize(im->ctx->stream));
+  out_backproject[0] = im->bp_fx, out_backproject[1] = im->bp_fy, out_backproject[2] = im->bp_cx;
+  out_backproject[3] = im->bp_cy, out_backproject[4] = im->depth_scale;
+  *out_points_from_depth = im->points_from_depth ? 1 : 0;
+  return A3D_OK;
+}
+#endif
+
+}
diff --git a/align3d_amd/csrc/image_icp.hip b/align3d_amd/csrc/image_icp.hip
--- a/align3d_amd/csrc/image_icp.hip
+++ b/align3d_amd/csrc/image_icp.hip
@@ -20,9 +20,14 @@
   float fx, fy, cx, cy;
   uint32_t flags;
   uint32_t ppt;
+  uint32_t src_w;
+  const uint16_t* src_depth;
+  const uint16_t* tgt_depth;
+  float src_bp[5], tgt_bp[5];
+  float src_inv_w;
   uint32_t pad;
 };
-static_assert(sizeof(LevelDesc) == 96, "LevelDesc layout");
+static_assert(sizeof(LevelDesc) == 160, "LevelDesc layout");
 
 struct Gates {
   float max_distance_sqr;
@@ -78,11 +83,44 @@
   V3 sp;
   uint8_t intensity;
   bool live;
+  uint32_t depth, row, col;
 };
-template <bool ZMASK = false>
+struct BackProj {
+  float fx, fy, cx, cy, scale;
+  DivBy dfx, dfy;
+  bool focal_ok;
+};
+struct BackProj2 {
+  BackProj src, tgt;
+};
+__device__ __forceinline__ float uniform_f(float x) {
+  return __int_as_float(__builtin_amdgcn_readfirstlane(__float_as_int(x)));
+}
+__device__ __forceinline__ BackProj make_backproj(const float (&k)[5]) {
+  BackProj b;
+  b.fx = k[0], b.fy = k[1], b.cx = k[2], b.cy = k[3], b.scale = k[4];
+  const DivBy dx = div_prepare(b.fx), dy = div_prepare(b.fy);
+  b.dfx = DivBy{uniform_f(dx.negz), uniform_f(dx.y)}, b.dfy = DivBy{uniform_f(dy.negz), uniform_f(dy.y)};
+  b.focal_ok = div_den_ok(b.fx) & div_den_ok(b.fy);
+  return b;
+}
+constexpr int D16_TGT = 1, D16_SRC = 2;
+#ifndef A3D_ICP_DEPTH16_SRC
+#define A3D_ICP_DEPTH16_SRC 1
+#endif
+constexpr int D16_SIDES = D16_TGT | (A3D_ICP_DEPTH16_SRC ? D16_SRC : 0);
+template <bool ZMASK = false, int D16 = 0>
 __device__ __forceinline__ SrcPx stage_a(const LevelDesc& d, uint32_t i, bool in_range) {
   const uint32_t ii = in_range ? i : 0u;
   SrcPx s;
+  if (D16 & D16_SRC) {
+    const uint32_t r = f32_as_usize(((float)ii + 0.5f) * d.src_inv_w);
+    s.row = r, s.col = ii - __umul24(r, d.src_w);
+    s.depth = ld<uint16_t>(d.src_depth, ii * 2u);
+    s.intensity = ld<uint8_t>(d.src_intensities, ii);
+    s.live = in_range;
+    return s;
+  }
   s.sp = ld_v3(d.src_points, ii);
   s.intensity = ld<uint8_t>(d.src_intensities, ii);
   if (ZMASK) {
@@ -100,11 +138,20 @@
   V3 tp, tn;
   uint8_t tmask;
   bool live;
+  uint32_t tdepth, trow, tcol;
 };
-template <bool ZMASK = false>
-__device__ __forceinline__ ProjPx stage_b(const LevelDesc& d, const Pose& T, const SrcPx& s, float twf, float thf) {
+template <bool ZMASK = false, int D16 = 0>
+__device__ __forceinline__ ProjPx stage_b(const LevelDesc& d, const Pose& T, const SrcPx& s, float twf, float thf,
+                                          const BackProj2& bp = BackProj2{}) {
   ProjPx o;
-  o.p = transform_vector(T, s.sp);
+  V3 sp = s.sp;
+  bool slive = s.live;
+  if (D16 & D16_SRC) {
+    sp = backproject_px(s.depth, (int)s.row, (int)s.col, bp.src.fx, bp.src.fy, bp.src.cx, bp.src.cy, bp.src.scale, bp.src.dfx,
+                        bp.src.dfy, bp.src.focal_ok);
+    slive = slive & (s.depth != 0u);
+  }
+  o.p = transform_vector(T, sp);
   const float z = o.p.z, au = o.p.x * d.fx, av = o.p.y * d.fy;
   const DivBy dz = div_prepare(z);
   float qu = div_by(au, dz), qv = div_by(av, dz);
@@ -113,9 +160,15 @@
   o.u = qu + d.cx;
   o.v = qv + d.cy;
   const float ur = o.u + 0.5f, vr = o.v + 0.5f;
-  o.live = s.live & !((ur <= -1.0f) | (ur >= twf) | (vr <= -1.0f) | (vr >= thf));
+  o.live = slive & !((ur <= -1.0f) | (ur >= twf) | (vr <= -1.0f) | (vr >= thf));
   const uint32_t col = (uint32_t)f32_as_i32(ur), row = (uint32_t)f32_as_i32(vr);
   const uint32_t tidx = o.live ? __umul24(row, d.tw) + col : 0u;
+  if (D16 & D16_TGT) {
+    o.tdepth = ld<uint16_t>(d.tgt_depth, tidx * 2u);
+    o.trow = row, o.tcol = col;
+    o.tn = ld_v3(d.tgt_normals, tidx);
+    return o;
+  }
   o.tp = ld_v3(d.tgt_points, tidx);
   o.tn = ld_v3(d.tgt_normals, tidx);
   o.tmask = ZMASK ? (uint8_t)0 : ld<uint8_t>(d.tgt_mask, tidx);
@@ -126,11 +179,21 @@
   float t00, t10, t01, t11;
   uint32_t ui, vi;
 };
-template <bool ZMASK = false>
-__device__ __forceinline__ MapPx stage_c(const LevelDesc& d, const Gates& gt, ProjPx& px, uint32_t mw) {
+template <bool ZMASK = false, int D16 = 0>
+__device__ __forceinline__ MapPx stage_c(const LevelDesc& d, const Gates& gt, ProjPx& px, uint32_t mw,
+                                         const BackProj2& bp = BackProj2{}) {
+  bool tvalid;
+  if (D16 & D16_TGT) {
+    const uint32_t td = px.live ? px.tdepth : 0u;
+    px.tp = backproject_px(td, (int)px.trow, (int)px.tcol, bp.tgt.fx, bp.tgt.fy, bp.tgt.cx, bp.tgt.cy, bp.tgt.scale,
+                           bp.tgt.dfx, bp.tgt.dfy, bp.tgt.focal_ok);
+    tvalid = td != 0u;
+  } else {
+    tvalid = ZMASK ? px.tp.z != 0.0f : px.tmask == 1;
+  }
   const V3 diff = px.tp - px.p;
   const float pn = dot(px.p, px.tn);
-  px.live = px.live & (ZMASK ? px.tp.z != 0.0f : px.tmask == 1)
+  px.live = px.live & tvalid
             & !(norm_squared(diff) > gt.max_distance_sqr)
             & !((pn >= -1.0f) & (pn <= gt.dot_reject_max));
   MapPx m;
@@ -343,23 +406,26 @@
 
 #endif
 
-template <bool ZMASK>
+template <bool ZMASK, int D16 = 0>
 __device__ __forceinline__ SrcPx pixel_source_at(const LevelDesc& d, uint32_t base, int ppt, int k0) {
   const uint32_t i = base + (uint32_t)k0 * 256u;
-  return stage_a<ZMASK>(d, i, (k0 < ppt) && (i < d.src_n));
-}
-template <bool ZMASK>
+  return stage_a<ZMASK, D16>(d, i, (k0 < ppt) && (i < d.src_n));
+}
+template <bool ZMASK, int D16 = 0>
 __device__ __forceinline__ void pixel_pass(const LevelDesc& d, const Gates& gt, const Pose& T, uint32_t base, int ppt,
                                            const SrcPx& s0, SrcPx sa, float (&acc)[GN_PARTIAL]) {
   const uint32_t mw = d.tw + 2;
   const float twf = (float)d.tw, thf = (float)d.th;
+  BackProj2 bp{};
+  if (D16 & D16_SRC) bp.src = make_backproj(d.src_bp);
+  if (D16 & D16_TGT) bp.tgt = make_backproj(d.tgt_bp);
   SrcPx sb;
-  ProjPx pa = stage_b<ZMASK>(d, T, s0, twf, thf), pb;
+  ProjPx pa = stage_b<ZMASK, D16>(d, T, s0, twf, thf, bp), pb;
   uint8_t ia = s0.intensity, ib;
   auto step = [&](ProjPx& cur, uint8_t cur_i, ProjPx& nxt, uint8_t& nxt_i, const SrcPx& s_next, SrcPx& s_new, int k0) {
-    s_new = pixel_source_at<ZMASK>(d, base, ppt, k0 + 2);
-    const MapPx mp = stage_c<ZMASK>(d, gt, cur, mw);
-    nxt = stage_b<ZMASK>(d, T, s_next, twf, thf);
+    s_new = pixel_source_at<ZMASK, D16>(d, base, ppt, k0 + 2);
+    const MapPx mp = stage_c<ZMASK, D16>(d, gt, cur, mw, bp);
+    nxt = stage_b<ZMASK, D16>(d, T, s_next, twf, thf, bp);
     nxt_i = s_next.intensity;
     if (cur.live) {
       const Terms t = stage_d(d, gt, cur, mp, cur_i, mw);
@@ -374,7 +440,7 @@
   }
 }
 
-template <bool ZMASK>
+template <bool ZMASK, bool DEPTH16>
 __global__ void __launch_bounds__(256, 1)
     image_icp_head_kernel(const LevelDesc* __restrict__ descs, const JobState* __restrict__ states_in,
                           JobState* __restrict__ states_out, Gates gt, const float* __restrict__ partials_in,
@@ -396,7 +462,8 @@
   const LevelDesc d = descs[pair];
   const int ppt = (int)d.ppt;
   const uint32_t base = tile * (256u * (uint32_t)ppt) + threadIdx.x;
-  const SrcPx s0 = pixel_source_at<ZMASK>(d, base, ppt, 0), s1 = pixel_source_at<ZMASK>(d, base, ppt, 1);
+  constexpr int D16 = DEPTH16 ? D16_SIDES : 0;
+  const SrcPx s0 = pixel_source_at<ZMASK, D16>(d, base, ppt, 0), s1 = pixel_source_at<ZMASK, D16>(d, base, ppt, 1);
   A3D_HEAD_STAMP(1);
   head_advance(states_in + pair, tile == 0 ? states_out + pair : nullptr, partials_in + (size_t)pair * job_stride, head,
                pair, s_state, tile == 0);
@@ -404,7 +471,7 @@
   if ((int)s_state[15] == A3D_OK) {
     auto uni = [&](int k) { return __uint_as_float(__builtin_amdgcn_readfirstlane(s_state[k])); };
     const Pose T{{uni(0), uni(1), uni(2)}, {uni(3), uni(4), uni(5), uni(6)}};
-    pixel_pass<ZMASK>(d, gt, T, base, ppt, s0, s1, acc);
+    pixel_pass<ZMASK, D16>(d, gt, T, base, ppt, s0, s1, acc);
   }
   A3D_HEAD_STAMP(3);
   block_reduce_store<GN_PARTIAL, false>(acc, partials_out + (size_t)pair * job_stride + (size_t)tile * GN_PARTIAL);
@@ -532,7 +599,7 @@
     for (uint32_t it = 0; it < lv.iterations; ++it) {
       const uint32_t base0 = rank * (256u * (uint32_t)ppt) + threadIdx.x;
       SrcPx s0{}, s1{};
-      if (mine) s0 = pixel_source_at<ZMASK>(d, base0, ppt, 0), s1 = pixel_source_at<ZMASK>(d, base0, ppt, 1);
+      if (mine) s0 = pixel_source_at<ZMASK, 0>(d, base0, ppt, 0), s1 = pixel_source_at<ZMASK, 0>(d, base0, ppt, 1);
       head(rank == 0);
       if (!alive) break;
       const bool ok = (int)s_state[15] == A3D_OK;
@@ -545,8 +612,8 @@
         for (int k = 0; k < GN_PARTIAL; ++k) acc[k] = 0.0f;
         if (ok && tile < own_tiles) {
           const uint32_t base = tile * (256u * (uint32_t)ppt) + threadIdx.x;
-          if (tile != rank) s0 = pixel_source_at<ZMASK>(d, base, ppt, 0), s1 = pixel_source_at<ZMASK>(d, base, ppt, 1);
-          pixel_pass<ZMASK>(d, lv.gates, T, base, ppt, s0, s1, acc);
+          if (tile != rank) s0 = pixel_source_at<ZMASK, 0>(d, base, ppt, 0), s1 = pixel_source_at<ZMASK, 0>(d, base, ppt, 1);
+          pixel_pass<ZMASK, 0>(d, lv.gates, T, base, ppt, s0, s1, acc);
         }
         block_reduce_store<GN_PARTIAL, true>(acc, job_partials + (size_t)(seq & 1u) * partials_half + (size_t)tile * GN_PARTIAL);
         __syncthreads();
@@ -880,6 +947,7 @@
   bool profile_kernels = false;
   uint32_t resident_blocks = 1024;
   bool zmask = false;
+  bool depth16 = false;
   uint32_t n_streams = 1;
   hipStream_t aux_streams[3] = {nullptr, nullptr, nullptr};
   hipEvent_t ev_fork = nullptr, ev_join[3] = {nullptr, nullptr, nullptr};
@@ -932,6 +1000,15 @@
   d->fx = target->fx, d->fy = target->fy, d->cx = target->cx, d->cy = target->cy;
   d->flags = (target->mask_is_z && source->mask_is_z) ? 1u : 0u;
   d->ppt = 2, d->pad = 0;
+  d->src_w = source->width;
+  d->src_inv_w = 1.0f / (float)std::max(1u, source->width);
+  const bool from_depth = target->points_from_depth && source->points_from_depth && target->depth16 && source->depth16;
+  if (from_depth) d->flags |= 2u;
+  d->src_depth = from_depth ? source->depth16 : nullptr;
+  d->tgt_depth = from_depth ? target->depth16 : nullptr;
+  const float sbp[5] = {source->bp_fx, source->bp_fy, source->bp_cx, source->bp_cy, source->depth_scale};
+  const float tbp[5] = {target->bp_fx, target->bp_fy, target->bp_cx, target->bp_cy, target->depth_scale};
+  for (int k = 0; k < 5; ++k) d->src_bp[k] = sbp[k], d->tgt_bp[k] = tbp[k];
   return A3D_OK;
 }
 
@@ -1062,12 +1139,15 @@
   const float* part_in = b->d_partials + (size_t)((seq + 1u) & 1u) * b->partials_half + (size_t)p0 * job_stride;
   float* part_out = b->d_partials + (size_t)(seq & 1u) * b->partials_half + (size_t)p0 * job_stride;
   const LevelDesc* descs = b->d_descs + (size_t)level * P + p0;
-  if (b->zmask)
-    hipLaunchKernelGGL(image_icp_head_kernel<true>, dim3(b->tiles[level], count), dim3(256), 0, s, descs, st_in, st_out,
-                       b->gates[level], part_in, part_out, job_stride, prev);
+  if (b->depth16 && level == 0)
+    hipLaunchKernelGGL((image_icp_head_kernel<true, true>), dim3(b->tiles[level], count), dim3(256), 0, s, descs, st_in,
+                       st_out, b->gates[level], part_in, part_out, job_stride, prev);
+  else if (b->zmask)
+    hipLaunchKernelGGL((image_icp_head_kernel<true, false>), dim3(b->tiles[level], count), dim3(256), 0, s, descs, st_in,
+                       st_out, b->gates[level], part_in, part_out, job_stride, prev);
   else
-    hipLaunchKernelGGL(image_icp_head_kernel<false>, dim3(b->tiles[level], count), dim3(256), 0, s, descs, st_in, st_out,
-                       b->gates[level], part_in, part_out, job_stride, prev);
+    hipLaunchKernelGGL((image_icp_head_kernel<false, false>), dim3(b->tiles[level], count), dim3(256), 0, s, descs, st_in,
+                       st_out, b->gates[level], part_in, part_out, job_stride, prev);
   A3D_HIP_TRY(hipGetLastError());
   return A3D_OK;
 }
@@ -1081,6 +1161,12 @@
   const char* zenv = A3D_DIAG_ENV("A3D_ICP_ZMASK");
   b->zmask = !(zenv && atoi(zenv) == 0);
   for (const LevelDesc& dsc : b->h_descs) b->zmask = b->zmask && (dsc.flags & 1u);
+  const char* denv = A3D_DIAG_ENV("A3D_ICP_DEPTH16");
+  b->depth16 = b->zmask && L > 0 && !(denv && atoi(denv) == 0);
+  for (uint32_t p = 0; p < P && b->depth16; ++p) {
+    const LevelDesc& dsc = b->h_descs[p];
+    b->depth16 = (dsc.flags & 2u) && dsc.src_n <= (1u << 22);
+  }
   b->partials_half = max_partials;
   if (b->partials_capacity < 2 * max_partials) {
     if (b->d_partials) A3D_HIP_TRY(hipFree(b->d_partials));
@@ -1112,7 +1198,7 @@
       per_cu = fallback_per_cu;
     return (uint32_t)std::max(1, ctx->num_cus) * (uint32_t)std::max(0, per_cu);
   };
-  b->resident_blocks = resident(image_icp_head_kernel<true>, 4);
+  b->resident_blocks = resident(image_icp_head_kernel<true, false>, 4);
 #ifdef A3D_DIAGNOSTICS
   b->persist_resident_blocks = resident(image_icp_persistent_kernel<true>, 0);
   if (const char* env = getenv("A3D_ICP_ACCUM")) {
diff --git a/include/align3d_hip.h b/include/align3d_hip.h
--- a/include/align3d_hip.h
+++ b/include/align3d_hip.h
@@ -158,6 +158,8 @@
 a3d_status a3d_image_icp_accumulate_weighted(a3d_context* ctx, const a3d_icp_params* params,
                                              const a3d_device_image* target, const a3d_device_image* source,
                                              const a3d_pose* pose, a3d_gn_state* out_state);
+a3d_status a3d_range_image_download_depth16(a3d_device_image* image, uint16_t* out_depth, float out_backproject[5],
+                                            int32_t* out_points_from_depth);
 #endif
 
 a3d_status a3d_image_icp_align_trace(a3d_context* ctx, const a3d_icp_params* params,
```

Measured after the change: 23870 frame-pairs/s (median of 6 runs). 1.07x the previous value.
